# Nashatyrev/shadow

Hardware: AMD Instinct MI355X
Metric: APSP wall time + source-SSSPs/sec, 10k-vertex GML graph, 1/2/4/8 MI355X (higher is better)
Workload: dtype u32+f32

## Files before the change

### include/shadow_routing.h

```cpp
#ifndef SHADOW_ROUTING_H
#define SHADOW_ROUTING_H

#include <stddef.h>
#include <stdint.h>

#ifdef __cplusplus
extern "C" {
#endif

#define SRG_OK 0
#define SRG_ERR_ARG 1
#define SRG_ERR_NO_EDGE 2
#define SRG_ERR_MULTI_EDGE 3
#define SRG_ERR_UNREACHABLE 4
#define SRG_ERR_LATENCY_RANGE 5
#define SRG_ERR_HIP 6
#define SRG_ERR_OOM 7
#define SRG_ERR_PARSE 8
#define SRG_ERR_RCCL 9
#define SRG_ERR_INTERNAL 10

typedef struct srg_edge_list {
    uint32_t num_vertices;
    uint32_t directed;
    uint64_t num_edges;
    const uint32_t* src;
    const uint32_t* dst;
    const uint64_t* latency_ns;
    const float* packet_loss;
    const uint32_t* node_ids;
} srg_edge_list;

typedef struct srg_stats {
    double ms_total;
    double ms_h2d;
    double ms_build;
    double ms_fw;
    double ms_scan;
    double ms_loss;
    double ms_extract;
    double ms_d2h;
    int32_t path_kind;
    int32_t loss_rounds;
    uint64_t multi_pred_pairs;
    uint64_t relaxations;
    uint64_t essential_edges;
    int32_t scan_kind;
    int32_t table_keys;
    uint64_t prof_launches;
    double prof_kernel_ms;
    uint64_t prof_relaxations;
    double ms_exchange;
    int32_t nranks;
    int32_t rank;
    uint64_t local_sources;
    double ms_host_register;
    uint64_t d2h_overlapped_bytes;
    uint64_t min_latency_ns;
    uint64_t latency_unit_ns;
    int32_t fw_overlap_pivots;
    int32_t fw_overlap_kept;
    int32_t d2h_key_rows;
    int32_t reserved0;
    double ms_key_widen;
} srg_stats;

#define SRG_PATH_DENSE_U32 0
#define SRG_PATH_DENSE_U64 1
#define SRG_PATH_DIRECT 2
#define SRG_PATH_SPARSE_U32 3
#define SRG_PATH_SPARSE_U64 4

#define SRG_SCAN_NONE 0
#define SRG_SCAN_SPARSE 1
#define SRG_SCAN_DENSE 2

typedef struct srg_ctx srg_ctx;

int srg_create(srg_ctx** out, int device, char* errbuf, size_t errlen);
void srg_destroy(srg_ctx* ctx);


#define SRG_OPT_PROFILING 1
#define SRG_OPT_SPARSE_THRESHOLD 2
#define SRG_OPT_GATHER_OUTPUT 3
#define SRG_OPT_ALGORITHM 4
#define SRG_ALGO_AUTO 0
#define SRG_ALGO_DENSE 1
#define SRG_ALGO_SPARSE 2
#define SRG_OPT_SPARSE_LOCALITY 5
#define SRG_OPT_SIMULATE_RANK 6
#define SRG_OPT_FW_TILE 7
#define SRG_OPT_SPARSE_DELTA_DIV 12
#define SRG_OPT_SPARSE_GLOBAL_BITMAPS 14
#define SRG_OPT_FW_SYMMETRIC 17
#define SRG_OPT_D2H_MODE 20
#define SRG_OPT_LOSS_CHUNKS 21
#define SRG_OPT_SCAN_GROUPS 22
#define SRG_OPT_H2D_CODEC 25
#define SRG_OPT_EDGE_SHARD 29
#define SRG_OPT_LATE_LOSS 30
#define SRG_OPT_FW_LINE_SPLIT 31
#define SRG_OPT_FW_STEP 32
#define SRG_OPT_FW_OVERLAP 33
#define SRG_OPT_TEST_FAULT 34
#define SRG_OPT_TABLE_POOL_BYTES 35
#define SRG_OPT_TABLE_POOL_IDLE_BYTES 36
#define SRG_OPT_CREATE_MS_RUNTIME 37
#define SRG_OPT_CREATE_MS_LIBRARY 38
#define SRG_OPT_FW_XCD_ORDER 39
#define SRG_OPT_SCAN_MIRROR 40
#define SRG_OPT_SCAN_MIRRORED 41
#define SRG_OPT_SCAN_MIRROR_CAP 42
#define SRG_OPT_LOSS_KIND 43
#define SRG_OPT_ROUTE_TREE_ROWS 44
#define SRG_LOSS_NONE 0
#define SRG_LOSS_ROWS_LDS 1
#define SRG_LOSS_GLOBAL_ENTRIES 2
#define SRG_LOSS_DENSE_SCAN 3
int srg_set_option(srg_ctx* ctx, int option, double value);
int srg_get_option(srg_ctx* ctx, int option, double* value);

int srg_compute_shortest_paths(srg_ctx* ctx, const srg_edge_list* graph,
                               const uint32_t* nodes, uint32_t num_nodes,
                               uint64_t* out_latency_ns, float* out_packet_loss,
                               srg_stats* stats, char* errbuf, size_t errlen);

int srg_compute_shortest_paths_device(srg_ctx* ctx, const srg_edge_list* graph_dev,
                                      const uint32_t* nodes_dev, uint32_t num_nodes,
                                      uint64_t* out_latency_ns_dev, float* out_packet_loss_dev,
                                      void* hip_stream, srg_stats* stats,
                                      char* errbuf, size_t errlen);

int srg_get_direct_paths(srg_ctx* ctx, const srg_edge_list* graph,
                         const uint32_t* nodes, uint32_t num_nodes,
                         uint64_t* out_latency_ns, float* out_packet_loss,
                         srg_stats* stats, char* errbuf, size_t errlen);

typedef struct srg_routing_info srg_routing_info;
int srg_routing_info_build(srg_ctx* ctx, const srg_edge_list* graph, const uint32_t* gml_ids, uint32_t num_ids,
                           int use_shortest_paths, srg_routing_info** out, srg_stats* stats,
                           char* errbuf, size_t errlen);
struct srg_multi;
int srg_routing_info_build_multi(struct srg_multi* m, const srg_edge_list* graph, const uint32_t* gml_ids,
                                 uint32_t num_ids, int use_shortest_paths, srg_routing_info** out, srg_stats* stats,
                                 char* errbuf, size_t errlen);
void srg_routing_info_free(srg_routing_info* ri);
uint32_t srg_routing_info_num_nodes(const srg_routing_info* ri);
int srg_routing_info_path(const srg_routing_info* ri, uint32_t start_id, uint32_t end_id,
                          uint64_t* latency_ns, float* packet_loss);
void srg_routing_info_increment_packet_count(srg_routing_info* ri, uint32_t start_id, uint32_t end_id);
uint64_t srg_routing_info_packet_count(srg_routing_info* ri, uint32_t start_id, uint32_t end_id);
int srg_routing_info_smallest_latency_ns(const srg_routing_info* ri, uint64_t* out);
void srg_routing_info_tables(const srg_routing_info* ri, const uint64_t** latency_ns, const float** packet_loss,
                             const uint32_t** gml_ids, uint32_t* n);

typedef struct srg_graph srg_graph;

int srg_graph_parse_gml(const char* text, size_t len, srg_graph** out,
                        char* errbuf, size_t errlen);
void srg_graph_free(srg_graph* g);
void srg_graph_edge_list(const srg_graph* g, srg_edge_list* out);
uint32_t srg_graph_num_vertices(const srg_graph* g);
uint64_t srg_graph_num_edges(const srg_graph* g);
int srg_graph_directed(const srg_graph* g);
int srg_graph_node_index(const srg_graph* g, uint32_t gml_id, uint32_t* out_index);
uint32_t srg_graph_node_id(const srg_graph* g, uint32_t index);
void srg_graph_node_bandwidth(const srg_graph* g, uint32_t index,
                              uint64_t* down_bits, int* has_down,
                              uint64_t* up_bits, int* has_up);
void srg_graph_node_bandwidths(const srg_graph* g, uint64_t* down_bits, int* has_down,
                               uint64_t* up_bits, int* has_up);
uint32_t srg_graph_parse_chunks(const srg_graph* g);

#define SRG_UNIQUE_ID_BYTES 128
int srg_comm_unique_id(unsigned char id[SRG_UNIQUE_ID_BYTES], char* errbuf, size_t errlen);
int srg_comm_init(srg_ctx* ctx, int nranks, int rank, const unsigned char id[SRG_UNIQUE_ID_BYTES],
                  char* errbuf, size_t errlen);
typedef struct srg_local_group srg_local_group;
int srg_local_group_create(int nranks, srg_local_group** out);
void srg_local_group_release(srg_local_group* g);
int srg_comm_init_local(srg_ctx* ctx, srg_local_group* g, int rank, char* errbuf, size_t errlen);
int srg_comm_size(srg_ctx* ctx, int* nranks, int* rank);

typedef struct srg_multi srg_multi;
int srg_multi_create(srg_multi** out, const int* devices, int num_devices, char* errbuf, size_t errlen);
void srg_multi_destroy(srg_multi* m);
int srg_multi_size(const srg_multi* m);
int srg_multi_set_option(srg_multi* m, int option, double value);
int srg_multi_compute_shortest_paths(srg_multi* m, const srg_edge_list* graph, const uint32_t* nodes,
                                     uint32_t num_nodes, uint64_t* out_latency_ns, float* out_packet_loss,
                                     srg_stats* stats, char* errbuf, size_t errlen);
int srg_multi_get_direct_paths(srg_multi* m, const srg_edge_list* graph, const uint32_t* nodes, uint32_t num_nodes,
                               uint64_t* out_latency_ns, float* out_packet_loss, srg_stats* stats, char* errbuf,
                               size_t errlen);

#define SRG_ERR_EVENT_ORDER 11
typedef struct srg_event_batch {
    uint64_t num_events;
    const uint32_t* src_node;
    const uint32_t* dst_node;
    const uint32_t* src_host;
    const uint32_t* dst_host;
    const uint64_t* send_time_ns;
    const uint64_t* src_event_id;
    uint32_t num_hosts;
    uint32_t reserved;
    uint64_t round_end_ns;
} srg_event_batch;

typedef struct srg_event_result {
    uint64_t min_next_event_ns;
    uint64_t min_used_latency_ns;
    uint32_t key_bits;
    uint32_t radix_passes;
    double ms_total;
} srg_event_result;

int srg_order_packet_events_device(srg_ctx* ctx, const srg_event_batch* batch_dev,
                                   const uint64_t* latency_table_dev, uint32_t table_n,
                                   uint64_t* out_deliver_ns_dev, uint32_t* out_order_dev,
                                   uint64_t* out_host_offsets_dev, void* hip_stream,
                                   srg_event_result* result, char* errbuf, size_t errlen);

typedef struct srg_path_table_dev {
    uint32_t n, reserved;
    const uint64_t* latency_ns;
    const uint32_t* latency_key;
    const uint64_t* diag_ns;
    uint64_t unit_ns;
    const float* packet_loss;
} srg_path_table_dev;

typedef struct srg_send_batch {
    srg_event_batch ev;
    const double* chance;
    const uint32_t* payload_size;
    uint64_t bootstrap_end_ns;
} srg_send_batch;

typedef struct srg_send_result { srg_event_result ev; uint64_t num_sent, num_dropped; } srg_send_result;

int srg_send_packets_device(srg_ctx* ctx, const srg_send_batch* batch_dev, const srg_path_table_dev* table,
                            uint8_t* out_status_dev, uint64_t* out_deliver_ns_dev, uint32_t* out_order_dev,
                            uint64_t* out_host_offsets_dev, uint64_t* packet_counts_dev ,
                            void* hip_stream, srg_send_result* result, char* errbuf, size_t errlen);

int srg_routing_info_key_tables(const srg_routing_info* ri, const uint32_t** key, const uint64_t** diag_ns,
                                uint64_t* unit_ns, const float** packet_loss, uint32_t* n);
void srg_routing_info_add_packet_counts(srg_routing_info* ri, const uint64_t* counts_by_position );

#define SRG_ERR_TIME_BACKWARD 12
typedef struct srg_event_queues srg_event_queues;
int srg_event_queues_create(srg_ctx* ctx, uint32_t num_hosts, uint64_t reserve_events, srg_event_queues** out,
                            char* errbuf, size_t errlen);
void srg_event_queues_destroy(srg_event_queues* q);
uint32_t srg_event_queues_merge_tile(void);

typedef struct srg_queue_result {
    uint64_t num_moved;
    uint64_t num_queued;
    uint64_t min_next_event_ns;
    double ms_total;
} srg_queue_result;

int srg_event_queues_push_device(srg_event_queues* q, const srg_event_batch* batch_dev,
                                 const uint64_t* deliver_ns_dev, const uint32_t* order_dev, uint64_t num_order,
                                 const uint64_t* tag_dev, void* hip_stream, srg_queue_result* result, char* errbuf,
                                 size_t errlen);

int srg_event_queues_pop_device(srg_event_queues* q, uint64_t until_ns, uint64_t out_capacity,
                                uint64_t* out_time_ns_dev, uint32_t* out_src_host_dev, uint64_t* out_src_event_id_dev,
                                uint64_t* out_tag_dev, uint64_t* out_host_offsets_dev, void* hip_stream,
                                srg_queue_result* result, char* errbuf, size_t errlen);

int srg_next_window(uint64_t min_next_event_ns, uint64_t runahead_ns, uint64_t end_time_ns,
                    uint64_t* window_start_ns, uint64_t* window_end_ns);

typedef struct srg_inbound srg_inbound;
int srg_inbound_create(srg_ctx* ctx, uint32_t num_hosts, const uint64_t* bw_down_bits, uint64_t sim_start_ns,
                       uint64_t bootstrap_end_ns, uint64_t reserve_packets, srg_inbound** out, char* errbuf,
                       size_t errlen);
void srg_inbound_destroy(srg_inbound* q);

typedef struct srg_inbound_result {
    uint64_t num_forwarded, num_dropped;
    uint64_t num_queued;
    uint64_t min_next_wake_ns;
    double ms_total;
} srg_inbound_result;

int srg_inbound_step_device(srg_inbound* q, uint64_t until_ns, uint64_t num_arrivals, const uint64_t* time_ns_dev,
                            const uint32_t* total_size_dev, const uint64_t* tag_dev, const uint64_t* host_offsets_dev,
                            uint64_t out_capacity, uint8_t* out_status_dev, uint64_t* out_time_ns_dev,
                            uint64_t* out_tag_dev, uint64_t* out_host_offsets_dev, void* hip_stream,
                            srg_inbound_result* result, char* errbuf, size_t errlen);

struct srg_inbound_host_state {
    uint64_t balance, last_refill_ns;
    uint64_t interval_end_ns, drop_next_ns;
    uint64_t current_drop_count, previous_drop_count, bytes_stored;
    uint64_t queued;
    uint64_t wake_ns, cached_tag;
    uint8_t mode;
    uint8_t has_interval_end, has_drop_next, pending, has_cached, reserved[3];
};
int srg_inbound_host_state(srg_inbound* q, uint32_t host, struct srg_inbound_host_state* out);

#define SRG_ERR_ROUTE 13
typedef struct srg_route_result {
    uint64_t num_pairs;
    uint64_t total_hops;
    uint64_t bad_pair;
    uint32_t max_hops, reserved;
    double ms_total;
} srg_route_result;

int srg_trace_routes_device(srg_ctx* ctx, const srg_edge_list* graph_dev, const srg_path_table_dev* table,
                            const uint32_t* src_dev, const uint32_t* dst_dev, uint64_t num_pairs,
                            uint64_t hop_capacity, uint64_t* out_hop_offsets_dev ,
                            uint32_t* out_hop_edge_dev ,
                            uint32_t* out_hop_vertex_dev ,
                            void* hip_stream, srg_route_result* result, char* errbuf, size_t errlen);

int srg_link_loads_device(srg_ctx* ctx, const srg_edge_list* graph_dev, const srg_path_table_dev* table,
                          const uint64_t* packet_counts_dev ,
                          uint64_t* edge_packets_dev ,
                          void* hip_stream, srg_route_result* result, char* errbuf, size_t errlen);

#define SRG_ROUTE_NONE 0xFFFFFFFFu

int srg_route_trees_device(srg_ctx* ctx, const srg_edge_list* graph_dev, const srg_path_table_dev* table,
                           const uint32_t* sources_dev, uint32_t num_sources,
                           uint32_t* out_pred_edge_dev   ,
                           uint32_t* out_pred_vertex_dev ,
                           uint32_t* out_hops_dev        ,
                           uint32_t* out_first_edge_dev  ,
                           void* hip_stream, srg_route_result* result, char* errbuf, size_t errlen);

int srg_link_loads_trees_device(srg_ctx* ctx, const srg_edge_list* graph_dev, const srg_path_table_dev* table,
                                const uint64_t* packet_counts_dev, uint64_t* edge_packets_dev,
                                void* hip_stream, srg_route_result* result, char* errbuf, size_t errlen);

const char* srg_version(void);

#ifdef __cplusplus
}
#endif
#endif
```

### shadow_amd/_native.py

```python
import ctypes
import os

_HERE = os.path.dirname(os.path.abspath(__file__))
LIB_PATH = os.path.join(_HERE, "libshadow_routing.so")

SRG_OK = 0
SRG_ERR_ARG = 1
SRG_ERR_NO_EDGE = 2
SRG_ERR_MULTI_EDGE = 3
SRG_ERR_UNREACHABLE = 4
SRG_ERR_LATENCY_RANGE = 5
SRG_ERR_HIP = 6
SRG_ERR_OOM = 7
SRG_ERR_PARSE = 8
SRG_ERR_RCCL = 9
SRG_ERR_INTERNAL = 10
SRG_ERR_EVENT_ORDER = 11
SRG_ERR_TIME_BACKWARD = 12
SRG_ERR_ROUTE = 13

SRG_PATH_DENSE_U32 = 0
SRG_PATH_DENSE_U64 = 1
SRG_PATH_DIRECT = 2
SRG_PATH_SPARSE_U32 = 3
SRG_PATH_SPARSE_U64 = 4

SRG_OPT_PROFILING = 1
SRG_OPT_SPARSE_THRESHOLD = 2
SRG_OPT_GATHER_OUTPUT = 3
SRG_OPT_ALGORITHM = 4
SRG_OPT_SPARSE_LOCALITY = 5
SRG_OPT_SIMULATE_RANK = 6
SRG_OPT_FW_TILE = 7
SRG_OPT_SPARSE_DELTA_DIV = 12
SRG_OPT_SPARSE_GLOBAL_BITMAPS = 14
SRG_OPT_FW_SYMMETRIC = 17
SRG_OPT_D2H_MODE = 20
SRG_OPT_LOSS_CHUNKS = 21
SRG_OPT_SCAN_GROUPS = 22
SRG_OPT_H2D_CODEC = 25
SRG_OPT_EDGE_SHARD = 29
SRG_OPT_LATE_LOSS = 30
SRG_OPT_FW_LINE_SPLIT = 31
SRG_OPT_FW_STEP = 32
SRG_OPT_FW_OVERLAP = 33
SRG_OPT_TEST_FAULT = 34
SRG_OPT_TABLE_POOL_BYTES = 35
SRG_OPT_TABLE_POOL_IDLE_BYTES = 36
SRG_OPT_CREATE_MS_RUNTIME = 37
SRG_OPT_CREATE_MS_LIBRARY = 38
SRG_OPT_FW_XCD_ORDER = 39
SRG_OPT_SCAN_MIRROR = 40
SRG_OPT_SCAN_MIRRORED = 41
SRG_OPT_SCAN_MIRROR_CAP = 42
SRG_OPT_LOSS_KIND = 43
SRG_OPT_ROUTE_TREE_ROWS = 44
SRG_ROUTE_NONE = 0xFFFFFFFF
SRG_LOSS_NONE = 0
SRG_LOSS_ROWS_LDS = 1
SRG_LOSS_GLOBAL_ENTRIES = 2
SRG_LOSS_DENSE_SCAN = 3
SRG_ALGO_AUTO = 0
SRG_ALGO_DENSE = 1
SRG_ALGO_SPARSE = 2
SRG_UNIQUE_ID_BYTES = 128

SRG_SCAN_NONE = 0
SRG_SCAN_SPARSE = 1
SRG_SCAN_DENSE = 2

_u32p = ctypes.POINTER(ctypes.c_uint32)
_u64p = ctypes.POINTER(ctypes.c_uint64)
_f32p = ctypes.POINTER(ctypes.c_float)


class EdgeList(ctypes.Structure):
    _fields_ = [
        ("num_vertices", ctypes.c_uint32),
        ("directed", ctypes.c_uint32),
        ("num_edges", ctypes.c_uint64),
        ("src", ctypes.c_void_p),
        ("dst", ctypes.c_void_p),
        ("latency_ns", ctypes.c_void_p),
        ("packet_loss", ctypes.c_void_p),
        ("node_ids", ctypes.c_void_p),
    ]


class EventBatch(ctypes.Structure):
    _fields_ = [
        ("num_events", ctypes.c_uint64),
        ("src_node", ctypes.c_void_p),
        ("dst_node", ctypes.c_void_p),
        ("src_host", ctypes.c_void_p),
        ("dst_host", ctypes.c_void_p),
        ("send_time_ns", ctypes.c_void_p),
        ("src_event_id", ctypes.c_void_p),
        ("num_hosts", ctypes.c_uint32),
        ("reserved", ctypes.c_uint32),
        ("round_end_ns", ctypes.c_uint64),
    ]


class EventResult(ctypes.Structure):
    _fields_ = [
        ("min_next_event_ns", ctypes.c_uint64),
        ("min_used_latency_ns", ctypes.c_uint64),
        ("key_bits", ctypes.c_uint32),
        ("radix_passes", ctypes.c_uint32),
        ("ms_total", ctypes.c_double),
    ]

    def as_dict(self):
        return {k: getattr(self, k) for k, _ in self._fields_}


class PathTableDev(ctypes.Structure):
    _fields_ = [
        ("n", ctypes.c_uint32),
        ("reserved", ctypes.c_uint32),
        ("latency_ns", ctypes.c_void_p),
        ("latency_key", ctypes.c_void_p),
        ("diag_ns", ctypes.c_void_p),
        ("unit_ns", ctypes.c_uint64),
        ("packet_loss", ctypes.c_void_p),
    ]


class SendBatch(ctypes.Structure):
    _fields_ = [
        ("ev", EventBatch),
        ("chance", ctypes.c_void_p),
        ("payload_size", ctypes.c_void_p),
        ("bootstrap_end_ns", ctypes.c_uint64),
    ]


class SendResult(ctypes.Structure):
    _fields_ = [
        ("ev", EventResult),
        ("num_sent", ctypes.c_uint64),
        ("num_dropped", ctypes.c_uint64),
    ]

    def as_dict(self):
        d = self.ev.as_dict()
        d.update(num_sent=self.num_sent, num_dropped=self.num_dropped)
        return d


class QueueResult(ctypes.Structure):
    _fields_ = [
        ("num_moved", ctypes.c_uint64),
        ("num_queued", ctypes.c_uint64),
        ("min_next_event_ns", ctypes.c_uint64),
        ("ms_total", ctypes.c_double),
    ]

    def as_dict(self):
        return {k: getattr(self, k) for k, _ in self._fields_}


class InboundResult(ctypes.Structure):
    _fields_ = [
        ("num_forwarded", ctypes.c_uint64),
        ("num_dropped", ctypes.c_uint64),
        ("num_queued", ctypes.c_uint64),
        ("min_next_wake_ns", ctypes.c_uint64),
        ("ms_total", ctypes.c_double),
    ]

    def as_dict(self):
        return {k: getattr(self, k) for k, _ in self._fields_}


class InboundHostState(ctypes.Structure):
    _fields_ = [
        ("balance", ctypes.c_uint64),
        ("last_refill_ns", ctypes.c_uint64),
        ("interval_end_ns", ctypes.c_uint64),
        ("drop_next_ns", ctypes.c_uint64),
        ("current_drop_count", ctypes.c_uint64),
        ("previous_drop_count", ctypes.c_uint64),
        ("bytes_stored", ctypes.c_uint64),
        ("queued", ctypes.c_uint64),
        ("wake_ns", ctypes.c_uint64),
        ("cached_tag", ctypes.c_uint64),
        ("mode", ctypes.c_uint8),
        ("has_interval_end", ctypes.c_uint8),
        ("has_drop_next", ctypes.c_uint8),
        ("pending", ctypes.c_uint8),
        ("has_cached", ctypes.c_uint8),
        ("reserved", ctypes.c_uint8 * 3),
    ]

    def as_dict(self):
        return {k: int(getattr(self, k)) for k, _ in self._fields_ if k != "reserved"}


class RouteResult(ctypes.Structure):
    _fields_ = [
        ("num_pairs", ctypes.c_uint64),
        ("total_hops", ctypes.c_uint64),
        ("bad_pair", ctypes.c_uint64),
        ("max_hops", ctypes.c_uint32),
        ("reserved", ctypes.c_uint32),
        ("ms_total", ctypes.c_double),
    ]

    def as_dict(self):
        return {k: getattr(self, k) for k, _ in self._fields_}


class Stats(ctypes.Structure):
    _fields_ = [
        ("ms_total", ctypes.c_double),
        ("ms_h2d", ctypes.c_double),
        ("ms_build", ctypes.c_double),
        ("ms_fw", ctypes.c_double),
        ("ms_scan", ctypes.c_double),
        ("ms_loss", ctypes.c_double),
        ("ms_extract", ctypes.c_double),
        ("ms_d2h", ctypes.c_double),
        ("path_kind", ctypes.c_int32),
        ("loss_rounds", ctypes.c_int32),
        ("multi_pred_pairs", ctypes.c_uint64),
        ("relaxations", ctypes.c_uint64),
        ("essential_edges", ctypes.c_uint64),
        ("scan_kind", ctypes.c_int32),
        ("table_keys", ctypes.c_int32),
        ("prof_launches", ctypes.c_uint64),
        ("prof_kernel_ms", ctypes.c_double),
        ("prof_relaxations", ctypes.c_uint64),
        ("ms_exchange", ctypes.c_double),
        ("nranks", ctypes.c_int32),
        ("rank", ctypes.c_int32),
        ("local_sources", ctypes.c_uint64),
        ("ms_host_register", ctypes.c_double),
        ("d2h_overlapped_bytes", ctypes.c_uint64),
        ("min_latency_ns", ctypes.c_uint64),
        ("latency_unit_ns", ctypes.c_uint64),
        ("fw_overlap_pivots", ctypes.c_int32),
        ("fw_overlap_kept", ctypes.c_int32),
        ("d2h_key_rows", ctypes.c_int32),
        ("reserved0", ctypes.c_int32),
        ("ms_key_widen", ctypes.c_double),
    ]

    def as_dict(self):
        return {k: getattr(self, k) for k, _ in self._fields_}


EXPORTS = [
    "srg_create", "srg_destroy", "srg_set_option", "srg_compute_shortest_paths", "srg_compute_shortest_paths_device",
    "srg_get_direct_paths", "srg_graph_parse_gml", "srg_graph_free", "srg_graph_edge_list",
    "srg_graph_num_vertices", "srg_graph_num_edges", "srg_graph_directed", "srg_graph_node_index",
    "srg_graph_node_id", "srg_graph_node_bandwidth", "srg_graph_node_bandwidths", "srg_graph_parse_chunks",
    "srg_version", "srg_comm_unique_id", "srg_comm_init",
    "srg_local_group_create", "srg_local_group_release", "srg_comm_init_local", "srg_comm_size",
    "srg_order_packet_events_device", "srg_routing_info_build", "srg_routing_info_free", "srg_routing_info_num_nodes",
    "srg_routing_info_path", "srg_routing_info_increment_packet_count", "srg_routing_info_packet_count",
    "srg_routing_info_smallest_latency_ns", "srg_routing_info_tables",
    "srg_multi_create", "srg_multi_destroy", "srg_multi_size", "srg_multi_set_option", "srg_multi_compute_shortest_paths",
    "srg_multi_get_direct_paths", "srg_routing_info_build_multi", "srg_get_option",
    "srg_send_packets_device", "srg_routing_info_key_tables", "srg_routing_info_add_packet_counts",
    "srg_event_queues_create", "srg_event_queues_destroy", "srg_event_queues_merge_tile",
    "srg_event_queues_push_device", "srg_event_queues_pop_device", "srg_next_window",
    "srg_trace_routes_device", "srg_link_loads_device", "srg_route_trees_device", "srg_link_loads_trees_device",
    "srg_inbound_create", "srg_inbound_destroy", "srg_inbound_step_device", "srg_inbound_host_state",
]

_lib = None


def lib():
    global _lib
    if _lib is not None:
        return _lib
    try:
        import torch
    except ImportError:
        pass
    if not os.path.exists(LIB_PATH):
        raise ImportError(
            f"{LIB_PATH} is missing: build it with `python shadow_amd/build.py` "
            "(hipcc --offload-arch=gfx950); there is no CPU fallback")
    L = ctypes.CDLL(os.environ.get("SRG_LIB_PATH") or LIB_PATH)
    c = ctypes
    L.srg_create.restype = c.c_int
    L.srg_create.argtypes = [c.POINTER(c.c_void_p), c.c_int, c.c_char_p, c.c_size_t]
    L.srg_set_option.restype = c.c_int
    L.srg_set_option.argtypes = [c.c_void_p, c.c_int, c.c_double]
    L.srg_destroy.restype = None
    L.srg_destroy.argtypes = [c.c_void_p]
    host_sig = [c.c_void_p, c.POINTER(EdgeList), c.c_void_p, c.c_uint32, c.c_void_p, c.c_void_p,
                c.POINTER(Stats), c.c_char_p, c.c_size_t]
    L.srg_compute_shortest_paths.restype = c.c_int
    L.srg_compute_shortest_paths.argtypes = host_sig
    L.srg_get_direct_paths.restype = c.c_int
    L.srg_get_direct_paths.argtypes = host_sig
    L.srg_compute_shortest_paths_device.restype = c.c_int
    L.srg_compute_shortest_paths_device.argtypes = [
        c.c_void_p, c.POINTER(EdgeList), c.c_void_p, c.c_uint32, c.c_void_p, c.c_void_p, c.c_void_p,
        c.POINTER(Stats), c.c_char_p, c.c_size_t]
    L.srg_graph_parse_gml.restype = c.c_int
    L.srg_graph_parse_gml.argtypes = [c.c_char_p, c.c_size_t, c.POINTER(c.c_void_p), c.c_char_p, c.c_size_t]
    L.srg_graph_free.restype = None
    L.srg_graph_free.argtypes = [c.c_void_p]
    L.srg_graph_edge_list.restype = None
    L.srg_graph_edge_list.argtypes = [c.c_void_p, c.POINTER(EdgeList)]
    L.srg_graph_num_vertices.restype = c.c_uint32
    L.srg_graph_num_vertices.argtypes = [c.c_void_p]
    L.srg_graph_num_edges.restype = c.c_uint64
    L.srg_graph_num_edges.argtypes = [c.c_void_p]
    L.srg_graph_directed.restype = c.c_int
    L.srg_graph_directed.argtypes = [c.c_void_p]
    L.srg_graph_node_index.restype = c.c_int
    L.srg_graph_node_index.argtypes = [c.c_void_p, c.c_uint32, _u32p]
    L.srg_graph_node_id.restype = c.c_uint32
    L.srg_graph_node_id.argtypes = [c.c_void_p, c.c_uint32]
    L.srg_graph_node_bandwidth.restype = None
    L.srg_graph_node_bandwidth.argtypes = [c.c_void_p, c.c_uint32, _u64p, c.POINTER(c.c_int), _u64p,
                                           c.POINTER(c.c_int)]
    L.srg_graph_node_bandwidths.restype = None
    L.srg_graph_node_bandwidths.argtypes = [c.c_void_p, c.c_void_p, c.c_void_p, c.c_void_p, c.c_void_p]
    L.srg_graph_parse_chunks.restype = c.c_uint32
    L.srg_graph_parse_chunks.argtypes = [c.c_void_p]
    L.srg_version.restype = c.c_char_p
    L.srg_version.argtypes = []
    L.srg_comm_unique_id.restype = c.c_int
    L.srg_comm_unique_id.argtypes = [c.c_char_p, c.c_char_p, c.c_size_t]
    L.srg_comm_init.restype = c.c_int
    L.srg_comm_init.argtypes = [c.c_void_p, c.c_int, c.c_int, c.c_char_p, c.c_char_p, c.c_size_t]
    L.srg_local_group_create.restype = c.c_int
    L.srg_local_group_create.argtypes = [c.c_int, c.POINTER(c.c_void_p)]
    L.srg_local_group_release.restype = None
    L.srg_local_group_release.argtypes = [c.c_void_p]
    L.srg_comm_init_local.restype = c.c_int
    L.srg_comm_init_local.argtypes = [c.c_void_p, c.c_void_p, c.c_int, c.c_char_p, c.c_size_t]
    L.srg_order_packet_events_device.restype = c.c_int
    L.srg_order_packet_events_device.argtypes = [
        c.c_void_p, c.POINTER(EventBatch), c.c_void_p, c.c_uint32, c.c_void_p, c.c_void_p, c.c_void_p, c.c_void_p,
        c.POINTER(EventResult), c.c_char_p, c.c_size_t]
    L.srg_send_packets_device.restype = c.c_int
    L.srg_send_packets_device.argtypes = [
        c.c_void_p, c.POINTER(SendBatch), c.POINTER(PathTableDev), c.c_void_p, c.c_void_p, c.c_void_p, c.c_void_p,
        c.c_void_p, c.c_void_p, c.POINTER(SendResult), c.c_char_p, c.c_size_t]
    L.srg_routing_info_key_tables.restype = c.c_int
    L.srg_routing_info_key_tables.argtypes = [c.c_void_p, c.POINTER(_u32p), c.POINTER(_u64p), _u64p, c.POINTER(_f32p),
                                              c.POINTER(c.c_uint32)]
    L.srg_routing_info_add_packet_counts.restype = None
    L.srg_routing_info_add_packet_counts.argtypes = [c.c_void_p, c.c_void_p]
    L.srg_event_queues_create.restype = c.c_int
    L.srg_event_queues_create.argtypes = [c.c_void_p, c.c_uint32, c.c_uint64, c.POINTER(c.c_void_p), c.c_char_p,
                                          c.c_size_t]
    L.srg_event_queues_destroy.restype = None
    L.srg_event_queues_destroy.argtypes = [c.c_void_p]
    L.srg_event_queues_merge_tile.restype = c.c_uint32
    L.srg_event_queues_merge_tile.argtypes = []
# ... 83 lines not shown
```

### shadow_amd/csrc/dense.hip.h

```cpp
template <class K, int T>
bool run_dense(srg_ctx& c, const DevGraph& g, const Plan& pl, const uint32_t* nodes, uint32_t n, uint64_t* out_lat,
               float* out_loss, hipStream_t st, const Prelude& P, srg_stats* stats, HostSink* sink,
               FwOverlap* ov = nullptr) {
    const bool pre = ov && ov->on && ov->ok && ov->ended && sizeof(K) == 4 && T == FwOverlap::T;
    if (sizeof(K) == 8 && c.kout_key) {
        if (!(sink && sink->widen)) fail(SRG_INTERNAL_NEED_U64, "the build needs u64 latency keys: no u32 key table");
        sink->widen = false;
        c.kout_key = nullptr;
        c.kout_diag = nullptr;
    }
    const uint32_t V = g.V;
    const size_t Vp = ((size_t)V + T - 1) / T * T;
    const size_t VV = Vp * Vp;
    const bool multi = c.comm && c.comm->nranks > 1;
    Timer tm(st);

    K* W = (K*)c.b_W.get(VV * sizeof(K));
    uint32_t* WL = (uint32_t*)c.b_WL.get(VV * 4);
    K* D = (K*)c.b_D.get(VV * sizeof(K));
    bool wl_late = false;
    if (pre) {
        wl_late = g.late && !g.late->applied;
    } else if constexpr (sizeof(K) == 4) {
        static_assert(T % 64 == 0, "tile");
        unsigned long long* KW = (unsigned long long*)c.b_PRED.get(VV * 8);
        HIP_CHECK(hipMemsetAsync(KW, 0xFF, VV * 8, st));
        wl_late = g.late && !g.late->applied;
        if (g.E) k_w_key<<<grid_for(g.E), kThreads, 0, st>>>(g.E, g.src, g.dst, g.lat, P.unit, wl_late ? nullptr : g.loss, KW, Vp);
        const unsigned nb64 = (unsigned)(Vp / 64);
        k_w_split<false><<<dim3(nb64, nb64), 256, 0, st>>>(KW, Vp, g.directed, (uint32_t*)W, WL, (uint32_t*)D);
    } else {
        loss_arrive(g, P.selfloss, st);
        k_fill<K><<<grid_for(VV), kThreads, 0, st>>>(W, VV, KeyOps<K>::INF);
        HIP_CHECK(hipMemsetAsync(WL, 0xFF, VV * 4, st));
        if (g.E) {
            k_w_lat<K><<<grid_for(g.E), kThreads, 0, st>>>(g.E, g.src, g.dst, g.lat, P.unit, g.directed, W, Vp);
            k_w_loss<K><<<grid_for(g.E), kThreads, 0, st>>>(g.E, g.src, g.dst, g.lat, P.unit, g.loss, g.directed, W, WL,
                                                             Vp);
        }
        k_init_d<K><<<grid_for(VV), kThreads, 0, st>>>(W, D, Vp);
    }
    const uint32_t nloc = (uint32_t)pl.lnodes.size();
    uint32_t* lnodes = (uint32_t*)c.b_lnodes.get(std::max<size_t>(nloc, 1) * 4);
    uint32_t* lpos = (uint32_t*)c.b_lpos.get(std::max<size_t>(nloc, 1) * 4);
    if (nloc) {
        HIP_CHECK(hipMemcpyAsync(lnodes, pl.lnodes.data(), (size_t)nloc * 4, hipMemcpyHostToDevice, st));
        HIP_CHECK(hipMemcpyAsync(lpos, pl.lpos.data(), (size_t)nloc * 4, hipMemcpyHostToDevice, st));
    }
    HIP_CHECK(hipGetLastError());
    const double ms_build = tm.lap();

    uint64_t prof_relax = 0;
    int prof_n = 0;
    double ms_dx = 0;
    if (pre) {
        prof_relax = ov->prof_relax;
        prof_n = ov->prof_n;
    } else if (sym_fw_for<K, T>(c, g)) {
        if constexpr ((sizeof(K) == 4 && T == 128) || (sizeof(K) == 8 && T == 64))
            fw_line_sym<K, T>(c, pl, D, Vp, st, prof_relax, prof_n, ms_dx);
    } else {
        if constexpr (sizeof(K) == 4) fw_blocked<K, T, 2>(c, pl, D, Vp, st, prof_relax, prof_n);
        else fw_blocked<K, T, 0>(c, pl, D, Vp, st, prof_relax, prof_n);
        if (multi) gather_rows<K>(c, pl, D, Vp, T, st, ms_dx);
    }
    HIP_CHECK(hipGetLastError());
    if (sym_fw_for<K, T>(c, g)) rb_async(c, MS_TIMEOUT, c.fw_timeout, st);
    const double ms_fw = tm.lap();
    if (sym_fw_for<K, T>(c, g) && rb_get<uint32_t>(c, MS_TIMEOUT))
        fail(SRG_ERR_HIP, fw_timeout_message(rb_get<uint32_t>(c, MS_TIMEOUT)));
#ifdef SRG_TEST_HOOKS
    if (c.test_fault == 1)
        HIP_CHECK(hipMemsetAsync(D, 0, VV * sizeof(K), st));
#endif
    if (wl_late) {
        hipStream_t ax = c.aux_stream;
        const auto tl0 = std::chrono::steady_clock::now();
        loss_arrive(g, P.selfloss, ax);
        if (srg_env::debug_overlap())
            std::fprintf(stderr, "late loss: the host waited %.2f ms for the loss thread after FW\n",
                         std::chrono::duration<double, std::milli>(std::chrono::steady_clock::now() - tl0).count());
        if constexpr (sizeof(K) == 4) {
            unsigned long long* KW = (unsigned long long*)c.b_PRED.get(VV * 8);
            HIP_CHECK(hipMemsetAsync(KW, 0xFF, VV * 8, ax));
            if (g.E) k_w_key<<<grid_for(g.E), kThreads, 0, ax>>>(g.E, g.src, g.dst, g.lat, P.unit, g.loss, KW, Vp);
            const unsigned nb64 = (unsigned)(Vp / 64);
            k_w_split<true><<<dim3(nb64, nb64), 256, 0, ax>>>(KW, Vp, g.directed, nullptr, WL, nullptr);
            HIP_CHECK(hipGetLastError());
        }
        HIP_CHECK(hipEventRecord(c.ev_wlate, ax));
    }
    if (prof_n && stats) {
        double sum = 0;
        for (int i = 0; i < prof_n; ++i) {
            float ms = 0;
            HIP_CHECK(hipEventElapsedTime(&ms, c.prof_events[2 * i], c.prof_events[2 * i + 1]));
            sum += ms;
        }
        stats->prof_launches += prof_n;
        stats->prof_kernel_ms += sum;
        stats->prof_relaxations += prof_relax;
    }

    hipStream_t cs = c.comm_stream;
    auto cs_after_st = [&]() {
        HIP_CHECK(hipEventRecord(c.ev_a, st));
        HIP_CHECK(hipStreamWaitEvent(cs, c.ev_a, 0));
    };
    auto st_after_cs = [&]() {
        HIP_CHECK(hipEventRecord(c.ev_b, cs));
        HIP_CHECK(hipStreamWaitEvent(st, c.ev_b, 0));
    };
    auto reduce_flag = [&](uint32_t* flag_dev) -> uint32_t {
        uint32_t* red = (uint32_t*)c.b_red.get(16);
        HIP_CHECK(hipMemcpyAsync(red, flag_dev, 4, hipMemcpyDeviceToDevice, st));
        if (multi) {
            cs_after_st();
            c.comm->allreduce_max_u32(red, 1, cs);
            st_after_cs();
        }
        rb_async(c, MS_REDUCE, red, st);
        HIP_CHECK(hipStreamSynchronize(st));
        return rb_get<uint32_t>(c, MS_REDUCE);
    };
    const bool exchange = multi && c.gather_output;
    auto exchange_rows = [&](void* out, size_t elem) {
        const size_t row = (size_t)n * elem;
        std::vector<size_t> offs, lens;
        slice_tables(n, pl.G, row, offs, lens);
        cs_after_st();
        c.comm->allgatherv(out, offs.data(), lens.data(), cs);
    };

    hipStream_t es = multi ? st : c.comm_stream;
    auto drain_es = [&]() {
        if (es != st) HIP_CHECK(hipStreamSynchronize(es));
    };
    constexpr int TS = 64;
    constexpr int VE = 16 / (int)sizeof(K);
    const size_t nmax = std::max<uint32_t>(nloc, 1);
    uint32_t* PRED = (uint32_t*)c.b_PRED.get(nmax * Vp * 4);
    unsigned long long* multi_cnt = (unsigned long long*)c.b_multi.get(16);
    uint32_t* mirror_cnt = (uint32_t*)(multi_cnt + 1);
    int rounds = 0;
    unsigned long long nmulti = 0;
    uint64_t n_ess = 0;
    int scan_kind = SRG_SCAN_NONE;
    bool loss_written = false;
    float* Lfin = nullptr;
    double ms_scan = 0;
    HIP_CHECK(hipMemsetAsync(multi_cnt, 0, 8, st));
    const uint32_t nw64 = (V + 63) / 64;
    unsigned long long* ess = (unsigned long long*)c.b_ess.get((size_t)V * nw64 * 8);
    k_ess_mask<K><<<V, 256, 0, es>>>(W, D, Vp, V, 0u, V, nw64, ess);
    uint32_t* indeg = (uint32_t*)c.b_indeg.get(((size_t)nw64 * 64 + 1) * 4);
    uint32_t* cscoff = (uint32_t*)c.b_cscoff.get(((size_t)nw64 * 64 + 1) * 4);
    HIP_CHECK(hipMemsetAsync(indeg, 0, ((size_t)nw64 * 64 + 1) * 4, es));
    const bool v5lo = sizeof(K) == 8;
    const uint32_t SB = V5_SB;
    const size_t npad = ((size_t)nloc + SB - 1) / SB * SB;
    const size_t dst_bytes = (size_t)nw64 * 64 * std::max<size_t>(npad, 64) * sizeof(K);
    const uint32_t NT = nw64 * 64;
    const uint32_t nK5 = (V + V5_UC - 1) / V5_UC, nbTT5 = (NT + V5_TT - 1) / V5_TT;
    const size_t NG5 = (size_t)nbTT5 * nK5 * V5_WAVES;
    uint32_t* v5_cnt = (uint32_t*)c.b_ecnt.get((size_t)nbTT5 * nK5 * V5_TT * 4);
    uint32_t* v5_goff = (uint32_t*)c.b_eoff.get((NG5 + 1) * 4);
    uint64_t E_ess = 0, E_layout = 0;
    {
        uint32_t* v5_glen = (uint32_t*)c.b_rlen.get((NG5 + 1) * 4);
        HIP_CHECK(hipMemsetAsync(v5_cnt, 0, (size_t)nbTT5 * nK5 * V5_TT * 4, es));
        HIP_CHECK(hipMemsetAsync(v5_glen, 0, (NG5 + 1) * 4, es));
        const size_t nwaves = (size_t)nw64 * nK5;
        k_v5_count<<<(unsigned)((nwaves * 64 + 255) / 256), 256, 0, es>>>(ess, V, nw64, nK5, v5_cnt, v5_glen, indeg);
        HIP_CHECK(hipGetLastError());
        size_t ta = 0, tc = 0;
        HIP_CHECK(hipcub::DeviceScan::ExclusiveSum(nullptr, ta, indeg, cscoff, (int)(NT + 1), es));
        HIP_CHECK(hipcub::DeviceScan::ExclusiveSum(nullptr, tc, v5_glen, v5_goff, (int)(NG5 + 1), es));
        const size_t tbytes = std::max(ta, tc);
        void* tmp = c.b_scantmp.get(tbytes);
        HIP_CHECK(hipcub::DeviceScan::ExclusiveSum(tmp, ta, indeg, cscoff, (int)(NT + 1), es));
        HIP_CHECK(hipcub::DeviceScan::ExclusiveSum(tmp, tc, v5_glen, v5_goff, (int)(NG5 + 1), es));
        HIP_CHECK(hipGetLastError());
    }

    HIP_CHECK(hipMemsetAsync(&P.flags->inf_in_used_row, 0, 4, st));
    HIP_CHECK(hipMemsetAsync(&P.flags->impossible, 0, 4, st));
    if (nloc)
        k_certify<K><<<nloc, kThreads, 0, st>>>(
            D, Vp, lnodes, nloc, nodes, n,
            (K)std::min<uint64_t>(min_edge_key(P.es.min_lat_inv, P.unit), (uint64_t)KeyOps<K>::INF), P.flags);
    const bool simulated = c.comm && std::strcmp(c.comm->kind(), "simulated") == 0;
    uint32_t impossible = 0, inf_any = 0;
    if (multi) {
        impossible = reduce_flag(&P.flags->impossible);
        inf_any = reduce_flag(&P.flags->inf_in_used_row);
    } else {
        rb_async(c, MS_REDUCE, &P.flags->impossible, st);
        rb_async(c, MS_REDUCE2, &P.flags->inf_in_used_row, st);
        HIP_CHECK(hipStreamSynchronize(st));
        impossible = rb_get<uint32_t>(c, MS_REDUCE);
        inf_any = rb_get<uint32_t>(c, MS_REDUCE2);
    }
    if (impossible && !simulated)
        fail(SRG_ERR_INTERNAL, "FW produced an impossible table: a used pair's latency is below the smallest edge "
                               "latency (" + std::to_string(~P.es.min_lat_inv) + " ns)");
    if (sizeof(K) == 4 && inf_any) {
        const unsigned __int128 bound = (unsigned __int128)P.max_key * (V > 1 ? V - 1 : 1);
        if (bound >= KeyOps<uint32_t>::INF) {
            if (wl_late) HIP_CHECK(hipStreamWaitEvent(st, c.ev_wlate, 0));
            drain_es();
            return false;
        }
        fail(SRG_ERR_UNREACHABLE,
             "assertion `left == right` failed: paths.len() != nodes.len().pow(2) (a used node is unreachable "
             "from another used node)");
    }
    if (P.wrap_risk) {
        const unsigned __int128 bound = (unsigned __int128)P.max_key * (V > 1 ? V - 1 : 1);
        const bool inf_known = sizeof(K) == 4 ? bound < KeyOps<uint32_t>::INF : !P.range_risk;
        HIP_CHECK(hipMemsetAsync(&P.flags->wrap, 0, 8, st));
        for (uint32_t r0 = 0; r0 < nloc && g.E; r0 += 32768) {
            const uint32_t nr = std::min<uint32_t>(32768, nloc - r0);
            k_wrap_edges<K><<<dim3(grid_for(g.E, 64), nr), 256, 0, st>>>(g.E, g.src, g.dst, g.lat, g.directed, D, Vp,
                                                                        lnodes + r0, P.unit, inf_known ? 1 : 0, P.flags);
        }
        HIP_CHECK(hipGetLastError());
        const uint32_t wrapped = reduce_flag(&P.flags->wrap);
        if (wrapped)
            fail(SRG_ERR_LATENCY_RANGE, "a shortest-path relaxation sums past 2^64 ns (max edge latency " +
                                            std::to_string(P.es.max_lat) +
                                            " ns): the reference's u64 latency sum would wrap (mod.rs:327)");
        if (reduce_flag(&P.flags->wrap_inf)) {
            if (sizeof(K) == 4) {
                if (wl_late) HIP_CHECK(hipStreamWaitEvent(st, c.ev_wlate, 0));
                drain_es();
                return false;
            }
            fail(SRG_ERR_LATENCY_RANGE, "a vertex has no path below 2^62 latency units on a graph whose u64 latency "
                                        "sums can wrap (max edge latency " +
                                            std::to_string(P.es.max_lat) + " ns)");
        }
    }

    HIP_CHECK(hipMemsetAsync(&P.flags->unreachable_used_pair, 0, 4, st));
    const bool al16 = (((uintptr_t)out_lat | (uintptr_t)c.kout_key) & 15u) == 0;
    if (nloc && P.ident && n % 4 == 0 && al16)
        k_extract_ident<K><<<nloc, 256, 0, st>>>(D, Vp, lnodes, n, P.selflat, out_lat, P.flags, P.unit, c.kout_key,
                                                 c.kout_diag);
    else if (nloc)
        k_extract<K><<<nloc, kThreads, 0, st>>>(D, nullptr, Vp, lnodes, nloc, nodes, n, lpos,
                                                                      P.selflat, P.selfloss, out_lat, out_loss,
                                                                      P.flags, 1, P.unit, c.kout_key, c.kout_diag);
    HIP_CHECK(hipGetLastError());
    if (reduce_flag(&P.flags->unreachable_used_pair)) {
        if (sizeof(K) == 8 && P.range_risk)
            fail(SRG_ERR_LATENCY_RANGE, "a used pair has no path below 2^62 latency units (max edge latency " +
                                            std::to_string(P.es.max_lat) +
                                            " ns): unreachable, or a latency sum the reference's u64 would wrap");
        fail(SRG_ERR_UNREACHABLE,
             "assertion `left == right` failed: paths.len() != nodes.len().pow(2) (a used node is unreachable "
             "from another used node)");
    }
    if (exchange) exchange_rows(out_lat, 8);
    const bool sink_rows = sink && !exchange && nloc && sink->ok();
    if (sink && c.kout_key) sink->key_unit = P.unit;
    if (sink_rows) {
        if (c.kout_key && sink->widen) sink->send_keys(st, c.kout_key, pl.p0, nloc, P.unit);
        else if (c.kout_key) sink->send_rows(st, c.kout_key, sink->lat, pl.p0, nloc, 4);
        else sink->send_rows(st, out_lat, sink->lat, pl.p0, nloc, 8);
        sink->lat_sent = true;
    }

    {
        rb_async(c, MS_TAIL0, cscoff + NT, es);
        rb_async(c, MS_TAIL1, v5_goff + NG5, es);
        HIP_CHECK(hipStreamSynchronize(es));
        E_ess = rb_get<uint32_t>(c, MS_TAIL0);
        E_layout = 2ull * rb_get<uint32_t>(c, MS_TAIL1);
    }
    n_ess = E_ess;
    if (wl_late) HIP_CHECK(hipStreamWaitEvent(st, c.ev_wlate, 0));
    const bool sparse = (double)E_ess <= c.sparse_threshold * (double)V * (double)V &&
                        E_layout + 256 < 0xF0000000ull && dst_bytes < 0xFFFFFFFFull;
    if (sparse) {
        scan_kind = SRG_SCAN_SPARSE;
        K* DST = nullptr;
        const uint32_t* DSTs = nullptr;
        uint32_t dsts_bytes = 0;
        if (nloc) {
            hipStream_t ax = c.aux_stream;
            const uint32_t nbS = (uint32_t)(npad / 64);
            DST = (K*)c.b_DST.get(dst_bytes);
            k_build_dst<K><<<dim3(nw64, nbS), 256, 0, ax>>>(D, Vp, lnodes, nloc, DST, npad);
            DSTs = (const uint32_t*)DST;
            dsts_bytes = (uint32_t)std::min<size_t>(dst_bytes, 0xFFFFFFFFull);
            if (v5lo) {
                const size_t cnt = dst_bytes / 8;
                uint32_t* lo = (uint32_t*)c.b_DST2.get(cnt * 4);
                k_low_words<<<grid_for(cnt), kThreads, 0, ax>>>(reinterpret_cast<const uint64_t*>(DST), cnt, lo);
                DSTs = lo;
                dsts_bytes = (uint32_t)(cnt * 4);
            }
            HIP_CHECK(hipGetLastError());
            HIP_CHECK(hipEventRecord(c.ev_dst, ax));
        }
        const size_t Eb = E_layout + 256;
        uint32_t* cscpos = (uint32_t*)c.b_cscfill.get((size_t)nbTT5 * nK5 * V5_TT * 4);
        K* ent_w = (K*)c.b_entw.get(Eb * sizeof(K));
        uint2* ent_ub = (uint2*)c.b_grpe.get(Eb * 8);
        uint32_t* cscent = (uint32_t*)c.b_cscent.get(std::max<uint64_t>(E_ess, 1) * 4);
        k_v5_cscpos<<<(NT + 255) / 256, 256, 0, st>>>(v5_cnt, cscoff, NT, nK5, cscpos);
        uint2* rec = (uint2*)c.b_entkey.get((Eb + V5_SLACK) * 8);
        {
            const size_t nwaves = (size_t)nw64 * nK5;
            k_v5_fill<K><<<(unsigned)((nwaves * 64 + 255) / 256), 256, 0, st>>>(ess, W, WL, Vp, V, nw64, nK5, v5_cnt,
                                                                                  v5_goff, cscpos, rec, ent_w,
                                                                                  ent_ub, cscent);
        }
        HIP_CHECK(hipGetLastError());
        const size_t lds_rows = loss_rows_lds(V);
        const bool rows_lds = V <= srg_env::loss_rows_max_v(LOSS_ROWS_MAX_V);
        bool mirror = c.scan_mirror && !g.directed && pl.G == 1 && !multi && !simulated && nloc == n && P.ident &&
                      !v5lo && rows_lds;
        const uint32_t scan_groups = c.scan_groups ? (uint32_t)c.scan_groups : mirror ? 4u : 3u;
        const bool interleave = sink_rows && rows_lds && scan_groups > 1;
        if (interleave) set_lds(k_loss_rows<K, true>, lds_rows);
        uint32_t* PREDK = rows_lds ? (uint32_t*)c.b_PRED2.get(nmax * Vp * 8) : nullptr;
        auto pack_pred = [&](uint32_t r0, uint32_t r1) {
            const uint32_t nsb = (r1 - r0 + 127) / 128, nt8 = (nbTT5 + 7) / 8;
            k_pred_pack<<<8u * nt8 * nsb, 256, 0, st>>>(PRED, Vp, r0, r1, NT, nbTT5, nsb, ent_ub, (uint2*)PREDK,
                                                        multi_cnt, mirror ? 1u : 0u);
            HIP_CHECK(hipGetLastError());
        };
        auto mirror_rows = [&](uint32_t r0, uint32_t r1) {
            if (r1 <= r0 || r1 <= SB) return;
            const size_t pairs = (size_t)(r1 - r0) * Vp, room = std::min<size_t>(pairs / 2, (size_t)1 << 30);
            const uint32_t cap = (uint32_t)std::min<size_t>(
                room, c.scan_mirror_cap ? (size_t)c.scan_mirror_cap : std::max<size_t>(pairs / 1024, 256));
            uint2* work = (uint2*)(PRED + (size_t)r0 * Vp);
            HIP_CHECK(hipMemsetAsync(mirror_cnt, 0, 4, st));
            const uint32_t nlow = (r1 - 1) / SB * SB;
            k_pred_mirror<<<dim3(nlow / 64, (r1 - r0 + 63) / 64), 256, 0, st>>>((uint2*)PREDK, Vp, r0, r1, V, work, cap,
                                                                               mirror_cnt, multi_cnt);
            k_mirror_slow<K><<<1024, 256, 0, st>>>(work, mirror_cnt, cap, DST, npad, ent_ub, ent_w, cscoff, cscent,
                                                   (uint2*)PREDK, Vp, multi_cnt);
            HIP_CHECK(hipGetLastError());
        };
        std::vector<uint32_t> tri_h;
        if (nloc) HIP_CHECK(hipStreamWaitEvent(st, c.ev_dst, 0));
        for (bool again = nloc != 0; again;) {
            again = false;
            if (interleave) HIP_CHECK(hipMemsetAsync(&P.flags->changed, 0, 4, st));
            const uint32_t inf_check = v5lo ? 0u : 1u;
            const uint32_t nbS5 = (uint32_t)(npad / SB);
            const uint32_t ng = interleave ? std::min<uint32_t>(scan_groups, nbS5) : 1u;
            auto cut = [&](uint32_t q) { return mirror ? scan_group_cut_tri(q, ng, nbS5) : scan_group_cut(q, ng, nbS5); };
            const uint32_t* tri_d = nullptr;
            std::vector<size_t> tri_off(ng + 1, 0);
            if (mirror) {
                tri_h.clear();
                for (uint32_t gi = 0; gi < ng; ++gi) {
                    tri_scan_blocks(cut(gi), cut(gi + 1), nbTT5, tri_h);
                    tri_off[gi + 1] = tri_h.size();
                }
                uint32_t* d = (uint32_t*)c.b_tri.get(std::max<size_t>(tri_h.size(), 1) * 4);
                if (!tri_h.empty()) HIP_CHECK(hipMemcpyAsync(d, tri_h.data(), tri_h.size() * 4, hipMemcpyHostToDevice, st));
                HIP_CHECK(hipMemsetAsync(mirror_cnt, 0, 8, st));
                tri_d = d;
            }
            for (uint32_t gi = 0; gi < ng; ++gi) {
                const uint32_t c0 = cut(gi), c1 = cut(gi + 1);
                if (c1 == c0) continue;
                const uint32_t nblk = mirror ? (uint32_t)(tri_off[gi + 1] - tri_off[gi])
                                             : (nbTT5 + 3) / 4 * ((c1 - c0 + 7) / 8);
                if (nblk)
                    tight_v5<<<8u * 32u * ((nblk + 7) / 8), V5_WAVES * 64, 0, st>>>(
                        DSTs, npad, dsts_bytes, lnodes, nloc, V, NT, nbTT5, c1, nK5, c0, v5_goff,
                        (const uint32_t*)c.b_entkey.get(0), PRED, Vp, inf_check, mirror ? tri_d + tri_off[gi] : nullptr);
                HIP_CHECK(hipGetLastError());
                if (interleave) {
                    const uint32_t r0 = c0 * SB, r1 = std::min<uint32_t>(c1 * SB, nloc);
                    if (r1 <= r0) continue;
                    pack_pred(r0, r1);
                    if (mirror) mirror_rows(r0, r1);
                    k_loss_rows<K, true><<<r1 - r0, 1024, lds_rows, st>>>(PREDK, Vp, V, lnodes, nloc, ent_ub, ent_w,
                                                                   DST, npad, cscoff, cscent, P.selfloss, nodes, n,
                                                                   lpos, out_loss, &P.flags->changed, r0,
                                                                   mirror ? mirror_cnt + 1 : nullptr);
                    HIP_CHECK(hipGetLastError());
                    sink->send_rows(st, out_loss, sink->loss, pl.p0 + r0, r1 - r0, 4);
                }
            }
            if (!PREDK) k_count_multi<<<nloc, kThreads, 0, st>>>(PRED, nloc, V, Vp, multi_cnt);
            HIP_CHECK(hipGetLastError());
            ms_scan += tm.lap();
            if (interleave) {
                sink->loss_sent = true;
                rb_async(c, MS_CHANGED, &P.flags->changed, st);
                if (mirror) rb_async(c, MS_MIRROR, mirror_cnt + 1, st);
                HIP_CHECK(hipStreamSynchronize(st));
                rounds = (int)rb_get<uint32_t>(c, MS_CHANGED);
                loss_written = true;
                c.loss_kind = SRG_LOSS_ROWS_LDS;
            } else if (rows_lds) {
                set_lds(k_loss_rows<K, true>, lds_rows);
                HIP_CHECK(hipMemsetAsync(&P.flags->changed, 0, 4, st));
                pack_pred(0, nloc);
                if (mirror) mirror_rows(0, nloc);
                const uint32_t nchunk = std::max<uint32_t>(1, std::min<uint32_t>(c.loss_chunks ? c.loss_chunks : sink_rows ? 8 : 1, nloc));
                for (uint32_t q = 0; q < nchunk; ++q) {
                    const uint32_t r0 = (uint32_t)((uint64_t)nloc * q / nchunk);
                    const uint32_t r1 = (uint32_t)((uint64_t)nloc * (q + 1) / nchunk);
                    if (r1 == r0) continue;
                    k_loss_rows<K, true><<<r1 - r0, 1024, lds_rows, st>>>(PREDK, Vp, V, lnodes, nloc, ent_ub, ent_w,
                                                                   DST, npad, cscoff, cscent, P.selfloss, nodes, n,
                                                                   lpos, out_loss, &P.flags->changed, r0,
                                                                   mirror ? mirror_cnt + 1 : nullptr);
                    HIP_CHECK(hipGetLastError());
                    if (sink_rows) sink->send_rows(st, out_loss, sink->loss, pl.p0 + r0, r1 - r0, 4);
                }
                if (sink_rows) sink->loss_sent = true;
                rb_async(c, MS_CHANGED, &P.flags->changed, st);
                if (mirror) rb_async(c, MS_MIRROR, mirror_cnt + 1, st);
                HIP_CHECK(hipStreamSynchronize(st));
                rounds = (int)rb_get<uint32_t>(c, MS_CHANGED);
                loss_written = true;
                c.loss_kind = SRG_LOSS_ROWS_LDS;
            } else {
                c.loss_kind = SRG_LOSS_GLOBAL_ENTRIES;
                float* L0 = (float*)c.b_L0.get(nmax * Vp * 4);
                float* L1 = (float*)c.b_L1.get(nmax * Vp * 4);
                k_fill<float><<<grid_for((size_t)nloc * Vp), kThreads, 0, st>>>(L0, (size_t)nloc * Vp, 1.0f);
                float* Lin = L0;
                float* Lout = L1;
                for (;;) {
                    HIP_CHECK(hipMemsetAsync(&P.flags->changed, 0, 4, st));
                    k_loss_round_sparse<K><<<grid_for((size_t)nloc * V, 256 * 64), kThreads, 0, st>>>(
                        PRED, Vp, DST, npad, lnodes, nloc, V, ent_ub, ent_w, cscoff, cscent, Lin, Lout,
                        &P.flags->changed);
                    HIP_CHECK(hipGetLastError());
                    ++rounds;
                    rb_async(c, MS_CHANGED, &P.flags->changed, st);
                    HIP_CHECK(hipStreamSynchronize(st));
                    const uint32_t ch = rb_get<uint32_t>(c, MS_CHANGED);
                    std::swap(Lin, Lout);
                    if (!ch) break;
                    if (rounds > (int)V + 2) fail(SRG_ERR_INTERNAL, "loss rounds did not converge");
                }
                Lfin = Lin;
            }
            if (mirror) {
                c.scan_mirrored = 1;
                if (rb_get<uint32_t>(c, MS_MIRROR)) {
                    c.scan_mirrored = 2;
                    mirror = false;
                    again = true;
                    rounds = 0;
                    loss_written = false;
                    HIP_CHECK(hipMemsetAsync(multi_cnt, 0, 8, st));
                }
            }
        }
    } else {
        scan_kind = SRG_SCAN_DENSE;
        if (nloc) {
            c.loss_kind = SRG_LOSS_DENSE_SCAN;
            const size_t lds3 = (size_t)2 * KC * (TS + VE) * sizeof(K);
            set_lds(tight_scan<K, TS, KC>, lds3);
            tight_scan<K, TS, KC><<<dim3((unsigned)(Vp / TS), (nloc + TS - 1) / TS), 256, lds3, st>>>(D, W, Vp, lnodes,
                                                                                                    nloc, PRED);
            k_count_multi<<<nloc, kThreads, 0, st>>>(PRED, nloc, V, Vp, multi_cnt);
            float* L0 = (float*)c.b_L0.get(nmax * Vp * 4);
            float* L1 = (float*)c.b_L1.get(nmax * Vp * 4);
            k_fill<float><<<grid_for((size_t)nloc * Vp), kThreads, 0, st>>>(L0, (size_t)nloc * Vp, 1.0f);
            HIP_CHECK(hipGetLastError());
            ms_scan = tm.lap();
            float* Lin = L0;
            float* Lout = L1;
            for (;;) {
                HIP_CHECK(hipMemsetAsync(&P.flags->changed, 0, 4, st));
                k_loss_round<K><<<grid_for((size_t)nloc * V, 256 * 64), kThreads, 0, st>>>(
                    PRED, D, W, WL, lnodes, nloc, V, Vp, Lin, Lout, P.flags);
                HIP_CHECK(hipGetLastError());
                ++rounds;
                rb_async(c, MS_CHANGED, &P.flags->changed, st);
                HIP_CHECK(hipStreamSynchronize(st));
                const uint32_t ch = rb_get<uint32_t>(c, MS_CHANGED);
                std::swap(Lin, Lout);
                if (!ch) break;
                if (rounds > (int)V + 2) fail(SRG_ERR_INTERNAL, "loss rounds did not converge");
            }
            Lfin = Lin;
        }
    }
    rb_async(c, MS_NMULTI, multi_cnt, st);
    const double ms_loss = tm.lap();
    nmulti = rb_get<unsigned long long>(c, MS_NMULTI);

    if (nloc && !loss_written)
        k_extract<K><<<nloc, kThreads, 0, st>>>(D, Lfin, Vp, lnodes, nloc, nodes, n, lpos,
                                                                      P.selflat, P.selfloss, out_lat, out_loss,
                                                                      P.flags, 2, P.unit);
    HIP_CHECK(hipGetLastError());
    const double ms_extract = tm.lap();

    double ms_exchange = 0;
    if (exchange) {
        exchange_rows(out_loss, 4);
        st_after_cs();
        ms_exchange = tm.lap();
    }
    if (stats) {
        stats->ms_build += ms_build;
        stats->ms_fw += ms_fw;
        stats->ms_scan += ms_scan;
        stats->ms_loss += ms_loss;
        stats->ms_extract += ms_extract;
        stats->ms_exchange += ms_exchange + ms_dx;
        stats->path_kind = sizeof(K) == 4 ? SRG_PATH_DENSE_U32 : SRG_PATH_DENSE_U64;
        stats->loss_rounds = rounds;
        stats->multi_pred_pairs = nmulti;
        uint64_t own_tiles = 0;
        for (int I = 0; I < pl.nb; ++I)
            for (int J = I; J < pl.nb; ++J) own_tiles += (I + J) % pl.G == pl.g;
        stats->relaxations = sym_fw_for<K, T>(c, g) ? own_tiles * (uint64_t)pl.nb * T * T * T
                                                    : (uint64_t)(pl.rb1 - pl.rb0) * T * Vp * Vp;
        stats->essential_edges = n_ess;
        stats->scan_kind = scan_kind;
        stats->nranks = pl.G;
        stats->rank = pl.g;
        stats->local_sources = nloc;
    }
    return true;
}
```

### shadow_amd/csrc/host_entry.hip.h

```cpp

int check_entry_args(const srg_ctx* c, const srg_edge_list* g, const uint32_t* nodes, uint32_t num_nodes,
                     const uint64_t* out_lat, const float* out_loss, bool direct, const uint32_t* out_key,
                     const uint64_t* out_diag, char* errbuf, size_t errlen) {
    const bool keys = out_key != nullptr;
    if (keys && (direct || (c && c->comm && c->comm->nranks > 1) || (num_nodes && !out_diag))) {
        set_err(errbuf, errlen, "key table: one rank, shortest paths only");
        return SRG_ERR_ARG;
    }
    if (!c || !g || (num_nodes && (!nodes || !(out_lat || keys) || !out_loss)) ||
        (g->num_edges && (!g->src || !g->dst || !g->latency_ns || !g->packet_loss))) {
        set_err(errbuf, errlen, "null argument");
        return SRG_ERR_ARG;
    }
    return SRG_OK;
}

struct OutputPinning {
    int device = 0;
    std::thread th;
    bool ok = false;
    double ms = 0;
    void* p[2] = {nullptr, nullptr};
    void* view[2] = {nullptr, nullptr};
    size_t b[2] = {0, 0};
    hipStream_t wait = nullptr;
    bool fault = true;
    srg_table* tab[2] = {nullptr, nullptr};
    bool join() {
        if (th.joinable()) th.join();
        return ok;
    }
    void run() {
        const auto t0 = std::chrono::steady_clock::now();
        if (!b[0] || hipSetDevice(device) != hipSuccess) return;
        for (int i = 0; i < 2; ++i) {
            if (tab[i] && tab[i]->registered) {
                view[i] = tab[i]->view;
                continue;
            }
            advise_huge(p[i], b[i]);
            if (fault) prefault(p[i], b[i], 8);
            if (hipHostRegister(p[i], b[i], hipHostRegisterMapped) != hipSuccess) {
                if (i == 1 && !tab[0]) (void)hipHostUnregister(p[0]);
                return;
            }
            if (hipHostGetDevicePointer(&view[i], p[i], 0) != hipSuccess) view[i] = nullptr;
            if (tab[i]) tab[i]->registered = true, tab[i]->view = view[i];
        }
        ms = ms_since(t0);
        ok = true;
    }
    ~OutputPinning() {
        if (th.joinable()) th.join();
        if (ok) {
            (void)hipStreamSynchronize(wait);
            for (int i = 0; i < 2; ++i)
                if (!tab[i]) (void)hipHostUnregister(p[i]);
        }
    }
};

void start_pinning(OutputPinning& reg, const srg_ctx& c, const EntryPlan& ep, bool ext, unsigned char* lat_b,
                   size_t lat_elem, float* out_loss, size_t n, srg_table* const* tabs) {
    reg.device = c.device;
    reg.wait = c.d2h_stream;
    reg.fault = srg_env::prefault_on();
    if (!ep.early || ext) return;
    const bool pooled = !ep.rows_part && tabs && tabs[0] && tabs[1] && tabs[0]->p == lat_b &&
                        tabs[1]->p == (void*)out_loss && tabs[0]->cap >= n * n * lat_elem && tabs[1]->cap >= n * n * 4;
    reg.p[0] = lat_b + ep.rows.lo * n * lat_elem;
    reg.b[0] = ep.rows.size() * n * lat_elem;
    reg.p[1] = out_loss + ep.rows.lo * n;
    reg.b[1] = ep.rows.size() * n * 4;
    if (pooled)
        for (int i = 0; i < 2; ++i) reg.tab[i] = tabs[i], reg.b[i] = tabs[i]->cap;
    reg.th = std::thread([r = &reg]() { r->run(); });
}

struct Shipped {
    bool coded = false;
    bool all_narrow = false, all_seq = false;
    hipStream_t hst = nullptr;
};
Shipped ship_edges(srg_ctx& c, const srg_edge_list* g, const uint32_t* nodes, size_t n, bool direct, bool sparse,
                   const EntryPlan& ep, bool sim, hipStream_t st, DevGraph& dg, FwOverlap& ov, LateLoss& late,
                   srg_stats* stats) {
    const size_t E = g->num_edges, a0 = ep.edges.lo, a1 = ep.edges.hi;
    Shipped sh;
    const bool want_late = c.late_loss && !direct;
    const bool ov_want = c.fw_overlap && !direct && ep.nr == 1 && want_late && c.h2d_codec && E >= ((size_t)1 << 20) &&
                         !g->directed && c.fw_symmetric && (c.fw_tile == 0 || c.fw_tile == 128) &&
                         g->num_vertices >= 256 && n > 0 && !sparse;
    if (ov_want) {
        HIP_CHECK(hipStreamSynchronize(c.aux_stream));
        ov.init(c, g->num_vertices, std::vector<uint32_t>(nodes, nodes + n));
    }
    const hipStream_t hst = sh.hst = ov.on ? c.comm_stream : st;
    ChunkFn on_chunk = nullptr;
    if (ov.on) on_chunk = [&](size_t e0, size_t ne, const uint32_t* exc, size_t nexc, bool last) {
        ov.chunk(dg, e0, ne, exc, nexc, last);
    };
    const bool coded = sh.coded = c.h2d_codec && a1 - a0 >= ((size_t)1 << 20) &&
                                  codec_in(c, g, dg, hst, a0, a1, !want_late, sh.all_narrow, sh.all_seq, on_chunk);
    if (ov.on) ov.finish();
    if (ov.on && !coded) ov.ok = false;
    const int ov_early = ov.next;
    if (stats && ov.on && ov.ok) stats->fw_overlap_pivots = ov_early;
    if (ov.on && ov.ok && !ov.ended) ov.advance(ov.nb - 1);
    if (ov.on && srg_env::debug_overlap()) {
        std::fprintf(stderr, "fw-overlap: ok=%d pivots_during_h2d=%d of %d\n", ov.ok ? 1 : 0, ov_early, ov.nb);
        if (ov.ok) ov.report();
    }
    late.ls = c.loss_stream;
    if (coded && want_late) start_late_loss(c, g, dg, hst, late, a0, a1);
    if (!coded) {
        const size_t cnt = std::max<size_t>(E, 1);
        dg.src = (uint32_t*)c.b_src.get(cnt * 4);
        dg.dst = (uint32_t*)c.b_dst.get(cnt * 4);
        dg.lat = (uint64_t*)c.b_lat.get(cnt * 8);
        dg.loss = (float*)c.b_loss.get(cnt * 4);
        copy_plain(dg, g, a0, a1, true, st);
    }
    if (sim && (c.sim_edges != g->src || c.sim_E != E)) {
        copy_plain(dg, g, 0, a0, true, st);
        copy_plain(dg, g, a1, E, true, st);
        c.sim_edges = g->src;
        c.sim_E = E;
    }
    return sh;
}

void exchange_slices(srg_ctx& c, const srg_edge_list* g, const DevGraph& dg, const EntryPlan& ep, const Shipped& sh,
                     bool sim, hipStream_t st) {
    const size_t E = g->num_edges, a0 = ep.edges.lo, a1 = ep.edges.hi;
    const int nr = ep.nr, rk = ep.rk;
    std::vector<size_t> offs(nr), lens(nr);
    auto gather = [&](const void* p, size_t elem) {
        slice_tables(E, nr, elem, offs, lens);
        c.comm->allgatherv(const_cast<void*>(p), offs.data(), lens.data(), st);
    };
    auto late_or_gather_loss = [&]() {
        if (dg.late) {
            dg.late->comm = c.comm;
            slice_tables(E, nr, 4, dg.late->offs, dg.late->lens);
        } else {
            gather(dg.loss, 4);
        }
    };
    auto decode_others = [&](auto&& launch) {
        for (auto [e0, e1] : {std::pair<size_t, size_t>{0, a0}, std::pair<size_t, size_t>{a1, E}})
            if (e1 > e0 && !sim) launch(e0, e1);
        HIP_CHECK(hipGetLastError());
    };
    uint32_t* plain = (uint32_t*)c.b_red.get(16);
    const uint32_t mine = offered_form(sh.coded, sh.all_seq, sh.all_narrow);
    HIP_CHECK(hipMemcpyAsync(plain, &mine, 4, hipMemcpyHostToDevice, st));
    c.comm->allreduce_max_u32(plain, 1, st);
    uint32_t form = 2;
    HIP_CHECK(hipMemcpyAsync(&form, plain, 4, hipMemcpyDeviceToHost, st));
    HIP_CHECK(hipStreamSynchronize(st));
    if (form == 0) {
        const size_t xbase = ((size_t)nr * 4 + 255) / 256 * 256;
        uint32_t* xc = (uint32_t*)c.b_xexc.get(xbase);
        const uint32_t my_n = (uint32_t)(c.slice_exc.size() / 3);
        HIP_CHECK(hipMemcpyAsync(xc + rk, &my_n, 4, hipMemcpyHostToDevice, st));
        for (int q = 0; q < nr; ++q) {
            offs[q] = (size_t)q * 4;
            lens[q] = 4;
        }
        c.comm->allgatherv(xc, offs.data(), lens.data(), st);
        std::vector<uint32_t> cnt(nr);
        HIP_CHECK(hipMemcpyAsync(cnt.data(), xc, (size_t)nr * 4, hipMemcpyDeviceToHost, st));
        HIP_CHECK(hipStreamSynchronize(st));
        if (sim)
            for (int q = 0; q < nr; ++q) cnt[q] = my_n;
        size_t tot = 0, mine_at = 0;
        for (int q = 0; q < nr; ++q) {
            if (q == rk) mine_at = tot;
            offs[q] = xbase + tot * 12;
            lens[q] = (size_t)cnt[q] * 12;
            tot += cnt[q];
        }
        unsigned char* xb = (unsigned char*)c.b_xexc.get(xbase + std::max<size_t>(tot, 1) * 12);
        if (my_n)
            HIP_CHECK(hipMemcpyAsync(xb + xbase + mine_at * 12, c.slice_exc.data(), (size_t)my_n * 12,
                                     hipMemcpyHostToDevice, st));
        c.comm->allgatherv(xb, offs.data(), lens.data(), st);
        uint32_t* l32 = (uint32_t*)c.b_n32l.p;
        gather(l32, 4);
        late_or_gather_loss();
        decode_others([&](size_t e0, size_t e1) {
            k_decode_seq_global<<<grid_for(e1 - e0), kThreads, 0, st>>>(e0, e1, l32, (const uint32_t*)(xb + xbase),
                                                                         (uint32_t)tot, (uint32_t*)dg.src,
                                                                         (uint32_t*)dg.dst, (uint64_t*)dg.lat);
        });
    } else if (form == 1) {
        uint16_t* s16 = (uint16_t*)c.b_n16s.p;
        uint16_t* d16 = (uint16_t*)c.b_n16d.p;
        uint32_t* l32 = (uint32_t*)c.b_n32l.p;
        gather(s16, 2);
        gather(d16, 2);
        gather(l32, 4);
        late_or_gather_loss();
        decode_others([&](size_t e0, size_t e1) {
            k_widen_edges<<<grid_for(e1 - e0), kThreads, 0, st>>>(e1 - e0, s16 + e0, d16 + e0, l32 + e0, (uint32_t*)dg.src + e0,
                                                                   (uint32_t*)dg.dst + e0, (uint64_t*)dg.lat + e0);
        });
    } else {
        gather(dg.src, 4);
        gather(dg.dst, 4);
        gather(dg.lat, 8);
        if (dg.late) {
            dg.late->join();
            HIP_CHECK(hipStreamWaitEvent(st, dg.late->ev_in, 0));
        }
        gather(dg.loss, 4);
    }
}

struct DevTables {
    uint64_t* lat = nullptr;
    float* loss = nullptr;
    uint32_t* key = nullptr;
    uint64_t* diag = nullptr;
};

DevTables output_tables(srg_ctx& c, const EntryPlan& ep, size_t n) {
    const size_t q0 = ep.rows.lo, dev_nn = ep.rows.size() * n;
    DevTables t;
    t.lat = reinterpret_cast<uint64_t*>(reinterpret_cast<uintptr_t>(c.b_olat.get(std::max<size_t>(dev_nn, 1) * 8)) -
                                        q0 * n * 8);
    t.loss = reinterpret_cast<float*>(reinterpret_cast<uintptr_t>(c.b_oloss.get(std::max<size_t>(dev_nn, 1) * 4)) -
                                      q0 * n * 4);
    return t;
}

bool wants_key_rows(const srg_ctx& c, const EntryPlan& ep, bool keys, bool direct, size_t n, bool sparse) {
    return !keys && !direct && ep.early && ep.nr == 1 && c.sdma.ok && c.d2h_mode == 1 && c.h_ring && c.pool &&
           n * 4 <= c.h_ring_bytes / 3 && !srg_env::no_key_d2h() && !sparse;
}

struct KeyScope {
    srg_ctx& c;
    KeyScope(srg_ctx& c_, DevTables& t, bool kmode, size_t n) : c(c_) {
        t.key = kmode ? reinterpret_cast<uint32_t*>(t.lat) : nullptr;
        t.diag = kmode ? (uint64_t*)c.b_odiag.get(std::max<size_t>(n, 1) * 8) : nullptr;
        c.kout_key = t.key;
        c.kout_diag = t.diag;
    }
    ~KeyScope() { c.kout_key = nullptr, c.kout_diag = nullptr; }
};

void wire_sink(HostSink& sink, srg_ctx& c, const EntryPlan& ep, bool ext, OutputPinning& reg, uint64_t* host_lat,
               float* out_loss, size_t n, bool ikeys) {
    sink.lat = host_lat;
    sink.widen = ikeys;
    sink.pool = c.pool;
    sink.ring = (unsigned char*)c.h_ring;
    sink.ring_slot = c.h_ring_bytes / 3;
    sink.loss = out_loss;
    sink.n = n;
    sink.cs = c.d2h_stream;
    sink.ev = c.ev_e;
    if (!ep.early) return;
    sink.mode = c.d2h_mode;
    sink.sdma = &c.sdma;
    sink.device = c.device;
    if (ext) {
        sink.ready = [cp = &c, pin = &reg, s = &sink]() {
            void* v[2] = {nullptr, nullptr};
            if (!cp->ext_reg(v, &pin->ms)) return false;
            s->lat_view = v[0];
            s->loss_view = v[1];
            return true;
        };
    } else {
        sink.ready = [pin = &reg, s = &sink, reg_r0 = ep.rows.lo, n]() {
            if (!pin->join()) return false;
            s->lat_view = (unsigned char*)pin->view[0] - reg_r0 * n * 8;
            s->loss_view = (unsigned char*)pin->view[1] - reg_r0 * n * 4;
            return true;
        };
    }
}

unsigned long long ship_tail(srg_ctx& c, const EntryPlan& ep, size_t n, bool keys, bool ikeys, const DevTables& t,
                             HostSink& sink, uint64_t* out_lat, uint32_t* out_key, uint64_t* out_diag, float* out_loss,
                             const srg_stats* stats, hipStream_t st) {
    const bool kmode = keys || ikeys;
    const size_t r0 = ep.rows.lo, r1 = ep.rows.hi;
    const size_t rows_off = r0 * n, rows_nn = r1 > r0 ? (r1 - r0) * n : 0;
    unsigned long long hmin = ~0ull;
    if (rows_nn && stats) {
        unsigned long long* dmin = (unsigned long long*)c.b_multi.get(16);
        HIP_CHECK(hipMemsetAsync(dmin, 0xFF, 16, st));
        if (kmode) {
            k_min_u32<<<grid_for(rows_nn, 1024), kThreads, 0, st>>>(t.key + rows_off, rows_nn, dmin);
            k_min_u64<<<grid_for(n, 1024), kThreads, 0, st>>>(t.diag, n, dmin + 1);
        } else {
            k_min_u64<<<grid_for(rows_nn, 1024), kThreads, 0, st>>>(t.lat + rows_off, rows_nn, dmin);
        }
        HIP_CHECK(hipMemcpyAsync(c.hbox + 64 * MS_MIN, dmin, 16, hipMemcpyDeviceToHost, st));
    }
    if (rows_nn && !sink.lat_sent) {
        if (keys)
            HIP_CHECK(hipMemcpyAsync(out_key + rows_off, t.key + rows_off, rows_nn * 4, hipMemcpyDeviceToHost, st));
        else if (!ikeys)
            HIP_CHECK(hipMemcpyAsync(out_lat + rows_off, t.lat + rows_off, rows_nn * 8, hipMemcpyDeviceToHost, st));
    }
    if (keys && n) HIP_CHECK(hipMemcpyAsync(out_diag, t.diag, n * 8, hipMemcpyDeviceToHost, st));
    std::vector<uint64_t> hdiag(ikeys ? n : 0);
    if (ikeys && n) HIP_CHECK(hipMemcpyAsync(hdiag.data(), t.diag, n * 8, hipMemcpyDeviceToHost, st));
    if (rows_nn && !sink.loss_sent)
        HIP_CHECK(hipMemcpyAsync(out_loss + rows_off, t.loss + rows_off, rows_nn * 4, hipMemcpyDeviceToHost, st));
    HIP_CHECK(hipStreamSynchronize(st));
    if (rows_nn && stats) {
        hmin = rb_get<unsigned long long>(c, MS_MIN);
        if (kmode) {
            const unsigned long long dmin = *reinterpret_cast<const unsigned long long*>(c.hbox + 64 * MS_MIN + 8);
            const uint64_t unit = stats->latency_unit_ns ? stats->latency_unit_ns : 1;
            hmin = std::min<unsigned long long>(hmin == ~0ull ? ~0ull : hmin * unit, dmin);
        }
    }
    if (ikeys && rows_nn && !sink.lat_sent) {
        sink.send_keys(st, t.key, r0, r1 - r0, sink.key_unit);
        sink.lat_sent = true;
    }
    sink.finish();
    if (ikeys)
        for (size_t r = r0; r < r1; ++r) out_lat[r * n + r] = hdiag[r];
    return hmin;
}

int host_entry(srg_ctx* c, const srg_edge_list* g, const uint32_t* nodes, uint32_t num_nodes, uint64_t* out_lat,
               float* out_loss, srg_stats* stats, char* errbuf, size_t errlen, bool direct,
               uint32_t* out_key = nullptr, uint64_t* out_diag = nullptr, srg_table* const* tabs = nullptr) {
    if (const int rc = check_entry_args(c, g, nodes, num_nodes, out_lat, out_loss, direct, out_key, out_diag, errbuf, errlen))
        return rc;
    std::lock_guard<std::mutex> lk(c->mu);
    const bool keys = out_key != nullptr;
    const size_t n = num_nodes;
    const EntryPlan ep = make_entry_plan(direct, n, g->num_edges, c->comm ? c->comm->nranks : 1,
                                         c->comm ? c->comm->rank : 0, c->gather_output, c->edge_shard);
    const bool ext = (bool)c->ext_reg;
    OutputPinning reg;
    start_pinning(reg, *c, ep, ext, keys ? (unsigned char*)out_key : (unsigned char*)out_lat, keys ? 4 : 8, out_loss, n,
                  tabs);
    return guard(errbuf, errlen, [&]() {
        auto t0 = std::chrono::steady_clock::now();
        if (stats) std::memset(stats, 0, sizeof(*stats));
        HIP_CHECK(hipSetDevice(c->device));
        hipStream_t st = c->stream;
        DevGraph dg{g->num_vertices, (int)g->directed, g->num_edges, nullptr, nullptr, nullptr, nullptr,
                    nullptr, g->node_ids};
        const bool sparse = choose_sparse(*c, dg);
        const bool sim = ep.shard && std::strcmp(c->comm->kind(), "simulated") == 0;
        FwOverlap ov;
        LateLoss late;
        const Shipped sh = ship_edges(*c, g, nodes, n, direct, sparse, ep, sim, st, dg, ov, late, stats);
        if (ep.shard) exchange_slices(*c, g, dg, ep, sh, sim, st);
        const uint32_t* dn = stage_in(c->b_nodes, nodes, n, sh.hst);
        if (sh.hst != st) {
            HIP_CHECK(hipEventRecord(c->ev_c, sh.hst));
            HIP_CHECK(hipStreamWaitEvent(st, c->ev_c, 0));
        }
        DevTables dt = output_tables(*c, ep, n);
        HIP_CHECK(hipStreamSynchronize(sh.hst));
        const double ms_h2d = ms_since(t0);
        bool ikeys = wants_key_rows(*c, ep, keys, direct, n, sparse);
        KeyScope key_scope(*c, dt, keys || ikeys, n);
        HostSink sink;
        wire_sink(sink, *c, ep, ext, reg, keys ? reinterpret_cast<uint64_t*>(out_key) : out_lat, out_loss, n, ikeys);
        if (direct) {
            direct_device(*c, dg, dn, num_nodes, dt.lat, dt.loss, st);
        } else {
            compute_device(*c, dg, dn, num_nodes, dt.lat, dt.loss, st, stats, ep.early ? &sink : nullptr,
                           ov.on ? &ov : nullptr);
            if (ikeys && !sink.widen) {
                ikeys = false;
                dt.key = nullptr, dt.diag = nullptr;
            }
        }
        if (dg.late) {
            dg.late->join();
            HIP_CHECK(hipStreamSynchronize(c->loss_stream));
        }
        auto t1 = std::chrono::steady_clock::now();
        const unsigned long long hmin =
            ship_tail(*c, ep, n, keys, ikeys, dt, sink, out_lat, out_key, out_diag, out_loss, stats, st);
        if (stats) {
            stats->ms_h2d = ms_h2d;
            stats->ms_d2h = ms_since(t1);
            stats->ms_total = ms_since(t0);
            stats->ms_host_register = ext ? (sink.registered ? reg.ms : -1.0) : reg.join() ? reg.ms : -1.0;
            stats->d2h_overlapped_bytes = sink.early_bytes;
            stats->d2h_key_rows = ikeys ? 1 : 0;
            stats->ms_key_widen = sink.ms_widen;
            stats->min_latency_ns = hmin;
            if (direct) stats->path_kind = SRG_PATH_DIRECT;
        }
    });
}
```

### shadow_amd/csrc/routing.hip

```cpp
#include <hip/hip_runtime.h>
#include <hsa/hsa.h>
#include <hsa/hsa_ext_amd.h>
#include <sys/mman.h>

#include <algorithm>
#include <atomic>
#include <chrono>
#include <cmath>
#include <condition_variable>
#include <deque>
#include <cstdio>
#include <cstdlib>
#include <cstring>
#include <functional>
#include <map>
#include <memory>
#include <mutex>
#include <new>
#include <stdexcept>
#include <string>
#include <thread>
#include <vector>

#include "../../include/shadow_routing.h"
// ... 209 lines not shown
    for (size_t e = blockIdx.x * (size_t)blockDim.x + threadIdx.x; e < E; e += (size_t)gridDim.x * blockDim.x) {
        const uint32_t s = src[e];
        if (s == dst[e] && s < V) self_loss[s] = loss[e];
    }
}

template <class K>
__global__ void k_fill(K* __restrict__ p, size_t count, K v) {
    for (size_t i = blockIdx.x * (size_t)blockDim.x + threadIdx.x; i < count; i += (size_t)gridDim.x * blockDim.x)
        p[i] = v;
}

template <class K>
__device__ __forceinline__ K to_key(uint64_t l, uint64_t unit) {
    if (unit != 1) l /= unit;
    if constexpr (sizeof(K) == 4) return l >= KeyOps<K>::INF ? KeyOps<K>::INF : (uint32_t)l;
    else return (K)l;
}

template <class K>
__global__ void k_w_lat(uint64_t E, const uint32_t* __restrict__ src, const uint32_t* __restrict__ dst,
                        const uint64_t* __restrict__ lat, uint64_t unit, int directed, K* __restrict__ W, size_t ld) {
    for (size_t e = blockIdx.x * (size_t)blockDim.x + threadIdx.x; e < E; e += (size_t)gridDim.x * blockDim.x) {
        const uint32_t s = src[e], t = dst[e];
        if (s == t) continue;
        const K l = to_key<K>(lat[e], unit);
        atomicMin(&W[(size_t)s * ld + t], l);
        if (!directed) atomicMin(&W[(size_t)t * ld + s], l);
    }
}

template <class K>
__global__ void k_w_loss(uint64_t E, const uint32_t* __restrict__ src, const uint32_t* __restrict__ dst,
                         const uint64_t* __restrict__ lat, uint64_t unit, const float* __restrict__ loss, int directed,
                         const K* __restrict__ W, uint32_t* __restrict__ WL, size_t ld) {
    for (size_t e = blockIdx.x * (size_t)blockDim.x + threadIdx.x; e < E; e += (size_t)gridDim.x * blockDim.x) {
        const uint32_t s = src[e], t = dst[e];
        if (s == t) continue;
        const K l = to_key<K>(lat[e], unit);
        const uint32_t bits = __float_as_uint(loss[e] + 0.0f);
        if (W[(size_t)s * ld + t] == l) atomicMin(&WL[(size_t)s * ld + t], bits);
        if (!directed && W[(size_t)t * ld + s] == l) atomicMin(&WL[(size_t)t * ld + s], bits);
    }
}

__global__ void k_w_key(uint64_t E, const uint32_t* __restrict__ src, const uint32_t* __restrict__ dst,
                        const uint64_t* __restrict__ lat, uint64_t unit, const float* __restrict__ loss,
                        unsigned long long* __restrict__ KW, size_t ld, uint32_t V = 0xFFFFFFFFu) {
    for (size_t e = blockIdx.x * (size_t)blockDim.x + threadIdx.x; e < E; e += (size_t)gridDim.x * blockDim.x) {
        const uint32_t s = src[e], t = dst[e];
        if (s == t || s >= V || t >= V) continue;
        const uint64_t l = unit != 1 ? lat[e] / unit : lat[e];
        const unsigned long long k = ((unsigned long long)l << 32) | (loss ? __float_as_uint(loss[e] + 0.0f) : 0u);
        atomicMin(&KW[(size_t)s * ld + t], k);
    }
}

template <bool WL_ONLY = false>
__global__ void __launch_bounds__(256) k_w_split(const unsigned long long* __restrict__ KW, size_t ld, int directed,
                                                 uint32_t* __restrict__ W, uint32_t* __restrict__ WL,
                                                 uint32_t* __restrict__ D, uint32_t bi0 = 0) {
    __shared__ unsigned long long tb[64][65];
    const uint32_t bi = bi0 + blockIdx.y, bj = blockIdx.x;
    if (!directed && bj < bi) return;
    const uint32_t tx = threadIdx.x & 63, ty = threadIdx.x >> 6;
    if (!directed) {
        for (uint32_t r = ty; r < 64; r += 4) tb[r][tx] = KW[(size_t)(bj * 64 + r) * ld + bi * 64 + tx];
        __syncthreads();
    }
    for (uint32_t r = ty; r < 64; r += 4) {
        const size_t i = bi * 64 + r, j = bj * 64 + tx;
        unsigned long long k = KW[i * ld + j];
        if (!directed) k = min(k, tb[tx][r]);
        const uint32_t w = min((uint32_t)(k >> 32), KeyOps<uint32_t>::INF);
        WL[i * ld + j] = (uint32_t)k;
        if (!WL_ONLY) {
            W[i * ld + j] = w;
            D[i * ld + j] = i == j ? 0u : w;
        }
        if (!directed && bi != bj) tb[tx][r] = k;
    }
    if (!directed && bi != bj) {
        __syncthreads();
        for (uint32_t r = ty; r < 64; r += 4) {
            const size_t i = bj * 64 + r, j = bi * 64 + tx;
            const unsigned long long k = tb[r][tx];
            const uint32_t w = min((uint32_t)(k >> 32), KeyOps<uint32_t>::INF);
            WL[i * ld + j] = (uint32_t)k;
            if (!WL_ONLY) {
                W[i * ld + j] = w;
                D[i * ld + j] = w;
            }
        }
    }
}

template <class K>
__global__ void k_init_d(const K* __restrict__ W, K* __restrict__ D, size_t ld) {
    const size_t total = ld * ld;
    for (size_t i = blockIdx.x * (size_t)blockDim.x + threadIdx.x; i < total; i += (size_t)gridDim.x * blockDim.x) {
        const size_t r = i / ld, c = i - r * ld;
        D[i] = (r == c) ? (K)0 : W[i];
    }
}

template <class K>
__global__ void __launch_bounds__(256) k_certify(const K* __restrict__ D, size_t ld, const uint32_t* __restrict__ rows,
                                                 uint32_t nrows, const uint32_t* __restrict__ cols, uint32_t ncols,
                                                 K min_key, Flags* flags) {
    const uint32_t s = rows[blockIdx.x];
    const K* Dr = D + (size_t)s * ld;
    uint32_t hit = 0, bad = 0;
    constexpr uint32_t U = 8;
    for (uint32_t j0 = threadIdx.x; j0 < ncols; j0 += blockDim.x * U) {
        uint32_t cc[U];
        K d[U];
#pragma unroll
        for (uint32_t u = 0; u < U; ++u) {
            const uint32_t j = j0 + u * blockDim.x;
            cc[u] = cols[j < ncols ? j : 0];
        }
#pragma unroll
        for (uint32_t u = 0; u < U; ++u) d[u] = Dr[cc[u]];
#pragma unroll
        for (uint32_t u = 0; u < U; ++u) {
            const bool in = j0 + u * blockDim.x < ncols;
            hit |= in & (d[u] == KeyOps<K>::INF);
            bad |= in & impossible_key<K>(d[u], min_key, cc[u] == s);
        }
    }
    if (__ballot(hit) && (threadIdx.x & 63) == 0) atomicOr(&flags->inf_in_used_row, 1u);
    if (__ballot(bad) && (threadIdx.x & 63) == 0) atomicOr(&flags->impossible, 1u);
}

template <class K>
__global__ void k_loss_round(const uint32_t* __restrict__ PRED, const K* __restrict__ D, const K* __restrict__ W,
                             const uint32_t* __restrict__ WL, const uint32_t* __restrict__ nodes, uint32_t n,
                             uint32_t V, size_t ld, const float* __restrict__ Lin, float* __restrict__ Lout,
                             Flags* flags) {
    const size_t total = (size_t)n * V;
    uint32_t changed = 0;
    for (size_t i = blockIdx.x * (size_t)blockDim.x + threadIdx.x; i < total; i += (size_t)gridDim.x * blockDim.x) {
        const size_t r = i / V, t = i - r * V;
        const uint32_t s = nodes[r];
        const uint32_t p = PRED[r * ld + t];
        const float* Lrow = Lin + r * ld;
        float v;
        if (t == s) {
            v = 0.0f;
        } else if (p == PRED_NONE) {
            v = 1.0f;
        } else if (p != PRED_MULTI) {
            const float pl = __uint_as_float(WL[(size_t)p * ld + t]);
            v = fold_loss(Lrow[p], __fsub_rn(1.0f, pl));
        } else {
            const K dst_st = D[(size_t)s * ld + t];
            const K* Ds = D + (size_t)s * ld;
            v = 1.0f;
            for (uint32_t u = 0; u < V; ++u) {
                if (KeyOps<K>::add(Ds[u], W[(size_t)u * ld + t]) != dst_st) continue;
                const float pl = __uint_as_float(WL[(size_t)u * ld + t]);
                const float c = fold_loss(Lrow[u], __fsub_rn(1.0f, pl));
                v = c < v ? c : v;
            }
        }
        Lout[r * ld + t] = v;
        changed |= (v != Lrow[t]);
    }
    if (changed) atomicOr(&flags->changed, 1u);
}

template <class K>
__global__ void __launch_bounds__(256) k_wrap_edges(uint64_t E, const uint32_t* __restrict__ src,
                                                    const uint32_t* __restrict__ dst, const uint64_t* __restrict__ lat,
                                                    int directed, const K* __restrict__ D, size_t ld,
                                                    const uint32_t* __restrict__ rows, uint64_t unit, int inf_known,
                                                    Flags* flags) {
    const K* Ds = D + (size_t)rows[blockIdx.y] * ld;
    uint32_t wrap = 0, winf = 0;
    for (size_t e = blockIdx.x * (size_t)blockDim.x + threadIdx.x; e < E; e += (size_t)gridDim.x * blockDim.x) {
        const uint32_t s = src[e], t = dst[e];
        if (s == t) continue;
        const uint64_t w = lat[e];
        for (int dir = 0; dir < (directed ? 1 : 2); ++dir) {
            const uint32_t u = dir ? t : s, v = dir ? s : t;
            const K du = Ds[u], dv = Ds[v];
            if (du == KeyOps<K>::INF) {
                winf |= !inf_known;
                continue;
            }
            if (dv < du) continue;
            const unsigned __int128 sum = (unsigned __int128)du * unit + w;
            wrap |= (uint32_t)(sum >> 64) != 0;
        }
    }
    if (__ballot(wrap) && (threadIdx.x & 63) == 0) atomicOr(&flags->wrap, 1u);
    if (__ballot(winf) && (threadIdx.x & 63) == 0) atomicOr(&flags->wrap_inf, 1u);
}

__global__ void __launch_bounds__(256) k_count_multi(const uint32_t* __restrict__ PRED, uint32_t n, uint32_t V,
                                                     size_t ld, unsigned long long* out, uint32_t stride = 1) {
    const uint32_t* row = PRED + (size_t)blockIdx.x * ld * stride;
    unsigned long long c = 0;
    for (uint32_t t = threadIdx.x; t < V; t += blockDim.x) c += row[(size_t)t * stride] == PRED_MULTI;
    if (c) atomicAdd(out, c);
}

template <class K>
__global__ void __launch_bounds__(256) k_extract(const K* __restrict__ D, const float* __restrict__ L, size_t ld,
                                                 const uint32_t* __restrict__ snodes, uint32_t nloc,
                                                 const uint32_t* __restrict__ cols, uint32_t ncols,
                                                 const uint32_t* __restrict__ rowpos,
                                                 const uint64_t* __restrict__ self_lat, const float* __restrict__ self_loss,
                                                 uint64_t* __restrict__ out_lat, float* __restrict__ out_loss, Flags* flags,
                                                 int mode, uint64_t unit, uint32_t* __restrict__ out_key = nullptr,
                                                 uint64_t* __restrict__ out_diag = nullptr) {
    const uint32_t a = blockIdx.x;
    const uint32_t s = snodes[a], p = rowpos[a];
    const K* Ds = D + (size_t)s * ld;
    const float* La = L ? L + (size_t)a * ld : nullptr;
    uint64_t* ol = out_lat + (size_t)p * ncols;
    uint32_t* ok = out_key ? out_key + (size_t)p * ncols : nullptr;
    float* os = out_loss + (size_t)p * ncols;
    uint32_t unreach = 0;
    constexpr uint32_t U = 4;
    for (uint32_t b0 = threadIdx.x; b0 < ncols; b0 += blockDim.x * U) {
        uint32_t tt[U];
        K d[U];
        float l[U];
#pragma unroll
        for (uint32_t u = 0; u < U; ++u) {
            const uint32_t b = b0 + u * blockDim.x;
            tt[u] = cols[b < ncols ? b : 0];
        }
#pragma unroll
        for (uint32_t u = 0; u < U; ++u) {
            if (mode & 1) d[u] = Ds[tt[u]];
            if (mode & 2) l[u] = La[tt[u]];
        }
#pragma unroll
        for (uint32_t u = 0; u < U; ++u) {
            const uint32_t b = b0 + u * blockDim.x;
            if (b >= ncols) break;
            if (p == b) {
                if (mode & 1) {
                    if (ok) {
                        ok[b] = 0xFFFFFFFFu;
                        out_diag[p] = self_lat[s];
                    } else {
                        ol[b] = self_lat[s];
                    }
                }
                if (mode & 2) os[b] = self_loss[s];
            } else {
                if (mode & 1) {
                    unreach |= d[u] == KeyOps<K>::INF;
                    if (ok) ok[b] = (uint32_t)d[u];
                    else ol[b] = (uint64_t)d[u] * unit;
                }
                if (mode & 2) os[b] = l[u];
            }
        }
    }
    if (__ballot(unreach) && (threadIdx.x & 63) == 0) atomicOr(&flags->unreachable_used_pair, 1u);
}

template <class K>
__global__ void __launch_bounds__(256) k_extract_ident(const K* __restrict__ D, size_t ld, const uint32_t* __restrict__ snodes,
                                                       uint32_t ncols, const uint64_t* __restrict__ self_lat,
                                                       uint64_t* __restrict__ out_lat, Flags* flags, uint64_t unit,
                                                       uint32_t* __restrict__ out_key, uint64_t* __restrict__ out_diag) {
    const uint32_t s = snodes[blockIdx.x];
    const K* Ds = D + (size_t)s * ld;
    uint32_t unreach = 0;
    for (uint32_t b = threadIdx.x * 4; b < ncols; b += blockDim.x * 4) {
        K d[4];
        if constexpr (sizeof(K) == 4) {
            const uint4 v = *reinterpret_cast<const uint4*>(Ds + b);
            d[0] = v.x, d[1] = v.y, d[2] = v.z, d[3] = v.w;
        } else {
            const ulonglong2 v0 = *reinterpret_cast<const ulonglong2*>(Ds + b);
            const ulonglong2 v1 = *reinterpret_cast<const ulonglong2*>(Ds + b + 2);
            d[0] = v0.x, d[1] = v0.y, d[2] = v1.x, d[3] = v1.y;
        }
        uint64_t o[4];
        uint32_t k[4];
#pragma unroll
        for (int u = 0; u < 4; ++u) {
            const bool diag = b + u == s;
            unreach |= !diag && d[u] == KeyOps<K>::INF;
            k[u] = diag ? 0xFFFFFFFFu : (uint32_t)d[u];
            o[u] = diag ? self_lat[s] : (uint64_t)d[u] * unit;
        }
        if (out_key) {
            *reinterpret_cast<uint4*>(out_key + (size_t)s * ncols + b) = make_uint4(k[0], k[1], k[2], k[3]);
            if (b <= s && s < b + 4) out_diag[s] = self_lat[s];
        } else {
            uint64_t* ol = out_lat + (size_t)s * ncols + b;
            *reinterpret_cast<ulonglong2*>(ol) = make_ulonglong2(o[0], o[1]);
            *reinterpret_cast<ulonglong2*>(ol + 2) = make_ulonglong2(o[2], o[3]);
        }
    }
    if (__ballot(unreach) && (threadIdx.x & 63) == 0) atomicOr(&flags->unreachable_used_pair, 1u);
}

__global__ void k_min_u64(const uint64_t* __restrict__ a, size_t count, unsigned long long* out) {
    unsigned long long m = ~0ull;
    for (size_t i = blockIdx.x * (size_t)blockDim.x + threadIdx.x; i < count; i += (size_t)gridDim.x * blockDim.x)
        m = a[i] < m ? a[i] : m;
    for (int off = 32; off > 0; off >>= 1) {
        const unsigned long long o = __shfl_down(m, off, 64);
        m = o < m ? o : m;
    }
    if ((threadIdx.x & 63) == 0 && m != ~0ull) atomicMin(out, m);
}

__global__ void k_min_u32(const uint32_t* __restrict__ a, size_t count, unsigned long long* out) {
    uint32_t m = 0xFFFFFFFFu;
    for (size_t i = blockIdx.x * (size_t)blockDim.x + threadIdx.x; i < count; i += (size_t)gridDim.x * blockDim.x)
        m = a[i] < m ? a[i] : m;
    for (int off = 32; off > 0; off >>= 1) {
        const uint32_t o = __shfl_down(m, off, 64);
        m = o < m ? o : m;
    }
    if ((threadIdx.x & 63) == 0 && m != 0xFFFFFFFFu) atomicMin(out, (unsigned long long)m);
}

__global__ void k_positions(const uint32_t* __restrict__ nodes, uint32_t n, int32_t* __restrict__ pos) {
    for (size_t i = blockIdx.x * (size_t)blockDim.x + threadIdx.x; i < n; i += (size_t)gridDim.x * blockDim.x)
        pos[nodes[i]] = (int32_t)i;
}

__global__ void k_direct(uint64_t E, const uint32_t* __restrict__ src, const uint32_t* __restrict__ dst,
                         const uint64_t* __restrict__ lat, const float* __restrict__ loss, int directed,
                         const int32_t* __restrict__ pos, uint32_t n, uint32_t* __restrict__ cnt,
                         uint64_t* __restrict__ out_lat, float* __restrict__ out_loss) {
    for (size_t e = blockIdx.x * (size_t)blockDim.x + threadIdx.x; e < E; e += (size_t)gridDim.x * blockDim.x) {
        const int32_t ps = pos[src[e]], pt = pos[dst[e]];
        if (ps < 0 || pt < 0) continue;
        size_t k = (size_t)ps * n + pt;
        if (atomicAdd(&cnt[k], 1u) == 0) {
            out_lat[k] = lat[e];
            out_loss[k] = loss[e];
        }
        if (!directed && ps != pt) {
            k = (size_t)pt * n + ps;
            if (atomicAdd(&cnt[k], 1u) == 0) {
                out_lat[k] = lat[e];
                out_loss[k] = loss[e];
            }
        }
    }
}

__global__ void k_direct_check(const uint32_t* __restrict__ cnt, uint32_t n, Flags* flags) {
    const size_t total = (size_t)n * n;
    unsigned long long first = ~0ull;
    for (size_t i = blockIdx.x * (size_t)blockDim.x + threadIdx.x; i < total; i += (size_t)gridDim.x * blockDim.x)
        if (cnt[i] != 1 && i < first) first = i;
    if (first != ~0ull) atomicMin(&flags->first_bad, first);
}

double ms_since(std::chrono::steady_clock::time_point t0) {
    return std::chrono::duration<double, std::milli>(std::chrono::steady_clock::now() - t0).count();
}

}

struct SdmaAgents {
    bool ok = false;
    hsa_agent_t gpu{}, cpu{};
    uint32_t engine = 0;
    void init(int device) {
        if (hsa_init() != HSA_STATUS_SUCCESS) return;
        int bus = -1, dev = -1, dom = -1;
        if (hipDeviceGetAttribute(&bus, hipDeviceAttributePciBusId, device) != hipSuccess ||
            hipDeviceGetAttribute(&dev, hipDeviceAttributePciDeviceId, device) != hipSuccess ||
            hipDeviceGetAttribute(&dom, hipDeviceAttributePciDomainID, device) != hipSuccess)
            return;
        struct Q {
            int bus, dev, dom;
            hsa_agent_t gpu{}, cpu{};
            bool found = false, have_cpu = false;
        } q{bus, dev, dom};
        hsa_iterate_agents(
            [](hsa_agent_t a, void* p) -> hsa_status_t {
                Q& q = *static_cast<Q*>(p);
                hsa_device_type_t t;
                if (hsa_agent_get_info(a, HSA_AGENT_INFO_DEVICE, &t) != HSA_STATUS_SUCCESS) return HSA_STATUS_SUCCESS;
                if (t == HSA_DEVICE_TYPE_CPU && !q.have_cpu) {
                    q.cpu = a;
                    q.have_cpu = true;
                } else if (t == HSA_DEVICE_TYPE_GPU && !q.found) {
                    uint32_t bdf = 0, dom = 0;
                    if (hsa_agent_get_info(a, (hsa_agent_info_t)HSA_AMD_AGENT_INFO_BDFID, &bdf) == HSA_STATUS_SUCCESS &&
                        hsa_agent_get_info(a, (hsa_agent_info_t)HSA_AMD_AGENT_INFO_DOMAIN, &dom) == HSA_STATUS_SUCCESS &&
                        (int)(bdf >> 8) == q.bus && (int)((bdf >> 3) & 31) == q.dev && (int)dom == q.dom) {
                        q.gpu = a;
                        q.found = true;
                    }
                }
                return HSA_STATUS_SUCCESS;
            },
            &q);
        if (!q.found || !q.have_cpu) return;
        uint32_t mask = 0;
        if (hsa_amd_memory_copy_engine_status(q.cpu, q.gpu, &mask) != HSA_STATUS_SUCCESS || !mask) return;
        gpu = q.gpu;
        cpu = q.cpu;
        engine = mask & (~mask + 1);
        ok = true;
    }
};

struct TablePool;
struct srg_table {
    std::shared_ptr<TablePool> pool;
    void* p = nullptr;
    size_t cap = 0;
    void* view = nullptr;
    bool registered = false;
};
struct TablePool {
    std::mutex mu;
    std::vector<srg_table*> idle;
    size_t idle_bytes = 0;
    size_t limit = ~(size_t)0;
    size_t max_idle = 2;
    bool open = true;
    static void destroy(srg_table* t);
    void trim_locked(size_t keep) {
        while ((idle_bytes > keep || (max_idle && idle.size() > max_idle)) && !idle.empty()) {
            srg_table* t = idle.front();
            idle.erase(idle.begin());
            idle_bytes -= t->cap;
            destroy(t);
        }
    }
    void close() {
        std::lock_guard<std::mutex> lk(mu);
        open = false;
        trim_locked(0);
    }
};
void TablePool::destroy(srg_table* t) {
    if (t->registered) (void)hipHostUnregister(t->p);
    if (t->p) munmap(t->p, t->cap);
    delete t;
}

struct srg_ctx {
    int device = 0;
    double sparse_threshold = 0.35;
    bool profiling = false;
    bool gather_output = true;
    int algorithm = SRG_ALGO_AUTO;
    bool sparse_locality = true;
    int sparse_delta_div = 1;
    bool sparse_global_bitmaps = false;
    int fw_tile = 0;
    bool fw_symmetric = true;
    int d2h_mode = 1;
    DevBuf b_DST2;
    SdmaAgents sdma;
    int h2d_codec = 1;
    HostPool* pool = nullptr;
    void* h_ring = nullptr;
    size_t h_ring_bytes = 0;
    Event ev_ring[3];
    DevBuf b_n16s, b_n16d, b_n32l;
    DevBuf b_exc;
    std::vector<std::vector<uint32_t>> codec_ex;
    std::vector<uint32_t> slice_exc;
    DevBuf b_xexc;
    int late_loss = 1;
    hipStream_t loss_stream = nullptr;
    Event ev_ledges, ev_lin, ev_ldone, ev_wlate;
    void* h_lring = nullptr;
    Event ev_lring[3];
    int edge_shard = -1;
    const uint32_t* sim_edges = nullptr;
    size_t sim_E = 0;
    int scan_groups = 0;
    int loss_chunks = 0;
    srg::Comm* comm = nullptr;
    std::function<bool(void** views, double* ms)> ext_reg;
    std::vector<Event> prof_events;
    hipStream_t stream = nullptr;
    hipStream_t aux_stream = nullptr;
    hipStream_t comm_stream = nullptr;
    hipStream_t d2h_stream = nullptr;
    Event ev_a, ev_b, ev_c, ev_d, ev_e;
    std::mutex mu;
    DevBuf b_src, b_dst, b_lat, b_loss, b_nodes, b_olat, b_oloss;
    DevBuf b_W, b_WL, b_D, b_PRED, b_PRED2, b_L0, b_L1, b_mark, b_selfcnt, b_selflat, b_selfloss;
    DevBuf b_stats, b_flags, b_multi, b_pos, b_cnt;
    DevBuf b_ecnt, b_eoff, b_indeg, b_cscoff, b_cscfill, b_entkey, b_entw, b_entb, b_grpe, b_cscent, b_DST,
        b_scantmp, b_ess, b_rlen;
    DevBuf b_lnodes, b_lpos, b_red, b_outoff, b_outdst;
    DevBuf b_cflags, b_tiles, b_tslot;
    uint32_t* fw_timeout = nullptr;
    unsigned char* hbox = nullptr;
    uint32_t* sig[2] = {nullptr, nullptr};
    uint32_t sig_val[2] = {0, 0};
    bool hop_values = false;
    unsigned long long hop_bound_ticks = 200000000ull;
    Event ev_fwreset;
    Event ev_dst;
    int fw_line_split = 0;
    int fw_step = -1;
    DevBuf b_xlb, b_xflags;
    uint32_t xepoch = 0;
    std::vector<Event> ev_ov;
    uint32_t* kout_key = nullptr;
    uint64_t* kout_diag = nullptr;
    DevBuf b_odiag;
    int fw_overlap = 1;
    int fw_xcd_order = 1;
    int scan_mirror = 1;
    int scan_mirrored = 0;
    int loss_kind = 0;
    int scan_mirror_cap = 0;
    DevBuf b_tri;
    int test_fault = 0;
    std::shared_ptr<TablePool> tpool = std::make_shared<TablePool>();
    double ms_create_runtime = 0, ms_create_lib = 0;
    DevBuf b_ek0, b_ek1, b_eh0, b_eh1, b_ei0, b_ei1, b_ehist, b_eoffs, b_ered;
    DevBuf b_rt_off, b_rt_cur, b_rt_ce, b_rt_cu, b_rt_cl, b_rt_cp, b_rt_self, b_rt_state, b_rt_hops, b_rt_offs, b_rt_idx, b_rt_perm,
        b_rt_keys, b_rt_tmp, b_rt_pairs, b_rt_nsel;
    DevBuf b_rtt_pe, b_rtt_pv, b_rtt_hops, b_rtt_scr, b_rtt_rowmax, b_rtt_rownnz, b_rtt_active, b_rtt_nsel;
    int route_tree_rows = 0;
    ~srg_ctx() {
        delete comm;
        for (uint32_t* p : sig)
            if (p) (void)hipFree(p);
        if (h_lring) (void)hipHostFree(h_lring);
        if (hbox) (void)hipHostFree(hbox);
        for (hipStream_t s : {aux_stream, comm_stream, d2h_stream, stream})
            if (s) (void)hipStreamDestroy(s);
        delete pool;
        if (h_ring) (void)hipHostFree(h_ring);
        tpool->close();
    }
};

namespace {

struct LateLoss {
    hipStream_t ls = nullptr;
    std::thread th;
    hipEvent_t ev_in = nullptr;
    hipEvent_t ev_done = nullptr;
    bool joined = false, applied = false;
    std::string err;
    srg::Comm* comm = nullptr;
    std::vector<size_t> offs, lens;
    void join() {
        if (!joined) {
            if (th.joinable()) th.join();
            joined = true;
        }
        if (!err.empty()) fail(SRG_ERR_HIP, "loss H2D: " + err);
    }
    ~LateLoss() {
        if (th.joinable()) th.join();
        if (ls) (void)hipStreamSynchronize(ls);
    }
};

struct DevGraph {
    uint32_t V;
    int directed;
    uint64_t E;
    const uint32_t* src;
    const uint32_t* dst;
    const uint64_t* lat;
    const float* loss;
    const uint32_t* ids_dev;
    const uint32_t* ids_host;
    LateLoss* late = nullptr;
};

void loss_arrive(const DevGraph& g, float* self_loss, hipStream_t s) {
    LateLoss* L = g.late;
    if (!L) return;
    L->join();
    if (!L->applied) {
        HIP_CHECK(hipStreamWaitEvent(s, L->ev_in, 0));
        if (L->comm) L->comm->allgatherv(const_cast<float*>(g.loss), L->offs.data(), L->lens.data(), s);
        if (g.E) k_self_loss<<<grid_for(g.E), kThreads, 0, s>>>(g.E, g.src, g.dst, g.loss, g.V, self_loss);
        HIP_CHECK(hipGetLastError());
        HIP_CHECK(hipEventRecord(L->ev_done, s));
        L->applied = true;
    } else {
        HIP_CHECK(hipStreamWaitEvent(s, L->ev_done, 0));
    }
}

uint32_t node_gml_id(const DevGraph& g, uint32_t v, hipStream_t st) {
    if (g.ids_host) return g.ids_host[v];
    if (!g.ids_dev) return v;
    uint32_t id = v;
    HIP_CHECK(hipMemcpyAsync(&id, g.ids_dev + v, 4, hipMemcpyDeviceToHost, st));
    HIP_CHECK(hipStreamSynchronize(st));
    return id;
}

void ensure_prof_events(srg_ctx& c, size_t n) {
    while (c.prof_events.size() < n) {
        c.prof_events.emplace_back();
        c.prof_events.back().create_timed();
    }
}

template <class F>
void set_lds(F func, size_t bytes) {
    static_assert(sizeof(F) > 0, "");
    if (bytes > 65536)
        HIP_CHECK(hipFuncSetAttribute(reinterpret_cast<const void*>(func),
                                      hipFuncAttributeMaxDynamicSharedMemorySize, (int)bytes));
}

constexpr int kMailSlots = 64;
template <class T>
void rb_async(srg_ctx& c, int slot, const T* dev, hipStream_t st) {
    static_assert(sizeof(T) <= 64, "mailbox slot");
    HIP_CHECK(hipMemcpyAsync(c.hbox + 64 * slot, dev, sizeof(T), hipMemcpyDeviceToHost, st));
}
template <class T>
T rb_get(const srg_ctx& c, int slot) {
    T v;
    std::memcpy(&v, c.hbox + 64 * slot, sizeof(T));
    return v;
}
enum MailSlot { MS_EDGESTATS, MS_FLAGS, MS_TIMEOUT, MS_REDUCE, MS_TAIL0, MS_TAIL1, MS_NMULTI, MS_CHANGED, MS_MIN, MS_REDUCE2, MS_MIRROR };

struct Prelude {
    EdgeStats es;
    uint32_t* selfcnt;
    uint64_t* selflat;
    float* selfloss;
    Flags* flags;
    std::vector<uint32_t> nodes_h;
    bool ident = false;
    bool range_risk = false;
    bool wrap_risk = false;
    uint64_t unit = 1;
    unsigned long long max_key = 0;
};

Prelude prelude(srg_ctx& c, const DevGraph& g, const uint32_t* nodes, uint32_t n, hipStream_t st,
                bool check_selfloops) {
    Prelude P{};
    const uint32_t V = g.V;
    uint32_t* mark = (uint32_t*)c.b_mark.get((size_t)V * 4);
    P.selfcnt = (uint32_t*)c.b_selfcnt.get((size_t)V * 4);
    P.selflat = (uint64_t*)c.b_selflat.get((size_t)V * 8);
    P.selfloss = (float*)c.b_selfloss.get((size_t)V * 4);
    EdgeStats* es = (EdgeStats*)c.b_stats.get(sizeof(EdgeStats));
    P.flags = (Flags*)c.b_flags.get(sizeof(Flags));
    HIP_CHECK(hipMemsetAsync(mark, 0, (size_t)V * 4, st));
    HIP_CHECK(hipMemsetAsync(P.selfcnt, 0, (size_t)V * 4, st));
    HIP_CHECK(hipMemsetAsync(es, 0, sizeof(EdgeStats), st));
    HIP_CHECK(hipMemsetAsync(P.flags, 0, sizeof(Flags), st));
    if (n) k_check_nodes<<<grid_for(n), kThreads, 0, st>>>(nodes, n, V, mark, P.flags);
    if (g.E) {
        k_edge_scan<<<grid_for(g.E), kThreads, 0, st>>>(g.E, g.src, g.dst, g.lat, g.late ? nullptr : g.loss, V, P.selfcnt,
                                                       P.selflat, P.selfloss, es);
        k_lat_gcd<<<grid_for(g.E / 4, 1024), kThreads, 0, st>>>(g.E, g.src, g.dst, g.lat, &es->unit);
    }
    HIP_CHECK(hipGetLastError());
    Flags fl;
    P.nodes_h.resize(n);
    rb_async(c, MS_EDGESTATS, es, st);
    rb_async(c, MS_FLAGS, P.flags, st);
    if (n) HIP_CHECK(hipMemcpyAsync(P.nodes_h.data(), nodes, (size_t)n * 4, hipMemcpyDeviceToHost, st));
    HIP_CHECK(hipStreamSynchronize(st));
    P.es = rb_get<EdgeStats>(c, MS_EDGESTATS);
    fl = rb_get<Flags>(c, MS_FLAGS);
    P.ident = n == V;
    for (uint32_t i = 0; i < n && P.ident; ++i) P.ident = P.nodes_h[i] == i;
    if (P.es.bad_endpoint) fail(SRG_ERR_ARG, "edge endpoint out of range (>= num_vertices)");
    if (fl.bad_node & 1) fail(SRG_ERR_ARG, "node index out of range (>= num_vertices)");
    if (fl.bad_node & 2) fail(SRG_ERR_ARG, "duplicate node index in `nodes`");
    if (check_selfloops) {
        if (P.es.lat_overflow)
            fail(SRG_ERR_LATENCY_RANGE, "The resulting value is outside of the bounds [0, 18446744073709551615]");
        std::vector<uint32_t> cnt(V);
        HIP_CHECK(hipMemcpyAsync(cnt.data(), P.selfcnt, (size_t)V * 4, hipMemcpyDeviceToHost, st));
        HIP_CHECK(hipStreamSynchronize(st));
        for (uint32_t i = 0; i < n; ++i) {
            const uint32_t v = P.nodes_h[i];
            if (cnt[v] == 1) continue;
            const uint32_t id = node_gml_id(g, v, st);
            if (cnt[v] == 0)
                fail(SRG_ERR_NO_EDGE, "No edge connecting node " + std::to_string(id) + " to " + std::to_string(id));
            fail(SRG_ERR_MULTI_EDGE,
                 "More than one edge connecting node " + std::to_string(id) + " to " + std::to_string(id));
        }
    }
    return P;
}

struct Timer {
    hipStream_t st;
    std::chrono::steady_clock::time_point t0;
    explicit Timer(hipStream_t s) : st(s) { t0 = std::chrono::steady_clock::now(); }
    double lap() {
        HIP_CHECK(hipStreamSynchronize(st));
        double m = ms_since(t0);
        t0 = std::chrono::steady_clock::now();
        return m;
    }
};

struct HostSink {
    uint64_t* lat = nullptr;
    float* loss = nullptr;
    void* lat_view = nullptr;
    void* loss_view = nullptr;
    int mode = 1;
    const SdmaAgents* sdma = nullptr;
    int device = 0;
    size_t n = 0;
    hipStream_t cs = nullptr;
    hipEvent_t ev = nullptr;
    std::function<bool()> ready;
    bool checked = false, registered = false;
    bool lat_sent = false, loss_sent = false;
    uint64_t early_bytes = 0;
    struct Job {
        hipEvent_t ev;
        void* dst;
        const void* src;
        size_t bytes;
    };
    std::thread worker;
    std::mutex mu;
    std::condition_variable cv;
    std::deque<Job> jobs;
    bool closing = false;
    std::string err;
    std::vector<hsa_signal_t> sigs;
    std::vector<hipEvent_t> evs;
    bool widen = false;
    HostPool* pool = nullptr;
    unsigned char* ring = nullptr;
    size_t ring_slot = 0;
    std::thread kthread;
    std::string kerr;
    double ms_widen = 0;
    uint64_t key_unit = 1;
    void send_keys(hipStream_t st, const uint32_t* dkey, size_t row0, size_t rows, uint64_t unit) {
        if (!rows || !n) return;
        hipEvent_t e;
        HIP_CHECK(hipEventCreateWithFlags(&e, hipEventDisableTiming));
        evs.push_back(e);
        HIP_CHECK(hipEventRecord(e, st));
        kthread = std::thread([this, e, dkey, row0, rows, unit]() { key_worker(e, dkey, row0, rows, unit); });
        early_bytes += rows * n * 4;
    }
    void key_worker(hipEvent_t ev, const uint32_t* dkey, size_t row0, size_t rows, uint64_t unit) {
        (void)hipSetDevice(device);
        if (hipEventSynchronize(ev) != hipSuccess) {
            kerr = "hipEventSynchronize failed before the key D2H";
            return;
        }
        const auto t0 = std::chrono::steady_clock::now();
        constexpr int NS = 3;
        const size_t rpc = std::max<size_t>(1, ring_slot / (n * 4));
        const size_t nch = (rows + rpc - 1) / rpc;
        hsa_signal_t sg[NS];
        int made = 0;
        for (; made < NS; ++made)
            if (hsa_signal_create(0, 0, nullptr, &sg[made]) != HSA_STATUS_SUCCESS) break;
        if (made < NS) {
            for (int i = 0; i < made; ++i) hsa_signal_destroy(sg[i]);
            kerr = "hsa_signal_create failed";
            return;
        }
        auto issue = [&](size_t ci) {
            const size_t r = ci * rpc, cnt = std::min(rpc, rows - r);
            hsa_signal_store_relaxed(sg[ci % NS], 1);
            if (hsa_amd_memory_async_copy_on_engine(ring + (ci % NS) * ring_slot, sdma->cpu, dkey + (row0 + r) * n, sdma->gpu,
                                                    cnt * n * 4, 0, nullptr, sg[ci % NS],
                                                    (hsa_amd_sdma_engine_id_t)sdma->engine, true) != HSA_STATUS_SUCCESS) {
                kerr = "hsa_amd_memory_async_copy_on_engine failed (keys)";
                hsa_signal_store_relaxed(sg[ci % NS], 0);
                return false;
            }
            return true;
        };
        bool ok = true;
        for (size_t ci = 0; ci < std::min<size_t>(NS, nch) && ok; ++ci) ok = issue(ci);
        for (size_t ci = 0; ci < nch && ok; ++ci) {
            hsa_signal_wait_scacquire(sg[ci % NS], HSA_SIGNAL_CONDITION_LT, 1, UINT64_MAX, HSA_WAIT_STATE_BLOCKED);
            const size_t r = ci * rpc, cnt = std::min(rpc, rows - r);
            const uint32_t* kb = reinterpret_cast<const uint32_t*>(ring + (ci % NS) * ring_slot);
            uint64_t* ob = lat + (row0 + r) * n;
            const size_t tot = cnt * n;
            pool->run([&](int w, int nw) {
                const size_t a = tot * w / nw, z = tot * (w + 1) / nw;
                if (unit == 1)
                    for (size_t i = a; i < z; ++i) ob[i] = kb[i];
                else
                    for (size_t i = a; i < z; ++i) ob[i] = (uint64_t)kb[i] * unit;
            });
            if (ci + NS < nch) ok = issue(ci + NS);
        }
        for (int i = 0; i < NS; ++i) {
            hsa_signal_wait_scacquire(sg[i], HSA_SIGNAL_CONDITION_LT, 1, UINT64_MAX, HSA_WAIT_STATE_BLOCKED);
            hsa_signal_destroy(sg[i]);
        }
        ms_widen = ms_since(t0);
    }
    bool ok() {
        if (!checked) {
            registered = ready && ready();
            checked = true;
        }
        return registered;
    }
    void work() {
        (void)hipSetDevice(device);
        for (;;) {
            Job j;
            {
                std::unique_lock<std::mutex> lk(mu);
                cv.wait(lk, [&] { return closing || !jobs.empty(); });
                if (jobs.empty()) return;
                j = jobs.front();
                jobs.pop_front();
            }
            if (!err.empty()) continue;
            if (hipEventSynchronize(j.ev) != hipSuccess) {
                err = "hipEventSynchronize failed before a D2H copy";
                continue;
            }
            hsa_signal_t sg;
            if (hsa_signal_create(1, 0, nullptr, &sg) != HSA_STATUS_SUCCESS) {
                err = "hsa_signal_create failed";
                continue;
            }
            sigs.push_back(sg);
            if (hsa_amd_memory_async_copy_on_engine(j.dst, sdma->cpu, j.src, sdma->gpu, j.bytes, 0, nullptr, sg,
                                                    (hsa_amd_sdma_engine_id_t)sdma->engine, true) != HSA_STATUS_SUCCESS)
                err = "hsa_amd_memory_async_copy_on_engine failed";
        }
    }
    void send_rows(hipStream_t st, const void* dev, void* host, size_t row0, size_t rows, size_t elem) {
        const size_t off = row0 * n * elem, bytes = rows * n * elem;
        if (!bytes) return;
        const unsigned char* src = (const unsigned char*)dev + off;
        void* view = host == (void*)lat ? lat_view : host == (void*)loss ? loss_view : nullptr;
        if (mode == 1 && sdma && sdma->ok) {
            hipEvent_t e;
            HIP_CHECK(hipEventCreateWithFlags(&e, hipEventDisableTiming));
            evs.push_back(e);
            HIP_CHECK(hipEventRecord(e, st));
            {
                std::lock_guard<std::mutex> lk(mu);
                jobs.push_back(Job{e, (unsigned char*)(view ? view : host) + off, src, bytes});
            }
            if (!worker.joinable()) worker = std::thread([this] { work(); });
            cv.notify_one();
            early_bytes += bytes;
            return;
        }
        HIP_CHECK(hipEventRecord(ev, st));
        HIP_CHECK(hipStreamWaitEvent(cs, ev, 0));
        HIP_CHECK(hipMemcpyAsync((unsigned char*)host + off, src, bytes, hipMemcpyDeviceToHost, cs));
        early_bytes += bytes;
    }
    void finish() {
        drain();
        if (!kerr.empty()) fail(SRG_ERR_HIP, "key D2H: " + kerr);
        HIP_CHECK(hipStreamSynchronize(cs));
        if (!err.empty()) fail(SRG_ERR_HIP, "D2H copy: " + err);
    }
    ~HostSink() { drain(); }

   private:
    void drain() {
        if (kthread.joinable()) kthread.join();
        if (worker.joinable()) {
            {
                std::lock_guard<std::mutex> lk(mu);
                closing = true;
            }
            cv.notify_one();
            worker.join();
        }
        for (hsa_signal_t sg : sigs) {
            hsa_signal_wait_scacquire(sg, HSA_SIGNAL_CONDITION_LT, 1, UINT64_MAX, HSA_WAIT_STATE_BLOCKED);
            hsa_signal_destroy(sg);
        }
        sigs.clear();
        for (hipEvent_t e : evs) (void)hipEventDestroy(e);
        evs.clear();
    }
};

void advise_huge(void* p, size_t bytes) {
    const uintptr_t a = ((uintptr_t)p + ((size_t)2 << 20) - 1) & ~(uintptr_t)(((size_t)2 << 20) - 1);
    const uintptr_t e = ((uintptr_t)p + bytes) & ~(uintptr_t)(((size_t)2 << 20) - 1);
    if (e > a) (void)madvise((void*)a, e - a, MADV_HUGEPAGE);
}

void prefault(void* p, size_t bytes, int nthreads) {
    if (!p || bytes < ((size_t)64 << 20)) return;
    const size_t pg = 4096, per = (bytes / nthreads + pg - 1) / pg * pg;
    std::vector<std::thread> th;
    for (int t = 0; t < nthreads; ++t) {
        const size_t a = (size_t)t * per, e = std::min(bytes, a + per);
        if (a >= e) break;
        th.emplace_back([=]() {
            volatile unsigned char* b = (volatile unsigned char*)p;
            for (size_t o = a; o < e; o += pg) b[o] = 0;
        });
    }
    for (auto& x : th) x.join();
}

std::mutex g_dev_mu;
std::map<int, int> g_dev_ctx;

__global__ void k_hop_set(uint32_t* sig, uint32_t v) {
    if (threadIdx.x == 0) __hip_atomic_store(sig, v, __ATOMIC_RELAXED, __HIP_MEMORY_SCOPE_SYSTEM);
}
__global__ void k_hop_wait(const uint32_t* sig, uint32_t v, uint32_t* timeout, unsigned long long bound_ticks) {
    if (threadIdx.x != 0) return;
    const unsigned long long t0 = wall_clock64();
    while (__hip_atomic_load(sig, __ATOMIC_RELAXED, __HIP_MEMORY_SCOPE_SYSTEM) - v > 0x7FFFFFFFu) {
        if (__hip_atomic_load(timeout, __ATOMIC_RELAXED, __HIP_MEMORY_SCOPE_AGENT)) return;
        if (wall_clock64() - t0 > bound_ticks) {
            uint32_t zero = 0;
            __hip_atomic_compare_exchange_strong(timeout, &zero, 2u, __ATOMIC_RELAXED, __ATOMIC_RELAXED,
                                                 __HIP_MEMORY_SCOPE_AGENT);
// ... 720 lines not shown
    P.range_risk = bound >= ((unsigned __int128)1 << 62);
    P.wrap_risk = (unsigned __int128)P.es.max_lat * g.V >= ((unsigned __int128)1 << 64);
    const int G = c.comm ? c.comm->nranks : 1, rk = c.comm ? c.comm->rank : 0;
    if (choose_sparse(c, g) && !P.wrap_risk) {
        loss_arrive(g, P.selfloss, st);
        if (P.max_key < 0xFFFFFFFFull && run_sparse(c, g, nodes, n, out_lat, out_loss, st, P, stats)) return;
        run_sparse(c, g, nodes, n, out_lat, out_loss, st, P, stats, true);
        return;
    }
    if (pre) {
        if (run_dense<uint32_t, FwOverlap::T>(c, g, ov->pl, nodes, n, out_lat, out_loss, st, P, stats, sink, ov)) {
            if (stats) stats->fw_overlap_kept = 1;
            return;
        }
        P.unit = unit;
        P.max_key = P.es.max_lat / P.unit;
        if (stats) stats->latency_unit_ns = P.unit;
        P.range_risk = (unsigned __int128)P.max_key * (g.V > 1 ? g.V - 1 : 1) >= ((unsigned __int128)1 << 62);
    }
    if ((!pre || P.unit > 1) && P.max_key < 0xFFFFFFFFull) {
        const int tile = c.fw_tile ? c.fw_tile : 128;
        if (tile == 64) {
            Plan pl = make_plan(G, rk, g.V, 64, P.nodes_h);
            if (run_dense<uint32_t, 64>(c, g, pl, nodes, n, out_lat, out_loss, st, P, stats, sink)) return;
        } else {
            Plan pl = make_plan(G, rk, g.V, 128, P.nodes_h);
            if (run_dense<uint32_t, 128>(c, g, pl, nodes, n, out_lat, out_loss, st, P, stats, sink)) return;
        }
    }
    Plan pl = make_plan(G, rk, g.V, 64, P.nodes_h);
    run_dense<uint64_t, 64>(c, g, pl, nodes, n, out_lat, out_loss, st, P, stats, sink);
}

void direct_device(srg_ctx& c, const DevGraph& g, const uint32_t* nodes, uint32_t n, uint64_t* out_lat,
                   float* out_loss, hipStream_t st) {
    Prelude P = prelude(c, g, nodes, n, st, false);
    loss_arrive(g, P.selfloss, st);
    if (n == 0) return;
    int32_t* pos = (int32_t*)c.b_pos.get((size_t)g.V * 4);
    uint32_t* cnt = (uint32_t*)c.b_cnt.get((size_t)n * n * 4);
    HIP_CHECK(hipMemsetAsync(pos, 0xFF, (size_t)g.V * 4, st));
    HIP_CHECK(hipMemsetAsync(cnt, 0, (size_t)n * n * 4, st));
    HIP_CHECK(hipMemsetAsync(&P.flags->first_bad, 0xFF, 8, st));
    k_positions<<<grid_for(n), kThreads, 0, st>>>(nodes, n, pos);
    if (g.E)
        k_direct<<<grid_for(g.E), kThreads, 0, st>>>(g.E, g.src, g.dst, g.lat, g.loss, g.directed, pos, n, cnt,
                                                     out_lat, out_loss);
    k_direct_check<<<grid_for((size_t)n * n), kThreads, 0, st>>>(cnt, n, P.flags);
    HIP_CHECK(hipGetLastError());
    Flags fl;
    HIP_CHECK(hipMemcpyAsync(&fl, P.flags, sizeof(Flags), hipMemcpyDeviceToHost, st));
    HIP_CHECK(hipStreamSynchronize(st));
    if (fl.first_bad != ~0ull) {
        const size_t k = fl.first_bad;
        uint32_t cv = 0, a = 0, b = 0;
        HIP_CHECK(hipMemcpy(&cv, cnt + k, 4, hipMemcpyDeviceToHost));
        HIP_CHECK(hipMemcpy(&a, nodes + k / n, 4, hipMemcpyDeviceToHost));
        HIP_CHECK(hipMemcpy(&b, nodes + k % n, 4, hipMemcpyDeviceToHost));
        const std::string ia = std::to_string(node_gml_id(g, a, st)), ib = std::to_string(node_gml_id(g, b, st));
        if (cv == 0) fail(SRG_ERR_NO_EDGE, "No edge connecting node " + ia + " to " + ib);
        fail(SRG_ERR_MULTI_EDGE, "More than one edge connecting node " + ia + " to " + ib);
    }
    if (P.es.lat_overflow || P.es.max_lat == UINT64_MAX) {
        std::vector<uint64_t> lat((size_t)n * n);
        HIP_CHECK(hipMemcpy(lat.data(), out_lat, lat.size() * 8, hipMemcpyDeviceToHost));
        for (uint64_t v : lat)
            if (v == UINT64_MAX)
                fail(SRG_ERR_LATENCY_RANGE, "The resulting value is outside of the bounds [0, 18446744073709551615]");
    }
}

#include "events_run.hip.h"
#include "inbound_run.hip.h"
#include "h2d_codec.hip.h"

int guard(char* errbuf, size_t errlen, const std::function<void()>& body) {
    try {
        body();
        if (errbuf && errlen) errbuf[0] = 0;
        return SRG_OK;
    } catch (const Failure& f) {
        set_err(errbuf, errlen, f.msg);
        return f.code;
    } catch (const srg::CommError& e) {
        set_err(errbuf, errlen, std::string("collective: ") + e.what());
        return SRG_ERR_RCCL;
    } catch (const std::bad_alloc&) {
        set_err(errbuf, errlen, "out of host memory");
        return SRG_ERR_OOM;
    } catch (const std::exception& e) {
        set_err(errbuf, errlen, std::string("internal error: ") + e.what());
        return SRG_ERR_INTERNAL;
    } catch (...) {
        set_err(errbuf, errlen, "internal error");
        return SRG_ERR_INTERNAL;
    }
}

template <class F>
int device_call(srg_ctx* ctx, void* hip_stream, double* ms_total, char* errbuf, size_t errlen, F&& body) {
    std::lock_guard<std::mutex> lk(ctx->mu);
    auto t0 = std::chrono::steady_clock::now();
    const int rc = guard(errbuf, errlen, [&]() {
        HIP_CHECK(hipSetDevice(ctx->device));
        body(hip_stream ? (hipStream_t)hip_stream : ctx->stream);
    });
    if (ms_total) *ms_total = ms_since(t0);
    return rc;
}

#include "host_entry.hip.h"
}

extern "C" {

__global__ void k_warm(uint32_t* p) {
    if (threadIdx.x == 0 && blockIdx.x == 0) p[0] = 0;
}

void warm_context(srg_ctx& c) {
    ensure_pool(c);
    ensure_rings(c);
    uint32_t* d = (uint32_t*)c.b_red.get(128);
    const hipStream_t ss[4] = {c.stream, c.aux_stream, c.comm_stream, c.d2h_stream};
    for (hipStream_t s : ss) k_warm<<<1, 64, 0, s>>>(d);
    HIP_CHECK(hipGetLastError());
    HIP_CHECK(hipMemcpyAsync(d, c.h_ring, 64, hipMemcpyHostToDevice, c.comm_stream));
    HIP_CHECK(hipMemcpyAsync(c.h_lring, d + 16, 64, hipMemcpyDeviceToHost, c.d2h_stream));
    for (hipStream_t s : ss) HIP_CHECK(hipStreamSynchronize(s));
    if (c.sdma.ok) {
        hsa_signal_t sg;
        if (hsa_signal_create(1, 0, nullptr, &sg) == HSA_STATUS_SUCCESS) {
            if (hsa_amd_memory_async_copy_on_engine(c.h_ring, c.sdma.cpu, d, c.sdma.gpu, 64, 0, nullptr, sg,
                                                    (hsa_amd_sdma_engine_id_t)c.sdma.engine, true) == HSA_STATUS_SUCCESS)
                hsa_signal_wait_scacquire(sg, HSA_SIGNAL_CONDITION_LT, 1, UINT64_MAX, HSA_WAIT_STATE_BLOCKED);
            hsa_signal_destroy(sg);
        }
    }
}

int srg_create(srg_ctx** out, int device, char* errbuf, size_t errlen) {
    if (!out) {
        set_err(errbuf, errlen, "null argument");
        return SRG_ERR_ARG;
    }
    *out = nullptr;
    srg_ctx* c = nullptr;
    int rc = guard(errbuf, errlen, [&]() {
        const bool dbg = srg_env::debug_create();
        auto tc = std::chrono::steady_clock::now();
        auto lap = [&](const char* what) {
            if (dbg) std::fprintf(stderr, "srg_create: %-28s %7.2f ms\n", what, ms_since(tc));
            tc = std::chrono::steady_clock::now();
        };
        const auto tcreate = std::chrono::steady_clock::now();
        int count = 0;
        hipError_t e = hipGetDeviceCount(&count);
        lap("hipGetDeviceCount");
        if (e != hipSuccess || count == 0)
            fail(SRG_ERR_HIP, std::string("no HIP device available (") + hipGetErrorString(e) +
                                  "); the routing builder has no CPU fallback");
        if (device < 0 || device >= count) fail(SRG_ERR_ARG, "device index out of range");
        c = new srg_ctx();
        c->device = device;
        HIP_CHECK(hipSetDevice(device));
        HIP_CHECK(hipFree(nullptr));
        lap("hipSetDevice");
        HIP_CHECK(hipStreamCreateWithFlags(&c->stream, hipStreamNonBlocking));
        lap("stream main");
        c->ms_create_runtime = ms_since(tcreate);
        const auto tlib = std::chrono::steady_clock::now();
        int prio_lo = 0, prio_hi = 0;
        HIP_CHECK(hipDeviceGetStreamPriorityRange(&prio_lo, &prio_hi));
        HIP_CHECK(hipStreamCreateWithPriority(&c->aux_stream, hipStreamNonBlocking, prio_hi));
        HIP_CHECK(hipStreamCreateWithFlags(&c->comm_stream, hipStreamNonBlocking));
        HIP_CHECK(hipStreamCreateWithFlags(&c->d2h_stream, hipStreamNonBlocking));
        lap("streams aux, comm, d2h");
        HIP_CHECK(hipHostMalloc((void**)&c->hbox, 64 * kMailSlots, hipHostMallocDefault));
        lap("mailbox");
        c->sdma.init(device);
        lap("sdma agents");
        c->loss_stream = c->d2h_stream;
        for (Event* e : {&c->ev_a, &c->ev_b, &c->ev_c, &c->ev_d, &c->ev_e, &c->ev_ledges, &c->ev_wlate, &c->ev_fwreset,
                         &c->ev_dst})
            e->create();
        int wv = 0;
        if (hipDeviceGetAttribute(&wv, hipDeviceAttributeCanUseStreamWaitValue, device) == hipSuccess && wv) {
            for (uint32_t*& p : c->sig) HIP_CHECK(hipExtMallocWithFlags((void**)&p, 8, hipMallocSignalMemory));
            HIP_CHECK(hipStreamWriteValue32(c->stream, c->sig[0], 0, 0));
            HIP_CHECK(hipStreamWriteValue32(c->stream, c->sig[1], 0, 0));
            HIP_CHECK(hipStreamSynchronize(c->stream));
        }
        lap("events, signals");
        if (!srg_env::create_warm_off()) {
            warm_context(*c);
            lap("warm-up (module, rings, copies)");
        }
        c->ms_create_lib = ms_since(tlib);
        std::lock_guard<std::mutex> lk(g_dev_mu);
        ++g_dev_ctx[device];
    });
    if (rc != SRG_OK) {
        delete c;
        return rc;
    }
    *out = c;
    return SRG_OK;
}

int srg_set_option(srg_ctx* ctx, int option, double value) {
    if (!ctx) return SRG_ERR_ARG;
    std::lock_guard<std::mutex> lk(ctx->mu);
    switch (option) {
        case SRG_OPT_PROFILING:
            ctx->profiling = value != 0.0;
            return SRG_OK;
        case SRG_OPT_SPARSE_THRESHOLD:
            if (!(value >= 0.0)) return SRG_ERR_ARG;
            ctx->sparse_threshold = value;
            return SRG_OK;
        case SRG_OPT_GATHER_OUTPUT:
            ctx->gather_output = value != 0.0;
            return SRG_OK;
        case SRG_OPT_SIMULATE_RANK: {
            const int v = (int)value;
            delete ctx->comm;
            ctx->comm = nullptr;
            ctx->sim_edges = nullptr;
            if (v > 0) {
                const int nr = v / 1000, rk = v % 1000;
                if (nr < 1 || rk >= nr) return SRG_ERR_ARG;
                ctx->comm = srg::null_create(nr, rk);
            }
            return SRG_OK;
        }
        case SRG_OPT_FW_TILE:
            if (value != 0 && value != 64 && value != 128) return SRG_ERR_ARG;
            ctx->fw_tile = (int)value;
            return SRG_OK;
        case SRG_OPT_SPARSE_LOCALITY:
            ctx->sparse_locality = value != 0.0;
            return SRG_OK;
        case SRG_OPT_SPARSE_DELTA_DIV:
            if (!(value >= 0.0 && value <= 1e6)) return SRG_ERR_ARG;
            ctx->sparse_delta_div = (int)value;
            return SRG_OK;
        case SRG_OPT_SPARSE_GLOBAL_BITMAPS:
            ctx->sparse_global_bitmaps = value != 0.0;
            return SRG_OK;
        case SRG_OPT_FW_SYMMETRIC:
            ctx->fw_symmetric = value != 0.0;
            return SRG_OK;
        case SRG_OPT_LATE_LOSS:
            if (value != 0 && value != 1) return SRG_ERR_ARG;
            ctx->late_loss = (int)value;
            return SRG_OK;
        case SRG_OPT_EDGE_SHARD:
            if (value != 0 && value != 1 && value != -1) return SRG_ERR_ARG;
            ctx->edge_shard = (int)value;
            return SRG_OK;
        case SRG_OPT_H2D_CODEC:
            if (value != 0 && value != 1) return SRG_ERR_ARG;
            ctx->h2d_codec = (int)value;
            return SRG_OK;
        case SRG_OPT_SCAN_GROUPS:
            if (value < 0 || value > 1024) return SRG_ERR_ARG;
            ctx->scan_groups = (int)value;
            return SRG_OK;
        case SRG_OPT_LOSS_CHUNKS:
            if (value < 0 || value > 1024) return SRG_ERR_ARG;
            ctx->loss_chunks = (int)value;
            return SRG_OK;
        case SRG_OPT_D2H_MODE:
            if (value != 0 && value != 1) return SRG_ERR_ARG;
            ctx->d2h_mode = (int)value;
            return SRG_OK;
        case SRG_OPT_FW_LINE_SPLIT:
            if (value != 0 && value != 1 && value != 2 && value != 4) return SRG_ERR_ARG;
            ctx->fw_line_split = (int)value;
            return SRG_OK;
        case SRG_OPT_FW_STEP:
            if (value != 0 && value != 2 && value != -1) return SRG_ERR_ARG;
            ctx->fw_step = (int)value;
            return SRG_OK;
        case SRG_OPT_FW_OVERLAP:
            if (value != 0 && value != 1) return SRG_ERR_ARG;
            ctx->fw_overlap = (int)value;
            return SRG_OK;
        case SRG_OPT_TEST_FAULT:
            if (value != 0 && value != 1 && value != 2) return SRG_ERR_ARG;
#ifndef SRG_TEST_HOOKS
            if (value != 0) return SRG_ERR_ARG;
#endif
            ctx->test_fault = (int)value;
            return SRG_OK;
        case SRG_OPT_FW_XCD_ORDER:
            if (value != 0 && value != 1) return SRG_ERR_ARG;
            ctx->fw_xcd_order = (int)value;
            return SRG_OK;
        case SRG_OPT_SCAN_MIRROR:
            if (value != 0 && value != 1) return SRG_ERR_ARG;
            ctx->scan_mirror = (int)value;
            return SRG_OK;
        case SRG_OPT_SCAN_MIRROR_CAP:
            if (!(value >= 0 && value <= 1073741824.0)) return SRG_ERR_ARG;
            ctx->scan_mirror_cap = (int)value;
            return SRG_OK;
        case SRG_OPT_ROUTE_TREE_ROWS:
            if (!(value >= 0 && value <= 1073741824.0)) return SRG_ERR_ARG;
            ctx->route_tree_rows = (int)value;
            return SRG_OK;
        case SRG_OPT_TABLE_POOL_BYTES: {
            if (!(value >= 0.0 && value <= 1e15)) return SRG_ERR_ARG;
            std::lock_guard<std::mutex> pl(ctx->tpool->mu);
            ctx->tpool->limit = (size_t)value;
            ctx->tpool->max_idle = 0;
            ctx->tpool->trim_locked(ctx->tpool->limit);
            return SRG_OK;
        }
        case SRG_OPT_ALGORITHM:
            if (value != SRG_ALGO_AUTO && value != SRG_ALGO_DENSE && value != SRG_ALGO_SPARSE) return SRG_ERR_ARG;
            ctx->algorithm = (int)value;
            return SRG_OK;
        default:
            return SRG_ERR_ARG;
    }
}

int srg_get_option(srg_ctx* ctx, int option, double* value) {
    if (!ctx || !value) return SRG_ERR_ARG;
    std::lock_guard<std::mutex> lk(ctx->mu);
    switch (option) {
        case SRG_OPT_PROFILING: *value = ctx->profiling; break;
        case SRG_OPT_SPARSE_THRESHOLD: *value = ctx->sparse_threshold; break;
        case SRG_OPT_GATHER_OUTPUT: *value = ctx->gather_output; break;
        case SRG_OPT_ALGORITHM: *value = ctx->algorithm; break;
        case SRG_OPT_SPARSE_LOCALITY: *value = ctx->sparse_locality; break;
        case SRG_OPT_FW_TILE: *value = ctx->fw_tile; break;
        case SRG_OPT_SPARSE_DELTA_DIV: *value = ctx->sparse_delta_div; break;
        case SRG_OPT_SPARSE_GLOBAL_BITMAPS: *value = ctx->sparse_global_bitmaps; break;
        case SRG_OPT_FW_SYMMETRIC: *value = ctx->fw_symmetric; break;
        case SRG_OPT_D2H_MODE: *value = ctx->d2h_mode; break;
        case SRG_OPT_LOSS_CHUNKS: *value = ctx->loss_chunks; break;
        case SRG_OPT_SCAN_GROUPS: *value = ctx->scan_groups; break;
        case SRG_OPT_H2D_CODEC: *value = ctx->h2d_codec; break;
        case SRG_OPT_EDGE_SHARD: *value = ctx->edge_shard; break;
        case SRG_OPT_LATE_LOSS: *value = ctx->late_loss; break;
        case SRG_OPT_FW_LINE_SPLIT: *value = ctx->fw_line_split; break;
        case SRG_OPT_FW_STEP: *value = ctx->fw_step; break;
        case SRG_OPT_FW_OVERLAP: *value = ctx->fw_overlap; break;
        case SRG_OPT_TEST_FAULT: *value = ctx->test_fault; break;
        case SRG_OPT_TABLE_POOL_BYTES: {
            std::lock_guard<std::mutex> pl(ctx->tpool->mu);
            *value = (double)ctx->tpool->limit;
            break;
        }
        case SRG_OPT_TABLE_POOL_IDLE_BYTES: {
            std::lock_guard<std::mutex> pl(ctx->tpool->mu);
            *value = (double)ctx->tpool->idle_bytes;
            break;
        }
        case SRG_OPT_CREATE_MS_RUNTIME: *value = ctx->ms_create_runtime; break;
        case SRG_OPT_FW_XCD_ORDER: *value = ctx->fw_xcd_order; break;
        case SRG_OPT_CREATE_MS_LIBRARY: *value = ctx->ms_create_lib; break;
        case SRG_OPT_SCAN_MIRROR: *value = ctx->scan_mirror; break;
        case SRG_OPT_SCAN_MIRRORED: *value = ctx->scan_mirrored; break;
        case SRG_OPT_SCAN_MIRROR_CAP: *value = ctx->scan_mirror_cap; break;
        case SRG_OPT_LOSS_KIND: *value = ctx->loss_kind; break;
        case SRG_OPT_ROUTE_TREE_ROWS: *value = ctx->route_tree_rows; break;
        default: return SRG_ERR_ARG;
    }
    return SRG_OK;
}

void srg_destroy(srg_ctx* ctx) {
    if (!ctx) return;
    (void)hipSetDevice(ctx->device);
    {
        std::lock_guard<std::mutex> lk(g_dev_mu);
        --g_dev_ctx[ctx->device];
    }
    delete ctx;
}

int srg_internal_compute_table(srg_ctx* ctx, const srg_edge_list* graph, const uint32_t* nodes, uint32_t num_nodes,
                               int shortest, uint64_t* out_lat, uint32_t* out_key, uint64_t* out_diag, float* out_loss,
                               uint64_t* unit_ns, srg_table* tab_lat, srg_table* tab_loss, srg_stats* stats,
                               char* errbuf, size_t errlen) {
    srg_stats local{};
    srg_stats* st = stats ? stats : &local;
    srg_table* tabs[2] = {tab_lat, tab_loss};
    const int rc = host_entry(ctx, graph, nodes, num_nodes, out_key ? nullptr : out_lat, out_loss, st, errbuf, errlen,
                              !shortest, out_key, out_diag, tabs);
    if (unit_ns) *unit_ns = out_key && st->latency_unit_ns ? st->latency_unit_ns : 1;
    return rc;
}

uint32_t srg_internal_scan_group_cut_tri(uint32_t q, uint32_t ng, uint32_t nblocks) {
    return scan_group_cut_tri(q, ng, nblocks);
}

void srg_internal_loss_limits(uint32_t out[4]) {
    out[0] = LM_T;
    out[1] = LM_E;
    out[2] = MIRROR_STEPS;
    out[3] = LOSS_ROWS_MAX_V;
}

srg_table* srg_internal_table_get(srg_ctx* ctx, size_t bytes, void** host) {
    if (!ctx || !host) return nullptr;
    *host = nullptr;
    constexpr size_t HP = (size_t)2 << 20;
    const size_t cap = (std::max<size_t>(bytes, 1) + HP - 1) / HP * HP;
    TablePool& P = *ctx->tpool;
    {
        std::lock_guard<std::mutex> lk(P.mu);
        size_t best = SIZE_MAX;
        for (size_t i = 0; i < P.idle.size(); ++i)
            if (P.idle[i]->cap >= cap && P.idle[i]->cap <= 2 * cap && (best == SIZE_MAX || P.idle[i]->cap < P.idle[best]->cap))
                best = i;
        if (best != SIZE_MAX) {
            srg_table* t = P.idle[best];
            P.idle.erase(P.idle.begin() + best);
            P.idle_bytes -= t->cap;
            *host = t->p;
            return t;
        }
    }
    void* m = mmap(nullptr, cap + HP, PROT_READ | PROT_WRITE, MAP_PRIVATE | MAP_ANONYMOUS | MAP_NORESERVE, -1, 0);
    if (m == MAP_FAILED) return nullptr;
    const uintptr_t a = ((uintptr_t)m + HP - 1) / HP * HP;
    if (a > (uintptr_t)m) munmap(m, a - (uintptr_t)m);
    if ((uintptr_t)m + cap + HP > a + cap) munmap((void*)(a + cap), (uintptr_t)m + cap + HP - (a + cap));
    srg_table* t = new (std::nothrow) srg_table();
    if (!t) {
        munmap((void*)a, cap);
        return nullptr;
    }
    t->pool = ctx->tpool;
    t->p = (void*)a;
    t->cap = cap;
    *host = t->p;
    return t;
}

void srg_internal_table_put(srg_table* t) {
    if (!t) return;
    std::shared_ptr<TablePool> P = t->pool;
    std::lock_guard<std::mutex> lk(P->mu);
    if (P->open && t->cap <= P->limit) {
        P->idle.push_back(t);
        P->idle_bytes += t->cap;
        P->trim_locked(P->limit);
    } else {
        TablePool::destroy(t);
    }
}

int srg_compute_shortest_paths(srg_ctx* ctx, const srg_edge_list* graph, const uint32_t* nodes, uint32_t num_nodes,
                               uint64_t* out_latency_ns, float* out_packet_loss, srg_stats* stats, char* errbuf,
                               size_t errlen) {
    return host_entry(ctx, graph, nodes, num_nodes, out_latency_ns, out_packet_loss, stats, errbuf, errlen, false);
}

int srg_get_direct_paths(srg_ctx* ctx, const srg_edge_list* graph, const uint32_t* nodes, uint32_t num_nodes,
                         uint64_t* out_latency_ns, float* out_packet_loss, srg_stats* stats, char* errbuf,
                         size_t errlen) {
    return host_entry(ctx, graph, nodes, num_nodes, out_latency_ns, out_packet_loss, stats, errbuf, errlen, true);
}

int srg_compute_shortest_paths_device(srg_ctx* ctx, const srg_edge_list* g, const uint32_t* nodes_dev,
                                      uint32_t num_nodes, uint64_t* out_lat_dev, float* out_loss_dev,
                                      void* hip_stream, srg_stats* stats, char* errbuf, size_t errlen) {
    if (!ctx || !g || (num_nodes && (!nodes_dev || !out_lat_dev || !out_loss_dev))) {
        set_err(errbuf, errlen, "null argument");
        return SRG_ERR_ARG;
    }
    std::lock_guard<std::mutex> lk(ctx->mu);
    return guard(errbuf, errlen, [&]() {
        auto t0 = std::chrono::steady_clock::now();
        if (stats) std::memset(stats, 0, sizeof(*stats));
        HIP_CHECK(hipSetDevice(ctx->device));
        hipStream_t st = hip_stream ? (hipStream_t)hip_stream : ctx->stream;
        DevGraph dg{g->num_vertices, (int)g->directed, g->num_edges, g->src, g->dst, g->latency_ns,
                    g->packet_loss, g->node_ids, nullptr};
        compute_device(*ctx, dg, nodes_dev, num_nodes, out_lat_dev, out_loss_dev, st, stats);
        HIP_CHECK(hipStreamSynchronize(st));
        if (stats) stats->ms_total = ms_since(t0);
    });
}

int srg_comm_unique_id(unsigned char id[SRG_UNIQUE_ID_BYTES], char* errbuf, size_t errlen) {
    if (!id) {
        set_err(errbuf, errlen, "null argument");
        return SRG_ERR_ARG;
    }
    return guard(errbuf, errlen, [&]() {
        const std::string e = srg::rccl_unique_id(id);
        if (!e.empty()) fail(SRG_ERR_RCCL, e);
    });
}

int srg_comm_init(srg_ctx* ctx, int nranks, int rank, const unsigned char id[SRG_UNIQUE_ID_BYTES], char* errbuf,
                  size_t errlen) {
    if (!ctx || !id || nranks < 1 || rank < 0 || rank >= nranks) {
        set_err(errbuf, errlen, "bad argument");
        return SRG_ERR_ARG;
    }
    std::lock_guard<std::mutex> lk(ctx->mu);
    return guard(errbuf, errlen, [&]() {
        srg::Comm* cm = nullptr;
        const std::string e = srg::rccl_create(nranks, rank, id, ctx->device, &cm);
        if (!e.empty()) fail(SRG_ERR_RCCL, e);
        delete ctx->comm;
        ctx->comm = cm;
    });
}

int srg_local_group_create(int nranks, srg_local_group** out) {
    if (!out || nranks < 1) return SRG_ERR_ARG;
    *out = reinterpret_cast<srg_local_group*>(srg::local_group_create(nranks));
    return SRG_OK;
}

void srg_local_group_release(srg_local_group* g) { srg::local_group_release(reinterpret_cast<srg::LocalGroup*>(g)); }

int srg_comm_init_local(srg_ctx* ctx, srg_local_group* g, int rank, char* errbuf, size_t errlen) {
    if (!ctx || !g) {
        set_err(errbuf, errlen, "null argument");
        return SRG_ERR_ARG;
    }
    std::lock_guard<std::mutex> lk(ctx->mu);
    return guard(errbuf, errlen, [&]() {
        srg::Comm* cm = nullptr;
        const std::string e = srg::local_create(reinterpret_cast<srg::LocalGroup*>(g), rank, ctx->device, &cm);
        if (!e.empty()) fail(SRG_ERR_ARG, e);
        delete ctx->comm;
        ctx->comm = cm;
    });
}

int srg_comm_size(srg_ctx* ctx, int* nranks, int* rank) {
    if (!ctx || !nranks || !rank) return SRG_ERR_ARG;
    *nranks = ctx->comm ? ctx->comm->nranks : 1;
    *rank = ctx->comm ? ctx->comm->rank : 0;
    return SRG_OK;
}

struct srg_multi {
    std::vector<srg_ctx*> ranks;
    std::vector<int> devices;
    srg::LocalGroup* group = nullptr;
    std::mutex mu;
    ~srg_multi() {
        for (srg_ctx* c : ranks) srg_destroy(c);
        if (group) srg::local_group_release(group);
    }
};

int srg_multi_create(srg_multi** out, const int* devices, int num_devices, char* errbuf, size_t errlen) {
    if (!out || !devices || num_devices < 1) {
        set_err(errbuf, errlen, "bad argument");
        return SRG_ERR_ARG;
    }
    *out = nullptr;
    auto* m = new srg_multi();
    m->devices.assign(devices, devices + num_devices);
    m->group = srg::local_group_create(num_devices);
    for (int r = 0; r < num_devices; ++r) {
        srg_ctx* c = nullptr;
        int rc = srg_create(&c, devices[r], errbuf, errlen);
        if (rc == SRG_OK) {
            m->ranks.push_back(c);
            if (num_devices > 1) rc = srg_comm_init_local(c, reinterpret_cast<srg_local_group*>(m->group), r, errbuf, errlen);
        }
        if (rc != SRG_OK) {
            delete m;
            return rc;
        }
    }
    *out = m;
    return SRG_OK;
}

void srg_multi_destroy(srg_multi* m) { delete m; }

int srg_multi_size(const srg_multi* m) { return m ? (int)m->ranks.size() : 0; }

int srg_multi_set_option(srg_multi* m, int option, double value) {
    if (!m) return SRG_ERR_ARG;
    if (option == SRG_OPT_GATHER_OUTPUT || option == SRG_OPT_SIMULATE_RANK) return SRG_ERR_ARG;
    std::vector<double> old(m->ranks.size(), 0.0);
    for (size_t r = 0; r < m->ranks.size(); ++r)
        if (srg_get_option(m->ranks[r], option, &old[r]) != SRG_OK) return SRG_ERR_ARG;
    for (size_t r = 0; r < m->ranks.size(); ++r) {
        const int rc = srg_set_option(m->ranks[r], option, value);
        if (rc != SRG_OK) {
            for (size_t q = 0; q < r; ++q) (void)srg_set_option(m->ranks[q], option, old[q]);
            return rc;
        }
    }
    return SRG_OK;
}

int srg_multi_compute_shortest_paths(srg_multi* m, const srg_edge_list* graph, const uint32_t* nodes,
                                     uint32_t num_nodes, uint64_t* out_latency_ns, float* out_packet_loss,
                                     srg_stats* stats, char* errbuf, size_t errlen) {
    if (!m || !graph || (num_nodes && (!nodes || !out_latency_ns || !out_packet_loss))) {
        set_err(errbuf, errlen, "null argument");
        return SRG_ERR_ARG;
    }
    std::lock_guard<std::mutex> lk(m->mu);
    const int G = (int)m->ranks.size();
    if (G == 1) return srg_compute_shortest_paths(m->ranks[0], graph, nodes, num_nodes, out_latency_ns, out_packet_loss,
                                                  stats, errbuf, errlen);
    const auto t0 = std::chrono::steady_clock::now();
    const size_t nn = (size_t)num_nodes * num_nodes;
    struct Reg {
        std::mutex mu;
        std::thread th;
        bool done = false, ok = false;
        double ms = 0;
        void* p[2] = {nullptr, nullptr};
        size_t b[2] = {0, 0};
        bool wait() {
            std::lock_guard<std::mutex> l(mu);
            if (!done) {
                if (th.joinable()) th.join();
                done = true;
            }
            return ok;
        }
    } reg;
    reg.p[0] = out_latency_ns;
    reg.b[0] = nn * 8;
    reg.p[1] = out_packet_loss;
    reg.b[1] = nn * 4;
    const bool big = nn * 12 >= ((size_t)64 << 20);
    if (big) {
        const int dev0 = m->devices[0];
        reg.th = std::thread([&reg, dev0]() {
            const auto ts = std::chrono::steady_clock::now();
            if (hipSetDevice(dev0) != hipSuccess) return;
            const unsigned fl = hipHostRegisterPortable | hipHostRegisterMapped;
            advise_huge(reg.p[0], reg.b[0]);
            advise_huge(reg.p[1], reg.b[1]);
            if (hipHostRegister(reg.p[0], reg.b[0], fl) != hipSuccess) return;
            if (hipHostRegister(reg.p[1], reg.b[1], fl) != hipSuccess) {
                (void)hipHostUnregister(reg.p[0]);
                return;
            }
            reg.ms = ms_since(ts);
            reg.ok = true;
        });
    }
    std::vector<int> rc(G, SRG_OK);
    std::vector<std::string> msg(G);
    std::vector<srg_stats> st(G);
    std::vector<std::thread> th;
    for (int r = 0; r < G; ++r) {
        srg_ctx* c = m->ranks[r];
        c->gather_output = false;
        if (big)
            c->ext_reg = [&reg](void** views, double* ms) {
                if (!reg.wait()) return false;
                for (int i = 0; i < 2; ++i)
                    if (hipHostGetDevicePointer(&views[i], reg.p[i], 0) != hipSuccess) views[i] = nullptr;
                *ms = reg.ms;
                return true;
            };
        th.emplace_back([&, r, c]() {
// ... 350 lines not shown
```

### shadow_amd/csrc/tight_sparse.hip.h

```cpp
#pragma once
#include <hip/hip_runtime.h>
#include <stdint.h>

#include "kernels.hip.h"

namespace srg {

template <class K>
__global__ void __launch_bounds__(256) k_ess_mask(const K* __restrict__ W, const K* __restrict__ D, size_t ld,
                                                   uint32_t V, uint32_t u0, uint32_t u1, uint32_t nw64,
                                                   unsigned long long* __restrict__ ess) {
    const uint32_t lane = threadIdx.x & 63, wave = threadIdx.x >> 6;
    const uint32_t u = u0 + blockIdx.x;
    if (u >= u1) return;
    const K* Wu = W + (size_t)u * ld;
    const K* Du = D + (size_t)u * ld;
    unsigned long long* eu = ess + (size_t)u * nw64;
    if constexpr (sizeof(K) == 4) {
        for (uint32_t w0 = wave * 4; w0 < nw64; w0 += 16) {
            const uint32_t t = w0 * 64 + lane * 4;
            uint4 a = make_uint4(0u, 0u, 0u, 0u), d = make_uint4(1u, 1u, 1u, 1u);
            if (t < ld) {
                a = *reinterpret_cast<const uint4*>(Wu + t);
                d = *reinterpret_cast<const uint4*>(Du + t);
            }
            const uint32_t av[4] = {a.x, a.y, a.z, a.w}, dv[4] = {d.x, d.y, d.z, d.w};
            unsigned long long nib = 0;
#pragma unroll
            for (uint32_t j = 0; j < 4; ++j)
                nib |= (unsigned long long)(t + j < V && t + j != u && av[j] != KeyOps<K>::INF && av[j] == dv[j]) << j;
            unsigned long long v = nib << (4 * (lane & 15));
#pragma unroll
            for (int o = 1; o < 16; o <<= 1) v |= __shfl_xor(v, o, 64);
            const uint32_t w = w0 + (lane >> 4);
            if ((lane & 15) == 0 && w < nw64) eu[w] = v;
        }
    } else {
        for (uint32_t w0 = wave; w0 < nw64; w0 += 4) {
            const uint32_t t = w0 * 64 + lane;
            bool e = false;
            if (t < V && t != u) {
                const K w = Wu[t];
                e = (w != KeyOps<K>::INF) && (w == Du[t]);
            }
            const unsigned long long m = __ballot(e);
            if (lane == 0) eu[w0] = m;
        }
    }
}

template <class K>
__global__ void __launch_bounds__(256) k_build_dst(const K* __restrict__ D, size_t ld,
                                                    const uint32_t* __restrict__ nodes, uint32_t n,
                                                    K* __restrict__ DST, size_t npad) {
    __shared__ K tile[64][65];
    const uint32_t ub = blockIdx.x, rb = blockIdx.y;
    const uint32_t tx = threadIdx.x & 63, ty = threadIdx.x >> 6;
    for (uint32_t i = ty; i < 64; i += 4) {
        uint32_t r = rb * 64 + i;
        const uint32_t s = nodes[r < n ? r : n - 1];
        tile[i][tx] = D[(size_t)s * ld + ub * 64 + tx];
    }
    __syncthreads();
    for (uint32_t j = ty; j < 64; j += 4) DST[(size_t)(ub * 64 + j) * npad + rb * 64 + tx] = tile[tx][j];
}

__device__ __forceinline__ __amdgpu_buffer_rsrc_t make_rsrc(const void* base, uint32_t bytes) {
    return __builtin_amdgcn_make_buffer_rsrc(const_cast<void*>(base), (short)0, (int)bytes, 0x00027000);
}

constexpr uint32_t V5_WAVES = 8;
constexpr uint32_t V5_TW = 16;
constexpr uint32_t V5_TT = V5_WAVES * V5_TW;
constexpr uint32_t V5_UC = 64;
constexpr uint32_t V5_SB = 128;
constexpr uint32_t V5_SLACK = 256;

__global__ void __launch_bounds__(256) k_v5_count(const unsigned long long* __restrict__ ess, uint32_t V,
                                                   uint32_t nw64, uint32_t nK, uint32_t* __restrict__ cnt,
                                                   uint32_t* __restrict__ glen, uint32_t* __restrict__ indeg) {
    const uint32_t lane = threadIdx.x & 63;
    const size_t wv = (blockIdx.x * (size_t)blockDim.x + threadIdx.x) >> 6;
    if (wv >= (size_t)nw64 * nK) return;
    const uint32_t w64 = (uint32_t)(wv / nK), k = (uint32_t)(wv % nK);
    const uint32_t t = w64 * 64 + lane, b = t / V5_TT, tt = t % V5_TT;
    const uint32_t u0 = k * V5_UC, u1 = min(V, u0 + V5_UC);
    uint32_t c = 0;
    for (uint32_t u = u0; u < u1; ++u) c += (uint32_t)((ess[(size_t)u * nw64 + w64] >> lane) & 1ull);
    cnt[((size_t)b * nK + k) * V5_TT + tt] = c;
    if (c) atomicAdd(&indeg[t], c);
    uint32_t p = (c + 1) / 2;
#pragma unroll
    for (int off = 1; off < (int)V5_TW; off <<= 1) p += __shfl_xor(p, off, V5_TW);
    if ((lane % V5_TW) == 0) glen[((size_t)b * nK + k) * V5_WAVES + tt / V5_TW] = (p + 3) / 4 * 4;
}

__global__ void __launch_bounds__(256) k_v5_cscpos(const uint32_t* __restrict__ cnt, const uint32_t* __restrict__ csc_off,
                                                    uint32_t NT, uint32_t nK, uint32_t* __restrict__ pos) {
    const uint32_t t = blockIdx.x * blockDim.x + threadIdx.x;
    if (t >= NT) return;
    const uint32_t b = t / V5_TT, tt = t % V5_TT;
    uint32_t run = csc_off[t];
    for (uint32_t k = 0; k < nK; ++k) {
        const size_t i = ((size_t)b * nK + k) * V5_TT + tt;
        pos[i] = run;
        run += cnt[i];
    }
}

template <class K>
__global__ void __launch_bounds__(256) k_v5_fill(const unsigned long long* __restrict__ ess,
                                                  const K* __restrict__ W, const uint32_t* __restrict__ WL,
                                                  size_t ld, uint32_t V, uint32_t nw64, uint32_t nK,
                                                  const uint32_t* __restrict__ cnt, const uint32_t* __restrict__ goff,
                                                  const uint32_t* __restrict__ csc_pos,
                                                  uint2* __restrict__ rec, K* __restrict__ ent_w,
                                                  uint2* __restrict__ ent_ub, uint32_t* __restrict__ csc_ent) {
    const uint32_t lane = threadIdx.x & 63;
    const size_t wv = (blockIdx.x * (size_t)blockDim.x + threadIdx.x) >> 6;
    if (wv >= (size_t)nw64 * nK) return;
    const uint32_t w64 = (uint32_t)(wv / nK), k = (uint32_t)(wv % nK);
    const uint32_t t = w64 * 64 + lane, b = t / V5_TT, tt = t % V5_TT, j = tt % V5_TW;
    const uint32_t c = cnt[((size_t)b * nK + k) * V5_TT + tt];
    const uint32_t p = (c + 1) / 2;
    uint32_t incl = p;
#pragma unroll
    for (int off = 1; off < (int)V5_TW; off <<= 1) {
        const uint32_t y = __shfl_up(incl, off, V5_TW);
        if ((int)j >= off) incl += y;
    }
    const size_t g = ((size_t)b * nK + k) * V5_WAVES + tt / V5_TW;
    const uint32_t pbase = goff[g];
    size_t e = 2 * ((size_t)pbase + incl - p);
    const uint32_t u0 = k * V5_UC, u1 = min(V, u0 + V5_UC);
    uint32_t cp = csc_pos[((size_t)b * nK + k) * V5_TT + tt];
    for (uint32_t ub = u0; ub < u1; ub += 8) {
        bool on[8];
        K wv[8];
        uint32_t lv[8];
#pragma unroll
        for (uint32_t q = 0; q < 8; ++q) {
            const uint32_t u = ub + q;
            on[q] = u < u1 && ((ess[(size_t)u * nw64 + w64] >> lane) & 1ull);
            if (on[q]) {
                wv[q] = W[(size_t)u * ld + t];
                lv[q] = WL[(size_t)u * ld + t];
            }
        }
#pragma unroll
        for (uint32_t q = 0; q < 8; ++q) {
            if (!on[q]) continue;
            const uint32_t u = ub + q;
            rec[e] = make_uint2(((u - u0) * 512u) | ((e & 1) ? 0u : (j << 16)), (uint32_t)wv[q]);
            ent_w[e] = wv[q];
            ent_ub[e] = make_uint2(u, __float_as_uint(__fsub_rn(1.0f, __uint_as_float(lv[q]))));
            csc_ent[cp++] = (uint32_t)e;
            ++e;
        }
    }
    if (c & 1u) {
        rec[e] = make_uint2(0u, KeyOps<uint32_t>::INF);
        ent_w[e] = KeyOps<K>::INF;
        ent_ub[e] = make_uint2(0u, __float_as_uint(1.0f));
    }
    if (j == V5_TW - 1) {
        const uint32_t total = incl;
        for (size_t q = 2 * ((size_t)pbase + total); q < 2 * (size_t)goff[g + 1]; ++q) {
            rec[q] = make_uint2(0u, KeyOps<uint32_t>::INF);
            ent_w[q] = KeyOps<K>::INF;
            ent_ub[q] = make_uint2(0u, __float_as_uint(1.0f));
        }
    }
}

typedef uint32_t v16u_v5 __attribute__((ext_vector_type(16)));
struct alignas(64) V5Grp {
    uint32_t v[16];
};

__global__ void __launch_bounds__(512, 4) tight_v5(const uint32_t* __restrict__ DST, size_t npad, uint32_t dst_bytes,
                                                    const uint32_t* __restrict__ nodes, uint32_t n, uint32_t V,
                                                    uint32_t NT, uint32_t nbTT, uint32_t nbS, uint32_t nK, uint32_t c0,
                                                    const uint32_t* __restrict__ goff, const uint32_t* __restrict__ rec,
                                                    uint32_t* __restrict__ PRED, size_t ldp, uint32_t inf_check,
                                                    const uint32_t* __restrict__ tri) {
    __shared__ __attribute__((aligned(16))) uint32_t rows[2 * V5_UC * V5_SB];
    const uint32_t bid = blockIdx.x, xcd = bid & 7, slot = bid >> 3;
    const uint32_t blk = (slot >> 5) * 8 + xcd, nbb = (nbTT + 3) / 4;
    uint32_t tb = blk % nbb, sg = blk / nbb;
    if (tri) {
        const uint32_t d = tri[blk];
        if (d == 0xFFFFFFFFu) return;
        tb = d & 0xFFFFu;
        sg = d >> 16;
    }
    const uint32_t b = tb * 4 + (slot & 3), c = c0 + sg * 8 + ((slot >> 2) & 7);
    if (c >= nbS || b >= nbTT) return;
    if (tri && b < c) return;
    const uint32_t tid = threadIdx.x, lane = tid & 63;
    const uint32_t wave = (uint32_t)__builtin_amdgcn_readfirstlane(tid >> 6);
    const uint32_t r0 = c * V5_SB + 2 * lane;
    const __amdgpu_buffer_rsrc_t rsrc = make_rsrc(DST, dst_bytes);
    const uint32_t t0 = b * V5_TT + wave * V5_TW;
    const bool active = t0 < NT;
    v16u_v5 ndl, ndh, stl, sth;
#pragma unroll
    for (uint32_t j = 0; j < V5_TW; ++j) {
        uint32_t dl = 0, dh = 0;
        if (active) {
            const auto v = __builtin_amdgcn_raw_buffer_load_b64(rsrc, ((t0 + j) * (uint32_t)npad + r0) * 4u, 0, 0);
            dl = v[0];
            dh = v[1];
        }
        ndl[j] = 0u - dl;
        ndh[j] = 0u - dh;
        stl[j] = PRED_NONE;
        sth[j] = PRED_NONE;
    }
    const uint32_t srow = tid >> 5, scol = (tid & 31) * 4;
    uint4 sv[4];
    auto stage_load = [&](uint32_t k) {
#pragma unroll
        for (uint32_t i = 0; i < 4; ++i) {
            const uint32_t u = k * V5_UC + srow + 16 * i;
            const auto v = __builtin_amdgcn_raw_buffer_load_b128(rsrc, (u * (uint32_t)npad + c * V5_SB + scol) * 4u, 0, 0);
            sv[i] = make_uint4(v[0], v[1], v[2], v[3]);
        }
    };
    auto stage_store = [&](uint32_t buf) {
#pragma unroll
        for (uint32_t i = 0; i < 4; ++i)
            *reinterpret_cast<uint4*>(&rows[buf * (V5_UC * V5_SB) + (srow + 16 * i) * V5_SB + scol]) = sv[i];
    };
    stage_load(0);
    stage_store(0);
    __syncthreads();
    const unsigned char* lds = reinterpret_cast<const unsigned char*>(rows);
    for (uint32_t k = 0; k < nK; ++k) {
        if (k + 1 < nK) stage_load(k + 1);
        if (active) {
            const size_t q = ((size_t)b * nK + k) * V5_WAVES + wave;
            const uint32_t p0 = (uint32_t)__builtin_amdgcn_readfirstlane(goff[q]);
            const uint32_t p1 = (uint32_t)__builtin_amdgcn_readfirstlane(goff[q + 1]);
            const uint32_t vb = (k & 1u) * (V5_UC * V5_SB * 4u) + lane * 8u;
            auto group = [&](const V5Grp& cur, uint32_t p) {
                    uint2 A[8];
#pragma unroll
                    for (uint32_t i = 0; i < 4; ++i) {
                        A[2 * i] = *reinterpret_cast<const uint2*>(lds + vb + (cur.v[4 * i] & 0xFFFFu));
                        A[2 * i + 1] = *reinterpret_cast<const uint2*>(lds + vb + cur.v[4 * i + 2]);
                    }
#pragma unroll
                    for (uint32_t i = 0; i < 4; ++i) {
                        const uint32_t tl = cur.v[4 * i] >> 16;
                        const uint32_t dl = ndl[tl], dh = ndh[tl];
                        const uint32_t w0 = cur.v[4 * i + 1], w1 = cur.v[4 * i + 3];
                        const uint32_t x0l = A[2 * i].x + w0 + dl, x0h = A[2 * i].y + w0 + dh;
                        const uint32_t x1l = A[2 * i + 1].x + w1 + dl, x1h = A[2 * i + 1].y + w1 + dh;
                        const uint32_t m = min(min(x0l, x0h), min(x1l, x1h));
                        if (__builtin_expect(__ballot(m == 0) != 0, 0)) {
                            const uint32_t e0 = 2 * (p + i);
                            uint32_t sl = stl[tl], sh = sth[tl];
                            if (x0l == 0) sl = (sl == PRED_NONE) ? e0 : PRED_MULTI;
                            if (x1l == 0) sl = (sl == PRED_NONE) ? e0 + 1 : PRED_MULTI;
                            if (x0h == 0) sh = (sh == PRED_NONE) ? e0 : PRED_MULTI;
                            if (x1h == 0) sh = (sh == PRED_NONE) ? e0 + 1 : PRED_MULTI;
                            stl[tl] = sl;
                            sth[tl] = sh;
                        }
                    }
            };
            if (p0 < p1) {
                V5Grp ga = *reinterpret_cast<const V5Grp*>(rec + 4 * (size_t)p0);
                V5Grp gb = *reinterpret_cast<const V5Grp*>(rec + 4 * (size_t)(p0 + 4));
                for (uint32_t p = p0;; p += 8) {
                    group(ga, p);
                    if (p + 4 >= p1) break;
                    ga = *reinterpret_cast<const V5Grp*>(rec + 4 * (size_t)(p + 8));
                    group(gb, p + 4);
                    if (p + 8 >= p1) break;
                    gb = *reinterpret_cast<const V5Grp*>(rec + 4 * (size_t)(p + 12));
                }
            }
        }
        if (k + 1 < nK) {
            stage_store((k + 1) & 1u);
            __syncthreads();
        }
    }
    if (!active) return;
#pragma unroll
    for (uint32_t h = 0; h < 2; ++h) {
        const uint32_t r = r0 + h;
        if (r >= n) continue;
        const uint32_t s = nodes[r];
        uint32_t o[V5_TW];
#pragma unroll
        for (uint32_t j = 0; j < V5_TW; ++j) {
            const uint32_t t = t0 + j;
            const uint32_t nd = h ? ndh[j] : ndl[j];
            const uint32_t st = h ? sth[j] : stl[j];
            o[j] = (t >= V || t == s || (inf_check && nd == 0u - KeyOps<uint32_t>::INF)) ? PRED_NONE : st;
        }
        uint4* out = reinterpret_cast<uint4*>(PRED + (size_t)r * ldp + t0);
#pragma unroll
        for (uint32_t j = 0; j < V5_TW; j += 4) out[j / 4] = make_uint4(o[j], o[j + 1], o[j + 2], o[j + 3]);
    }
}

__global__ void __launch_bounds__(256) k_pred_pack(const uint32_t* __restrict__ PRED, size_t ldp, uint32_t r0,
                                                   uint32_t r1, uint32_t NT, uint32_t nbTT, uint32_t nsb,
                                                   const uint2* __restrict__ ent_ub, uint2* __restrict__ PK,
                                                   unsigned long long* __restrict__ multi, uint32_t tri) {
    const uint32_t xcd = blockIdx.x & 7, slot = blockIdx.x >> 3;
    const uint32_t b = xcd + 8 * (slot / nsb), sb = slot % nsb;
    if (b >= nbTT) return;
    if (tri && b < r0 / V5_SB + sb) return;
    const uint32_t tx = threadIdx.x & 31, ty = threadIdx.x >> 5;
    const uint32_t t = b * V5_TT + tx * 4;
    const bool tv = t < NT;
    uint32_t nm = 0;
    for (uint32_t i0 = ty; i0 < 128; i0 += 32) {
        uint32_t pv[4][4];
#pragma unroll
        for (int k = 0; k < 4; ++k) {
            const uint32_t r = r0 + sb * 128 + i0 + 8 * k;
            uint4 p = make_uint4(PRED_NONE, PRED_NONE, PRED_NONE, PRED_NONE);
            if (tv && r < r1) p = *reinterpret_cast<const uint4*>(PRED + (size_t)r * ldp + t);
            pv[k][0] = p.x;
            pv[k][1] = p.y;
            pv[k][2] = p.z;
            pv[k][3] = p.w;
        }
        uint2 q[4][4];
#pragma unroll
        for (int k = 0; k < 4; ++k)
#pragma unroll
            for (int j = 0; j < 4; ++j) {
                q[k][j] = pv[k][j] < PRED_MULTI ? ent_ub[pv[k][j]] : make_uint2(pv[k][j], 0u);
                nm += pv[k][j] == PRED_MULTI;
            }
#pragma unroll
        for (int k = 0; k < 4; ++k) {
            const uint32_t r = r0 + sb * 128 + i0 + 8 * k;
            if (!tv || r >= r1) break;
            uint4* o = reinterpret_cast<uint4*>(PK + (size_t)r * ldp + t);
            o[0] = make_uint4(q[k][0].x, q[k][0].y, q[k][1].x, q[k][1].y);
            o[1] = make_uint4(q[k][2].x, q[k][2].y, q[k][3].x, q[k][3].y);
        }
    }
    if (__ballot(nm != 0)) {
#pragma unroll
        for (int o = 32; o > 0; o >>= 1) nm += __shfl_xor(nm, o, 64);
        if ((threadIdx.x & 63) == 0) atomicAdd(multi, (unsigned long long)nm);
    }
}

constexpr uint32_t MIRROR_STEPS = 64;
__global__ void __launch_bounds__(256) k_pred_mirror(uint2* __restrict__ PK, size_t ldp, uint32_t r0, uint32_t r1,
                                                     uint32_t V, uint2* __restrict__ work, uint32_t cap,
                                                     uint32_t* __restrict__ wcnt,
                                                     unsigned long long* __restrict__ multi) {
    __shared__ uint2 tile[64][65];
    __shared__ uint32_t overflowed;
    const uint32_t tt = r0 / 64 + blockIdx.y, sc = blockIdx.x * 64;
    if (sc >= tt / 2 * V5_SB) return;
    if (threadIdx.x == 0) overflowed = wcnt[1];
    __syncthreads();
    if (overflowed) return;
    const uint32_t lane = threadIdx.x & 63, wave = threadIdx.x >> 6;
    const uint32_t t = tt * 64 + lane;
    uint32_t nm = 0;
    for (uint32_t i = 0; i < 16; ++i) {
        const uint32_t sl = wave * 16 + i, s = sc + sl, bs = s / V5_SB;
        uint2 res = make_uint2(PRED_NONE, 0u);
        if (t < r1) {
            const uint2* rs = PK + (size_t)s * ldp;
            uint32_t x = t;
            bool slow = true;
            for (uint32_t step = 0; step < MIRROR_STEPS; ++step) {
                if (x / V5_SB < bs) {
                    res = PK[(size_t)x * ldp + s];
                    slow = false;
                    break;
                }
                const uint2 e = rs[x];
                if (e.x == s) {
                    res = make_uint2(x, e.y);
                    slow = false;
                    break;
                }
                if (e.x >= V) break;
                x = e.x;
            }
            if (slow) {
                const uint32_t q = atomicAdd(&wcnt[0], 1u);
                if (q < cap) work[q] = make_uint2(t, s);
                else wcnt[1] = 1u;
            } else {
                nm += res.x == PRED_MULTI;
            }
        }
        tile[lane][sl] = res;
    }
    __syncthreads();
    const uint32_t c2 = (threadIdx.x & 31) * 2;
    for (uint32_t row = threadIdx.x >> 5; row < 64; row += 8) {
        const uint32_t tr = tt * 64 + row;
        if (tr >= r1) break;
        const uint2 a = tile[row][c2], b = tile[row][c2 + 1];
        *reinterpret_cast<uint4*>(PK + (size_t)tr * ldp + sc + c2) = make_uint4(a.x, a.y, b.x, b.y);
    }
    if (__ballot(nm != 0)) {
#pragma unroll
        for (int o = 32; o > 0; o >>= 1) nm += __shfl_xor(nm, o, 64);
        if (lane == 0) atomicAdd(multi, (unsigned long long)nm);
    }
}

template <class K>
__global__ void __launch_bounds__(256) k_mirror_slow(const uint2* __restrict__ work, const uint32_t* __restrict__ wcnt,
                                                     uint32_t cap, const K* __restrict__ DST, size_t npad,
                                                     const uint2* __restrict__ ent_ub, const K* __restrict__ ent_w,
                                                     const uint32_t* __restrict__ csc_off,
                                                     const uint32_t* __restrict__ csc_ent, uint2* __restrict__ PK,
                                                     size_t ldp, unsigned long long* __restrict__ multi) {
    const uint32_t lane = threadIdx.x & 63;
    if (wcnt[1]) return;
    const uint32_t nw = min(wcnt[0], cap), nwaves = gridDim.x * (blockDim.x >> 6);
    for (uint32_t i = blockIdx.x * (blockDim.x >> 6) + (threadIdx.x >> 6); i < nw; i += nwaves) {
        const uint2 ts = work[i];
        const uint32_t t = ts.x, s = ts.y;
        const K dst = DST[(size_t)s * npad + t];
        uint32_t cnt = 0, hit = 0;
        for (uint32_t k = csc_off[s] + lane; k < csc_off[s + 1]; k += 64) {
            const uint32_t e = csc_ent[k];
            if (KeyOps<K>::add(DST[(size_t)ent_ub[e].x * npad + t], ent_w[e]) != dst) continue;
            ++cnt;
            hit = e;
        }
#pragma unroll
        for (int o = 32; o > 0; o >>= 1) {
            cnt += __shfl_xor(cnt, o, 64);
            hit = max(hit, (uint32_t)__shfl_xor(hit, o, 64));
        }
        if (lane == 0) {
            PK[(size_t)t * ldp + s] = cnt == 1 ? ent_ub[hit] : make_uint2(cnt ? PRED_MULTI : PRED_NONE, 0u);
            if (cnt > 1) atomicAdd(multi, 1ull);
        }
    }
}

template <class K>
__global__ void k_loss_round_sparse(const uint32_t* __restrict__ PRED, size_t ldp, const K* __restrict__ DST,
                                    size_t npad, const uint32_t* __restrict__ nodes, uint32_t n, uint32_t V,
                                    const uint2* __restrict__ ent_ub, const K* __restrict__ ent_w,
                                    const uint32_t* __restrict__ csc_off,
                                    const uint32_t* __restrict__ csc_ent, const float* __restrict__ Lin,
                                    float* __restrict__ Lout, uint32_t* __restrict__ changed_flag) {
    const size_t total = (size_t)n * V;
    uint32_t changed = 0;
    for (size_t i = blockIdx.x * (size_t)blockDim.x + threadIdx.x; i < total; i += (size_t)gridDim.x * blockDim.x) {
        const size_t r = i / V, t = i - r * V;
        const uint32_t s = nodes[r];
        const uint32_t p = PRED[r * ldp + t];
        const float* Lrow = Lin + r * ldp;
        float v;
        if (t == s) {
            v = 0.0f;
        } else if (p == PRED_NONE) {
            v = 1.0f;
        } else if (p != PRED_MULTI) {
            const uint2 ub = ent_ub[p];
            v = fold_loss(Lrow[ub.x], __uint_as_float(ub.y));
// ... 155 lines not shown
```

Before: 232,200.

## Fuse post-FW certify, extract, ess mask and counting into one row pass

Adds a fused post-Floyd-Warshall kernel that, in a single read of each D/W row, certifies reachability, extracts output latencies, builds the essential-edge mask, counts per-tile entries, and computes the min key. A row-oriented fill kernel and a late-loss kernel restricted to essential edges are added, and the table copy reuses the precomputed minima instead of a separate reduction. The aim is to cut repeated full-matrix passes and host syncs after FW. The fused path applies only to single-device, identity-node, aligned cases, and it moves the late-loss wait after the read-back, which adds complexity and more special-case paths.

```diff
diff --git a/include/shadow_routing.h b/include/shadow_routing.h
--- a/include/shadow_routing.h
+++ b/include/shadow_routing.h
@@ -114,6 +114,8 @@
 #define SRG_OPT_SCAN_MIRROR_CAP 42
 #define SRG_OPT_LOSS_KIND 43
 #define SRG_OPT_ROUTE_TREE_ROWS 44
+#define SRG_OPT_POST_FW_FUSED 45
+#define SRG_OPT_POST_FW_RAN 46
 #define SRG_LOSS_NONE 0
 #define SRG_LOSS_ROWS_LDS 1
 #define SRG_LOSS_GLOBAL_ENTRIES 2
diff --git a/shadow_amd/_native.py b/shadow_amd/_native.py
--- a/shadow_amd/_native.py
+++ b/shadow_amd/_native.py
@@ -55,6 +55,8 @@
 SRG_OPT_SCAN_MIRROR_CAP = 42
 SRG_OPT_LOSS_KIND = 43
 SRG_OPT_ROUTE_TREE_ROWS = 44
+SRG_OPT_POST_FW_FUSED = 45
+SRG_OPT_POST_FW_RAN = 46
 SRG_ROUTE_NONE = 0xFFFFFFFF
 SRG_LOSS_NONE = 0
 SRG_LOSS_ROWS_LDS = 1
diff --git a/shadow_amd/csrc/dense.hip.h b/shadow_amd/csrc/dense.hip.h
--- a/shadow_amd/csrc/dense.hip.h
+++ b/shadow_amd/csrc/dense.hip.h
@@ -3,6 +3,7 @@
                float* out_loss, hipStream_t st, const Prelude& P, srg_stats* stats, HostSink* sink,
                FwOverlap* ov = nullptr) {
     const bool pre = ov && ov->on && ov->ok && ov->ended && sizeof(K) == 4 && T == FwOverlap::T;
+    c.post_min_valid = false;
     if (sizeof(K) == 8 && c.kout_key) {
         if (!(sink && sink->widen)) fail(SRG_INTERNAL_NEED_U64, "the build needs u64 latency keys: no u32 key table");
         sink->widen = false;
@@ -49,6 +50,12 @@
     }
     HIP_CHECK(hipGetLastError());
     const double ms_build = tm.lap();
+    const bool simulated = c.comm && std::strcmp(c.comm->kind(), "simulated") == 0;
+    const bool al16 = (((uintptr_t)out_lat | (uintptr_t)c.kout_key) & 15u) == 0;
+    const bool fused = c.post_fw_fused && pl.G == 1 && !multi && !simulated && nloc && nloc == n && n == V && P.ident &&
+                       n % 4 == 0 && al16;
+    const bool fused_rows = fused && !g.directed;
+    c.post_fw_ran = fused ? 1 | (wl_late && sizeof(K) == 4 ? 2 : 0) | (fused_rows ? 4 : 0) : 0;
 
     uint64_t prof_relax = 0;
     int prof_n = 0;
@@ -73,7 +80,10 @@
     if (c.test_fault == 1)
         HIP_CHECK(hipMemsetAsync(D, 0, VV * sizeof(K), st));
 #endif
-    if (wl_late) {
+    if (wl_late && fused) {
+        HIP_CHECK(hipMemsetAsync(WL, 0xFF, VV * 4, c.aux_stream));
+        HIP_CHECK(hipEventRecord(c.ev_wlate, c.aux_stream));
+    } else if (wl_late) {
         hipStream_t ax = c.aux_stream;
         const auto tl0 = std::chrono::steady_clock::now();
         loss_arrive(g, P.selfloss, ax);
@@ -132,7 +142,7 @@
         c.comm->allgatherv(out, offs.data(), lens.data(), cs);
     };
 
-    hipStream_t es = multi ? st : c.comm_stream;
+    hipStream_t es = multi || fused ? st : c.comm_stream;
     auto drain_es = [&]() {
         if (es != st) HIP_CHECK(hipStreamSynchronize(es));
     };
@@ -152,7 +162,7 @@
     HIP_CHECK(hipMemsetAsync(multi_cnt, 0, 8, st));
     const uint32_t nw64 = (V + 63) / 64;
     unsigned long long* ess = (unsigned long long*)c.b_ess.get((size_t)V * nw64 * 8);
-    k_ess_mask<K><<<V, 256, 0, es>>>(W, D, Vp, V, 0u, V, nw64, ess);
+    if (!fused) k_ess_mask<K><<<V, 256, 0, es>>>(W, D, Vp, V, 0u, V, nw64, ess);
     uint32_t* indeg = (uint32_t*)c.b_indeg.get(((size_t)nw64 * 64 + 1) * 4);
     uint32_t* cscoff = (uint32_t*)c.b_cscoff.get(((size_t)nw64 * 64 + 1) * 4);
     HIP_CHECK(hipMemsetAsync(indeg, 0, ((size_t)nw64 * 64 + 1) * 4, es));
@@ -166,12 +176,27 @@
     uint32_t* v5_cnt = (uint32_t*)c.b_ecnt.get((size_t)nbTT5 * nK5 * V5_TT * 4);
     uint32_t* v5_goff = (uint32_t*)c.b_eoff.get((NG5 + 1) * 4);
     uint64_t E_ess = 0, E_layout = 0;
+    const K min_key = (K)std::min<uint64_t>(min_edge_key(P.es.min_lat_inv, P.unit), (uint64_t)KeyOps<K>::INF);
+    PostFw* pf = fused ? (PostFw*)c.b_postfw.get(sizeof(PostFw)) : nullptr;
     {
         uint32_t* v5_glen = (uint32_t*)c.b_rlen.get((NG5 + 1) * 4);
         HIP_CHECK(hipMemsetAsync(v5_cnt, 0, (size_t)nbTT5 * nK5 * V5_TT * 4, es));
         HIP_CHECK(hipMemsetAsync(v5_glen, 0, (NG5 + 1) * 4, es));
         const size_t nwaves = (size_t)nw64 * nK5;
-        k_v5_count<<<(unsigned)((nwaves * 64 + 255) / 256), 256, 0, es>>>(ess, V, nw64, nK5, v5_cnt, v5_glen, indeg);
+        if (fused) {
+            HIP_CHECK(hipMemsetAsync(pf, 0xFF, sizeof(PostFw), st));
+            HIP_CHECK(hipMemsetAsync(pf, 0, 16, st));
+            k_closed_rows<K><<<nloc, 256, 0, st>>>(D, W, Vp, lnodes, V, nw64, min_key, P.selflat, P.unit, out_lat,
+                                                   c.kout_key, c.kout_diag, ess, fused_rows ? v5_cnt : nullptr, indeg,
+                                                   nK5, pf);
+            HIP_CHECK(hipGetLastError());
+        }
+        if (fused_rows) {
+            const size_t total = (size_t)nbTT5 * nK5 * V5_TT;
+            k_v5_glen<<<(unsigned)((total + 255) / 256), 256, 0, st>>>(v5_cnt, total, v5_glen);
+        } else {
+            k_v5_count<<<(unsigned)((nwaves * 64 + 255) / 256), 256, 0, es>>>(ess, V, nw64, nK5, v5_cnt, v5_glen, indeg);
+        }
         HIP_CHECK(hipGetLastError());
         size_t ta = 0, tc = 0;
         HIP_CHECK(hipcub::DeviceScan::ExclusiveSum(nullptr, ta, indeg, cscoff, (int)(NT + 1), es));
@@ -183,15 +208,25 @@
         HIP_CHECK(hipGetLastError());
     }
 
-    HIP_CHECK(hipMemsetAsync(&P.flags->inf_in_used_row, 0, 4, st));
-    HIP_CHECK(hipMemsetAsync(&P.flags->impossible, 0, 4, st));
-    if (nloc)
-        k_certify<K><<<nloc, kThreads, 0, st>>>(
-            D, Vp, lnodes, nloc, nodes, n,
-            (K)std::min<uint64_t>(min_edge_key(P.es.min_lat_inv, P.unit), (uint64_t)KeyOps<K>::INF), P.flags);
-    const bool simulated = c.comm && std::strcmp(c.comm->kind(), "simulated") == 0;
-    uint32_t impossible = 0, inf_any = 0;
-    if (multi) {
+    if (!fused) {
+        HIP_CHECK(hipMemsetAsync(&P.flags->inf_in_used_row, 0, 4, st));
+        HIP_CHECK(hipMemsetAsync(&P.flags->impossible, 0, 4, st));
+        if (nloc) k_certify<K><<<nloc, kThreads, 0, st>>>(D, Vp, lnodes, nloc, nodes, n, min_key, P.flags);
+    }
+    uint32_t impossible = 0, inf_any = 0, unreach_any = 0;
+    if (fused) {
+        rb_async(c, MS_POSTFW, pf, st);
+        rb_async(c, MS_TAIL0, cscoff + NT, st);
+        rb_async(c, MS_TAIL1, v5_goff + NG5, st);
+        HIP_CHECK(hipStreamSynchronize(st));
+        const PostFw h = rb_get<PostFw>(c, MS_POSTFW);
+        impossible = h.impossible, inf_any = h.inf_in_used_row, unreach_any = h.unreachable_used_pair;
+        E_ess = rb_get<uint32_t>(c, MS_TAIL0);
+        E_layout = 2ull * rb_get<uint32_t>(c, MS_TAIL1);
+        c.post_min[0] = h.min_key, c.post_min[1] = h.min_diag;
+        c.post_min_keys = c.kout_key != nullptr;
+        c.post_min_valid = true;
+    } else if (multi) {
         impossible = reduce_flag(&P.flags->impossible);
         inf_any = reduce_flag(&P.flags->inf_in_used_row);
     } else {
@@ -242,9 +277,10 @@
         }
     }
 
-    HIP_CHECK(hipMemsetAsync(&P.flags->unreachable_used_pair, 0, 4, st));
-    const bool al16 = (((uintptr_t)out_lat | (uintptr_t)c.kout_key) & 15u) == 0;
-    if (nloc && P.ident && n % 4 == 0 && al16)
+    if (!fused) HIP_CHECK(hipMemsetAsync(&P.flags->unreachable_used_pair, 0, 4, st));
+    if (fused)
+        ;
+    else if (nloc && P.ident && n % 4 == 0 && al16)
         k_extract_ident<K><<<nloc, 256, 0, st>>>(D, Vp, lnodes, n, P.selflat, out_lat, P.flags, P.unit, c.kout_key,
                                                  c.kout_diag);
     else if (nloc)
@@ -252,7 +288,8 @@
                                                                       P.selflat, P.selfloss, out_lat, out_loss,
                                                                       P.flags, 1, P.unit, c.kout_key, c.kout_diag);
     HIP_CHECK(hipGetLastError());
-    if (reduce_flag(&P.flags->unreachable_used_pair)) {
+    if (!fused) unreach_any = reduce_flag(&P.flags->unreachable_used_pair);
+    if (unreach_any) {
         if (sizeof(K) == 8 && P.range_risk)
             fail(SRG_ERR_LATENCY_RANGE, "a used pair has no path below 2^62 latency units (max edge latency " +
                                             std::to_string(P.es.max_lat) +
@@ -271,7 +308,7 @@
         sink->lat_sent = true;
     }
 
-    {
+    if (!fused) {
         rb_async(c, MS_TAIL0, cscoff + NT, es);
         rb_async(c, MS_TAIL1, v5_goff + NG5, es);
         HIP_CHECK(hipStreamSynchronize(es));
@@ -279,11 +316,32 @@
         E_layout = 2ull * rb_get<uint32_t>(c, MS_TAIL1);
     }
     n_ess = E_ess;
-    if (wl_late) HIP_CHECK(hipStreamWaitEvent(st, c.ev_wlate, 0));
+    auto wl_join = [&]() {
+        if (!wl_late) return;
+        if constexpr (sizeof(K) == 4) {
+            if (fused) {
+                hipStream_t ax = c.aux_stream;
+                const auto tl0 = std::chrono::steady_clock::now();
+                loss_arrive(g, P.selfloss, ax);
+                if (srg_env::debug_overlap())
+                    std::fprintf(stderr, "late loss: the host waited %.2f ms for the loss thread after the read-back\n",
+                                 std::chrono::duration<double, std::milli>(std::chrono::steady_clock::now() - tl0).count());
+                if (g.E)
+                    k_wl_ess<<<grid_for(g.E), kThreads, 0, ax>>>(g.E, g.src, g.dst, g.lat, P.unit, g.loss, g.directed,
+                                                               (const uint32_t*)W, WL, Vp, ess, nw64, V);
+                HIP_CHECK(hipGetLastError());
+                HIP_CHECK(hipEventRecord(c.ev_wlate, ax));
+            }
+        }
+    };
+    auto wl_wait = [&]() {
+        if (wl_late) HIP_CHECK(hipStreamWaitEvent(st, c.ev_wlate, 0));
+    };
     const bool sparse = (double)E_ess <= c.sparse_threshold * (double)V * (double)V &&
                         E_layout + 256 < 0xF0000000ull && dst_bytes < 0xFFFFFFFFull;
     if (sparse) {
         scan_kind = SRG_SCAN_SPARSE;
+        wl_join();
         K* DST = nullptr;
         const uint32_t* DSTs = nullptr;
         uint32_t dsts_bytes = 0;
@@ -310,8 +368,12 @@
         uint2* ent_ub = (uint2*)c.b_grpe.get(Eb * 8);
         uint32_t* cscent = (uint32_t*)c.b_cscent.get(std::max<uint64_t>(E_ess, 1) * 4);
         k_v5_cscpos<<<(NT + 255) / 256, 256, 0, st>>>(v5_cnt, cscoff, NT, nK5, cscpos);
+        wl_wait();
         uint2* rec = (uint2*)c.b_entkey.get((Eb + V5_SLACK) * 8);
-        {
+        if (fused_rows) {
+            k_v5_fill_rows<K><<<NT, 256, 0, st>>>(ess, W, WL, Vp, V, nw64, nK5, v5_cnt, v5_goff, cscpos, rec, ent_w,
+                                                  ent_ub, cscent);
+        } else {
             const size_t nwaves = (size_t)nw64 * nK5;
             k_v5_fill<K><<<(unsigned)((nwaves * 64 + 255) / 256), 256, 0, st>>>(ess, W, WL, Vp, V, nw64, nK5, v5_cnt,
                                                                                   v5_goff, cscpos, rec, ent_w,
@@ -463,6 +525,8 @@
         }
     } else {
         scan_kind = SRG_SCAN_DENSE;
+        wl_join();
+        wl_wait();
         if (nloc) {
             c.loss_kind = SRG_LOSS_DENSE_SCAN;
             const size_t lds3 = (size_t)2 * KC * (TS + VE) * sizeof(K);
diff --git a/shadow_amd/csrc/host_entry.hip.h b/shadow_amd/csrc/host_entry.hip.h
--- a/shadow_amd/csrc/host_entry.hip.h
+++ b/shadow_amd/csrc/host_entry.hip.h
@@ -291,7 +291,8 @@
     const size_t r0 = ep.rows.lo, r1 = ep.rows.hi;
     const size_t rows_off = r0 * n, rows_nn = r1 > r0 ? (r1 - r0) * n : 0;
     unsigned long long hmin = ~0ull;
-    if (rows_nn && stats) {
+    const bool have_min = c.post_min_valid && c.post_min_keys == kmode && r0 == 0 && r1 == n;
+    if (rows_nn && stats && !have_min) {
         unsigned long long* dmin = (unsigned long long*)c.b_multi.get(16);
         HIP_CHECK(hipMemsetAsync(dmin, 0xFF, 16, st));
         if (kmode) {
@@ -315,9 +316,10 @@
         HIP_CHECK(hipMemcpyAsync(out_loss + rows_off, t.loss + rows_off, rows_nn * 4, hipMemcpyDeviceToHost, st));
     HIP_CHECK(hipStreamSynchronize(st));
     if (rows_nn && stats) {
-        hmin = rb_get<unsigned long long>(c, MS_MIN);
+        hmin = have_min ? c.post_min[0] : rb_get<unsigned long long>(c, MS_MIN);
         if (kmode) {
-            const unsigned long long dmin = *reinterpret_cast<const unsigned long long*>(c.hbox + 64 * MS_MIN + 8);
+            const unsigned long long dmin =
+                have_min ? c.post_min[1] : *reinterpret_cast<const unsigned long long*>(c.hbox + 64 * MS_MIN + 8);
             const uint64_t unit = stats->latency_unit_ns ? stats->latency_unit_ns : 1;
             hmin = std::min<unsigned long long>(hmin == ~0ull ? ~0ull : hmin * unit, dmin);
         }
@@ -355,6 +357,7 @@
                     nullptr, g->node_ids};
         const bool sparse = choose_sparse(*c, dg);
         const bool sim = ep.shard && std::strcmp(c->comm->kind(), "simulated") == 0;
+        c->post_min_valid = false;
         FwOverlap ov;
         LateLoss late;
         const Shipped sh = ship_edges(*c, g, nodes, n, direct, sparse, ep, sim, st, dg, ov, late, stats);
diff --git a/shadow_amd/csrc/post_fw_rule.h b/shadow_amd/csrc/post_fw_rule.h
--- /dev/null
+++ b/shadow_amd/csrc/post_fw_rule.h
@@ -0,0 +1,42 @@
+#pragma once
+#include <stddef.h>
+#include <stdint.h>
+
+#if defined(__HIPCC__)
+#define SRG_PFW_HD __host__ __device__
+#else
+#define SRG_PFW_HD
+#endif
+
+namespace srg {
+
+constexpr uint32_t PFW_TT = 128;
+constexpr uint32_t PFW_TW = 16;
+constexpr uint32_t PFW_UC = 64;
+constexpr uint32_t PFW_GROUP = 4;
+
+SRG_PFW_HD inline uint32_t pfw_popc(unsigned long long w) {
+#if defined(__HIP_DEVICE_COMPILE__)
+    return (uint32_t)__popcll(w);
+#else
+    return (uint32_t)__builtin_popcountll(w);
+#endif
+}
+
+SRG_PFW_HD inline size_t pfw_cnt_index(uint32_t t, uint32_t k, uint32_t nK) {
+    return ((size_t)(t / PFW_TT) * nK + k) * PFW_TT + t % PFW_TT;
+}
+SRG_PFW_HD inline size_t pfw_slice_index(uint32_t t, uint32_t k, uint32_t nK) {
+    return ((size_t)(t / PFW_TT) * nK + k) * (PFW_TT / PFW_TW) + (t % PFW_TT) / PFW_TW;
+}
+SRG_PFW_HD inline uint32_t pfw_pairs(uint32_t c) { return (c + 1) / 2; }
+SRG_PFW_HD inline uint32_t pfw_glen(uint32_t pairs) { return (pairs + PFW_GROUP - 1) / PFW_GROUP * PFW_GROUP; }
+
+SRG_PFW_HD inline size_t pfw_entry(unsigned long long word, uint32_t lane, uint32_t goff, uint32_t before) {
+    return 2 * ((size_t)goff + before) + pfw_popc(word & ((1ull << lane) - 1ull));
+}
+SRG_PFW_HD inline uint32_t pfw_rec_lo(uint32_t lane, size_t e, uint32_t t) {
+    return lane * 512u | ((e & 1) ? 0u : ((t % PFW_TW) << 16));
+}
+
+}
diff --git a/shadow_amd/csrc/routing.hip b/shadow_amd/csrc/routing.hip
--- a/shadow_amd/csrc/routing.hip
+++ b/shadow_amd/csrc/routing.hip
@@ -535,6 +535,100 @@
         }
     }
     if (__ballot(unreach) && (threadIdx.x & 63) == 0) atomicOr(&flags->unreachable_used_pair, 1u);
+}
+
+struct PostFw {
+    uint32_t impossible, inf_in_used_row, unreachable_used_pair, pad;
+    unsigned long long min_key, min_diag;
+};
+
+template <class K>
+__global__ void __launch_bounds__(256) k_closed_rows(const K* __restrict__ D, const K* __restrict__ W, size_t ld,
+                                                     const uint32_t* __restrict__ snodes, uint32_t V, uint32_t nw64,
+                                                     K min_key, const uint64_t* __restrict__ self_lat, uint64_t unit,
+                                                     uint64_t* __restrict__ out_lat, uint32_t* __restrict__ out_key,
+                                                     uint64_t* __restrict__ out_diag, unsigned long long* __restrict__ ess,
+                                                     uint32_t* __restrict__ cnt, uint32_t* __restrict__ indeg, uint32_t nK,
+                                                     PostFw* pf) {
+    const uint32_t lane = threadIdx.x & 63;
+    const uint32_t s = snodes[blockIdx.x];
+    const K* Ds = D + (size_t)s * ld;
+    const K* Ws = W + (size_t)s * ld;
+    const uint64_t sl = self_lat[s];
+    uint32_t hit = 0, bad = 0, unreach = 0, pop = 0, mk = 0xFFFFFFFFu;
+    unsigned long long ml = ~0ull;
+    const uint32_t NT = nw64 * 64;
+    for (uint32_t t0 = 0; t0 < NT; t0 += 1024) {
+        const uint32_t t = t0 + threadIdx.x * 4;
+        K d[4] = {1, 1, 1, 1}, w[4] = {0, 0, 0, 0};
+        if (t < NT) {
+            if constexpr (sizeof(K) == 4) {
+                const uint4 a = *reinterpret_cast<const uint4*>(Ds + t);
+                const uint4 b = *reinterpret_cast<const uint4*>(Ws + t);
+                d[0] = a.x, d[1] = a.y, d[2] = a.z, d[3] = a.w;
+                w[0] = b.x, w[1] = b.y, w[2] = b.z, w[3] = b.w;
+            } else {
+                const ulonglong2 a0 = *reinterpret_cast<const ulonglong2*>(Ds + t);
+                const ulonglong2 a1 = *reinterpret_cast<const ulonglong2*>(Ds + t + 2);
+                const ulonglong2 b0 = *reinterpret_cast<const ulonglong2*>(Ws + t);
+                const ulonglong2 b1 = *reinterpret_cast<const ulonglong2*>(Ws + t + 2);
+                d[0] = a0.x, d[1] = a0.y, d[2] = a1.x, d[3] = a1.y;
+                w[0] = b0.x, w[1] = b0.y, w[2] = b1.x, w[3] = b1.y;
+            }
+        }
+        if (t < V) {
+            uint64_t o[4];
+            uint32_t k[4];
+#pragma unroll
+            for (int u = 0; u < 4; ++u) {
+                const bool diag = t + u == s;
+                hit |= d[u] == KeyOps<K>::INF;
+                bad |= impossible_key<K>(d[u], min_key, diag);
+                unreach |= !diag && d[u] == KeyOps<K>::INF;
+                k[u] = diag ? 0xFFFFFFFFu : (uint32_t)d[u];
+                o[u] = diag ? sl : (uint64_t)d[u] * unit;
+                mk = k[u] < mk ? k[u] : mk;
+                ml = o[u] < ml ? o[u] : ml;
+            }
+            if (out_key) {
+                *reinterpret_cast<uint4*>(out_key + (size_t)s * V + t) = make_uint4(k[0], k[1], k[2], k[3]);
+            } else {
+                uint64_t* ol = out_lat + (size_t)s * V + t;
+                *reinterpret_cast<ulonglong2*>(ol) = make_ulonglong2(o[0], o[1]);
+                *reinterpret_cast<ulonglong2*>(ol + 2) = make_ulonglong2(o[2], o[3]);
+            }
+        }
+        unsigned long long nib = 0;
+#pragma unroll
+        for (uint32_t j = 0; j < 4; ++j)
+            nib |= (unsigned long long)(t + j < V && t + j != s && w[j] != KeyOps<K>::INF && w[j] == d[j]) << j;
+        unsigned long long v = nib << (4 * (lane & 15));
+#pragma unroll
+        for (int o = 1; o < 16; o <<= 1) v |= __shfl_xor(v, o, 64);
+        if ((lane & 15) == 0 && t < NT) {
+            const uint32_t wi = t / 64;
+            ess[(size_t)s * nw64 + wi] = v;
+            if (cnt) {
+                const uint32_t c = pfw_popc(v);
+                cnt[pfw_cnt_index(s, wi, nK)] = c;
+                pop += c;
+            }
+        }
+    }
+    if (cnt && pop) atomicAdd(&indeg[s], pop);
+    if (__ballot(hit) && lane == 0) atomicOr(&pf->inf_in_used_row, 1u);
+    if (__ballot(bad) && lane == 0) atomicOr(&pf->impossible, 1u);
+    if (__ballot(unreach) && lane == 0) atomicOr(&pf->unreachable_used_pair, 1u);
+    unsigned long long m = out_key ? (mk == 0xFFFFFFFFu ? ~0ull : (unsigned long long)mk) : ml;
+    for (int off = 32; off > 0; off >>= 1) {
+        const unsigned long long o = __shfl_down(m, off, 64);
+        m = o < m ? o : m;
+    }
+    if (lane == 0 && m < *(volatile unsigned long long*)&pf->min_key) atomicMin(&pf->min_key, m);
+    if (threadIdx.x == 0 && out_key) {
+        out_diag[s] = sl;
+        if (sl < *(volatile unsigned long long*)&pf->min_diag) atomicMin(&pf->min_diag, (unsigned long long)sl);
+    }
 }
 
 __global__ void k_min_u64(const uint64_t* __restrict__ a, size_t count, unsigned long long* out) {
@@ -755,6 +849,12 @@
     int loss_kind = 0;
     int scan_mirror_cap = 0;
     DevBuf b_tri;
+    int post_fw_fused = 1;
+    int post_fw_ran = 0;
+    DevBuf b_postfw;
+    bool post_min_valid = false;
+    bool post_min_keys = false;
+    unsigned long long post_min[2] = {~0ull, ~0ull};
     int test_fault = 0;
     std::shared_ptr<TablePool> tpool = std::make_shared<TablePool>();
     double ms_create_runtime = 0, ms_create_lib = 0;
@@ -866,7 +966,7 @@
     std::memcpy(&v, c.hbox + 64 * slot, sizeof(T));
     return v;
 }
-enum MailSlot { MS_EDGESTATS, MS_FLAGS, MS_TIMEOUT, MS_REDUCE, MS_TAIL0, MS_TAIL1, MS_NMULTI, MS_CHANGED, MS_MIN, MS_REDUCE2, MS_MIRROR };
+enum MailSlot { MS_EDGESTATS, MS_FLAGS, MS_TIMEOUT, MS_REDUCE, MS_TAIL0, MS_TAIL1, MS_NMULTI, MS_CHANGED, MS_MIN, MS_REDUCE2, MS_MIRROR, MS_POSTFW };
 
 struct Prelude {
     EdgeStats es;
@@ -2193,6 +2293,10 @@
             if (value != 0 && value != 1) return SRG_ERR_ARG;
             ctx->scan_mirror = (int)value;
             return SRG_OK;
+        case SRG_OPT_POST_FW_FUSED:
+            if (value != 0 && value != 1) return SRG_ERR_ARG;
+            ctx->post_fw_fused = (int)value;
+            return SRG_OK;
         case SRG_OPT_SCAN_MIRROR_CAP:
             if (!(value >= 0 && value <= 1073741824.0)) return SRG_ERR_ARG;
             ctx->scan_mirror_cap = (int)value;
@@ -2258,6 +2362,8 @@
         case SRG_OPT_SCAN_MIRRORED: *value = ctx->scan_mirrored; break;
         case SRG_OPT_SCAN_MIRROR_CAP: *value = ctx->scan_mirror_cap; break;
         case SRG_OPT_LOSS_KIND: *value = ctx->loss_kind; break;
+        case SRG_OPT_POST_FW_FUSED: *value = ctx->post_fw_fused; break;
+        case SRG_OPT_POST_FW_RAN: *value = ctx->post_fw_ran; break;
         case SRG_OPT_ROUTE_TREE_ROWS: *value = ctx->route_tree_rows; break;
         default: return SRG_ERR_ARG;
     }
diff --git a/shadow_amd/csrc/tight_sparse.hip.h b/shadow_amd/csrc/tight_sparse.hip.h
--- a/shadow_amd/csrc/tight_sparse.hip.h
+++ b/shadow_amd/csrc/tight_sparse.hip.h
@@ -3,6 +3,7 @@
 #include <stdint.h>
 
 #include "kernels.hip.h"
+#include "post_fw_rule.h"
 
 namespace srg {
 
@@ -170,6 +171,100 @@
             ent_w[q] = KeyOps<K>::INF;
             ent_ub[q] = make_uint2(0u, __float_as_uint(1.0f));
         }
+    }
+}
+
+static_assert(PFW_TT == V5_TT && PFW_TW == V5_TW && PFW_UC == V5_UC, "post_fw_rule.h mirrors the scan's tile shape");
+__global__ void __launch_bounds__(256) k_v5_glen(const uint32_t* __restrict__ cnt, size_t total,
+                                                  uint32_t* __restrict__ glen) {
+    const size_t i = blockIdx.x * (size_t)blockDim.x + threadIdx.x;
+    uint32_t p = i < total ? pfw_pairs(cnt[i]) : 0u;
+#pragma unroll
+    for (int off = 1; off < (int)V5_TW; off <<= 1) p += __shfl_xor(p, off, V5_TW);
+    if (i < total && (threadIdx.x % V5_TW) == 0) glen[i / V5_TW] = pfw_glen(p);
+}
+
+template <class K>
+__global__ void __launch_bounds__(256) k_v5_fill_rows(const unsigned long long* __restrict__ ess,
+                                                       const K* __restrict__ W, const uint32_t* __restrict__ WL,
+                                                       size_t ld, uint32_t V, uint32_t nw64, uint32_t nK,
+                                                       const uint32_t* __restrict__ cnt, const uint32_t* __restrict__ goff,
+                                                       const uint32_t* __restrict__ csc_pos,
+                                                       uint2* __restrict__ rec, K* __restrict__ ent_w,
+                                                       uint2* __restrict__ ent_ub, uint32_t* __restrict__ csc_ent) {
+    const uint32_t lane = threadIdx.x & 63, wave = threadIdx.x >> 6;
+    const uint32_t t = blockIdx.x, j = t % V5_TW;
+    const K* Wt = W + (size_t)t * ld;
+    const uint32_t* WLt = WL + (size_t)t * ld;
+    for (uint32_t kb = 0; kb < nK; kb += 256) {
+        const uint32_t km = kb + lane * 4 + wave;
+        unsigned long long mword = 0;
+        uint32_t mbefore = 0, mtotal = 0, mgoff = 0, mgnext = 0, mcp = 0;
+        if (km < nK) {
+            if (t < V) mword = ess[(size_t)t * nw64 + km];
+            const size_t ci = pfw_cnt_index(t - j, km, nK);
+#pragma unroll
+            for (uint32_t q = 0; q < V5_TW; ++q) {
+                const uint32_t p = pfw_pairs(cnt[ci + q]);
+                mtotal += p;
+                mbefore += q < j ? p : 0u;
+            }
+            const size_t g = pfw_slice_index(t, km, nK);
+            mgoff = goff[g];
+            mgnext = goff[g + 1];
+            mcp = csc_pos[ci + j];
+        }
+        for (uint32_t i = 0; i < 64; ++i) {
+            const uint32_t k = kb + i * 4 + wave;
+            if (k >= nK) break;
+            const unsigned long long word = __shfl(mword, (int)i, 64);
+            const uint32_t before = __shfl(mbefore, (int)i, 64), pbase = __shfl(mgoff, (int)i, 64);
+            const uint32_t cp = __shfl(mcp, (int)i, 64);
+            const uint32_t c = pfw_popc(word);
+            if ((word >> lane) & 1ull) {
+                const uint32_t u = k * V5_UC + lane;
+                const uint32_t rank = pfw_popc(word & ((1ull << lane) - 1ull));
+                const size_t e = pfw_entry(word, lane, pbase, before);
+                const K w = Wt[u];
+                const uint32_t l = WLt[u];
+                rec[e] = make_uint2(pfw_rec_lo(lane, e, t), (uint32_t)w);
+                ent_w[e] = w;
+                ent_ub[e] = make_uint2(u, __float_as_uint(__fsub_rn(1.0f, __uint_as_float(l))));
+                csc_ent[cp + rank] = (uint32_t)e;
+            }
+            if (lane == 0 && (c & 1u)) {
+                const size_t e = 2 * ((size_t)pbase + before) + c;
+                rec[e] = make_uint2(0u, KeyOps<uint32_t>::INF);
+                ent_w[e] = KeyOps<K>::INF;
+                ent_ub[e] = make_uint2(0u, __float_as_uint(1.0f));
+            }
+            if (j == V5_TW - 1) {
+                const size_t q0 = 2 * ((size_t)pbase + __shfl(mtotal, (int)i, 64));
+                const size_t q1 = 2 * (size_t)__shfl(mgnext, (int)i, 64);
+                for (size_t q = q0 + lane; q < q1; q += 64) {
+                    rec[q] = make_uint2(0u, KeyOps<uint32_t>::INF);
+                    ent_w[q] = KeyOps<K>::INF;
+                    ent_ub[q] = make_uint2(0u, __float_as_uint(1.0f));
+                }
+            }
+        }
+    }
+}
+
+__global__ void k_wl_ess(uint64_t E, const uint32_t* __restrict__ src, const uint32_t* __restrict__ dst,
+                         const uint64_t* __restrict__ lat, uint64_t unit, const float* __restrict__ loss, int directed,
+                         const uint32_t* __restrict__ W, uint32_t* __restrict__ WL, size_t ld,
+                         const unsigned long long* __restrict__ ess, uint32_t nw64, uint32_t V) {
+    for (size_t e = blockIdx.x * (size_t)blockDim.x + threadIdx.x; e < E; e += (size_t)gridDim.x * blockDim.x) {
+        const uint32_t s = src[e], t = dst[e];
+        if (s == t || s >= V || t >= V) continue;
+        const bool fwd = (ess[(size_t)s * nw64 + t / 64] >> (t % 64)) & 1ull;
+        const bool bwd = !directed && ((ess[(size_t)t * nw64 + s / 64] >> (s % 64)) & 1ull);
+        if (!fwd && !bwd) continue;
+        const uint64_t l = unit != 1 ? lat[e] / unit : lat[e];
+        const uint32_t bits = __float_as_uint(loss[e] + 0.0f);
+        if (fwd && (uint64_t)W[(size_t)s * ld + t] == l) atomicMin(&WL[(size_t)s * ld + t], bits);
+        if (bwd && (uint64_t)W[(size_t)t * ld + s] == l) atomicMin(&WL[(size_t)t * ld + s], bits);
     }
 }
 
```

Result: slower. 215,000 (-7.4%).
